# Adredes-weslee/elliptic-gnn-project

Hardware: AMD Instinct MI355X
Metric: edges/s full-batch SAGE fwd+bwd, Elliptic 203k/234k/166-feat, 1→8 MI355X (higher is better)
Workload: dtype f32; 1 GPU; configs/sage.yaml + symmetrize_edges=true: SAGE 2L 166->128->2, dropout 0.5, full-batch train step (fwd+masked CE+bwd+clip+Adam); global_nodes=203769, global_edges=468710, feats=166, max_nodes_per_gpu=203769, max_edges_per_gpu=468710, parallelism=single, launch=hip-graph replay of the whole step

## Files before the change

### elliptic_gnn_project_amd/_lib.py

```python
from __future__ import annotations

import ctypes
import os
from pathlib import Path

import torch

PKG_DIR = Path(__file__).resolve().parent
LIB_PATH = Path(os.environ["GNNMP_LIB"]) if os.environ.get("GNNMP_LIB") else PKG_DIR / "libgnnmp.so"
ABI_VERSION = 27

DTYPE_F32 = 0
DTYPE_BF16 = 1

MATH_SPLIT_BF16 = 0
MATH_F32 = 1
MATH_HALF_PAIR = 2

PLANES_SPLIT_BF16 = 0
PLANES_HALF_PAIR = 1

GNN_OK = 0
_STATUS_EXC = {
    1: ValueError,
    2: IndexError,
    3: RuntimeError,
    4: RuntimeError,
    5: NotImplementedError,
}

LOOPS_KEEP = 0
LOOPS_REPLACE = 1

AGG_SUM = 0
AGG_MEAN = 1
AGG_MEAN_BWD = 2
AGG_GCN = 3
AGG_EDGE_W = 4

c_i64 = ctypes.c_int64
c_i32 = ctypes.c_int32
c_ptr = ctypes.c_void_p
c_size = ctypes.c_size_t


class GnnSplit(ctypes.Structure):
    _fields_ = [
        ("seg_len", c_i32),
        ("reserved", c_i32),
        ("num_long", c_i64),
        ("num_pieces", c_i64),
        ("ptr", c_ptr),
        ("nbr", c_ptr),
        ("piece0", c_ptr),
        ("piece_seg", c_ptr),
        ("long_seg", c_ptr),
        ("order", c_ptr),
    ]


class GnnGraph(ctypes.Structure):
    _fields_ = [
        ("num_nodes", c_i64),
# ... 26 lines not shown
        ("seed_ptr", c_ptr),
        ("addend2", c_ptr),
        ("ld_add2", c_i64),
    ]


class GnnGemmNTParams(ctypes.Structure):
    _fields_ = [
        ("M", c_i64), ("N", c_i64),
        ("a1", c_ptr), ("lda1", c_i64), ("k1", c_i64),
        ("a2", c_ptr), ("lda2", c_i64), ("k2", c_i64),
        ("bt", c_ptr), ("ldb", c_i64),
        ("w1", c_ptr), ("w2", c_ptr), ("ldw1", c_i64), ("ldw2", c_i64),
        ("c", c_ptr), ("ldc", c_i64),
        ("bias", c_ptr),
        ("relu", c_i32),
        ("dropout_p", ctypes.c_float),
        ("seed", ctypes.c_uint64),
        ("seed_ptr", c_ptr),
        ("proj", c_ptr), ("nproj", c_i32), ("z", c_ptr), ("ldz", c_i64),
        ("math", c_i32),
        ("workspace", c_ptr), ("workspace_bytes", c_size),
        ("a_dtype", c_i32), ("c_dtype", c_i32),
        ("mask", c_ptr), ("ldmask", c_i64), ("mask_scale", ctypes.c_float),
        ("a_planes", c_ptr), ("planes_ld", c_i64), ("planes_stride", c_i64), ("planes_col2", c_i64),
        ("planes_format", c_i32), ("keep_mask", c_ptr), ("b_ready", c_i32), ("planes_exp", c_i32),
        ("colsum_part", c_ptr), ("colsum_cap", c_i64),
        ("row_exp", c_ptr),
    ]


class GnnGemmTNParams(ctypes.Structure):
    _fields_ = [
        ("M", c_i64), ("Nr", c_i64),
        ("g", c_ptr), ("ldg", c_i64),
        ("dz", c_ptr), ("lddz", c_i64),
        ("proj", c_ptr), ("nproj", c_i32),
        ("h", c_ptr), ("ldh", c_i64), ("hscale", ctypes.c_float),
        ("gout", c_ptr), ("ldgout", c_i64),
        ("a1", c_ptr), ("lda1", c_i64), ("k1", c_i64),
        ("a2", c_ptr), ("lda2", c_i64), ("k2", c_i64),
        ("math", c_i32),
        ("a_dtype", c_i32), ("h_dtype", c_i32),
        ("a_planes", c_ptr), ("planes_ld", c_i64), ("planes_stride", c_i64), ("planes_col2", c_i64),
        ("planes_format", c_i32), ("g_dtype", c_i32), ("planes_exp", c_i32),
        ("sq_partial", c_ptr), ("sq_step", c_ptr), ("sq_skip_lo", c_i64), ("sq_skip_hi", c_i64), ("sq_cap", c_i64),
        ("row_exp", c_ptr),
        ("g_rowmax", c_ptr),
        ("dz_graph", c_ptr), ("dz_u", c_ptr), ("ldu", c_i64), ("dz_cols", c_i32),
    ]


ROWMAX_ROWS = 16


ACT_NONE = 0
ACT_ELU = 1


class GnnGatFwdParams(ctypes.Structure):
    _fields_ = [
        ("heads", c_i32), ("chans", c_i32), ("concat", c_i32),
        ("slope", ctypes.c_float),
        ("xh", c_ptr), ("ld_xh", c_i64),
        ("att_src", c_ptr), ("att_dst", c_ptr),
        ("bias", c_ptr),
        ("act", ctypes.c_int),
        ("dropout_p", ctypes.c_float),
        ("seed", ctypes.c_uint64), ("seed_ptr", c_ptr),
        ("a_src", c_ptr), ("a_dst", c_ptr),
        ("alpha", c_ptr),
        ("out", c_ptr), ("ldo", c_i64),
        ("edge_w", c_ptr),
        ("proj", c_ptr), ("nproj", c_i32), ("z", c_ptr), ("ldz", c_i64),
    ]


ADAM_MAX_TENSORS = 24


class GnnAdamTensor(ctypes.Structure):
    _fields_ = [("param", c_ptr), ("grad", c_ptr), ("exp_avg", c_ptr), ("exp_avg_sq", c_ptr), ("numel", c_i64)]


class GnnAdamGroup(ctypes.Structure):
    _fields_ = [
        ("num_tensors", c_i32),
        ("lr", ctypes.c_double), ("beta1", ctypes.c_double), ("beta2", ctypes.c_double), ("eps", ctypes.c_double),
        ("weight_decay", ctypes.c_double), ("max_norm", ctypes.c_double),
        ("tensors", GnnAdamTensor * ADAM_MAX_TENSORS),
        ("skip_nonfinite", c_i32),
        ("bump_counter", c_ptr),
        ("loss_partial", c_ptr), ("loss_nblk", c_i32), ("loss_scale", ctypes.c_float), ("loss_out", c_ptr),
        ("grad_sq_partial", c_ptr), ("grad_sq_nblk", c_i32),
    ]


class GnnCeSpec(ctypes.Structure):
    _fields_ = [
        ("y", c_ptr), ("mask", c_ptr), ("class_w", c_ptr), ("row_w", c_ptr),
        ("inv_denom", ctypes.c_float), ("focal", c_i32), ("focal_gamma", ctypes.c_float),
        ("reserved", c_i32 * 5),
    ]


SIGNATURES = {
    "gnn_abi_version": (ctypes.c_int, []),
    "gnn_status_string": (ctypes.c_char_p, [ctypes.c_int]),
    "gnn_last_error": (ctypes.c_char_p, []),
    "gnn_graph_workspace_size": (ctypes.c_int, [c_i64, c_i64, ctypes.POINTER(c_size)]),
    "gnn_graph_build": (
        ctypes.c_int,
        [c_ptr, c_i64, c_i64, ctypes.c_int, c_ptr, c_ptr, c_ptr, c_ptr, c_ptr, c_ptr, c_ptr, c_ptr, c_size, c_ptr],
    ),
    "gnn_split_workspace_size": (ctypes.c_int, [c_i64, ctypes.POINTER(c_size)]),
    "gnn_split_count": (ctypes.c_int, [c_ptr, c_i64, c_i32, c_ptr, c_ptr]),
    "gnn_split_build": (
        ctypes.c_int,
        [c_ptr, c_ptr, c_i64, c_i32, c_ptr, c_ptr, c_ptr, c_ptr, c_ptr, c_ptr, c_ptr, c_size, c_ptr],
    ),
    "gnn_in_degree_f32": (ctypes.c_int, [ctypes.POINTER(GnnGraph), c_ptr, c_ptr]),
    "gnn_gcn_norm_f32": (ctypes.c_int, [ctypes.POINTER(GnnGraph), c_ptr, c_ptr]),
    "gnn_aggregate_f32": (
        ctypes.c_int,
        [ctypes.POINTER(GnnGraph), ctypes.POINTER(GnnAggParams), c_ptr, c_i64, c_i64, c_ptr, c_i64, c_ptr],
    ),
    "gnn_aggregate_bf16": (
        ctypes.c_int,
        [ctypes.POINTER(GnnGraph), ctypes.POINTER(GnnAggParams), c_ptr, c_i64, c_i64, c_ptr, c_i64, c_ptr],
    ),
    "gnn_sage_mean_fwd_f32": (
        ctypes.c_int,
        [ctypes.POINTER(GnnGraph), c_ptr, c_ptr, c_i64, c_i64, c_ptr, c_i64, c_ptr],
    ),
    "gnn_split_planes_f32": (ctypes.c_int, [c_ptr, c_i64, c_i64, c_i64, c_ptr, c_i64, c_i64, c_i64, c_i64, c_ptr]),
    "gnn_sage_mean_fwd_planes": (
        ctypes.c_int,
        [ctypes.POINTER(GnnGraph), c_ptr, c_ptr, c_i64, c_i64, c_ptr, c_i64, c_i64, c_i64, c_ptr],
    ),
    "gnn_split_h2_f32": (ctypes.c_int, [c_ptr, c_i64, c_i64, c_i64, c_ptr, c_i64, c_i64, c_i64, c_i64, c_i32, c_ptr]),
    "gnn_sage_mean_fwd_h2": (
        ctypes.c_int,
        [ctypes.POINTER(GnnGraph), c_ptr, c_ptr, c_i64, c_i64, c_ptr, c_i64, c_i64, c_i64, c_i32,
         c_ptr, c_i64, ctypes.c_float, ctypes.c_uint64, c_ptr, ctypes.POINTER(GnnGemmNTParams),
         ctypes.POINTER(GnnSplit), c_ptr],
    ),
    "gnn_sage_out_mean_ce_f32": (
        ctypes.c_int,
        [ctypes.POINTER(GnnGraph), c_ptr, c_ptr, c_i64, c_i32, c_ptr, c_ptr, c_i64, c_ptr, c_ptr, c_ptr,
         ctypes.c_float, c_ptr, c_i64, c_ptr, c_i64, c_ptr, c_ptr, c_ptr, c_size, c_ptr],
    ),
    "gnn_sage_mean_bwd_f32": (
        ctypes.c_int,
        [ctypes.POINTER(GnnGraph), c_ptr, c_ptr, c_i64, c_i64, c_ptr, c_i64, c_ptr],
    ),
    "gnn_edge_dot_f32": (
        ctypes.c_int,
        [ctypes.POINTER(GnnGraph), c_ptr, c_ptr, c_ptr, c_i64, c_ptr, c_i64, c_i64, c_ptr, c_ptr],
    ),
    "gnn_gat_scores_f32": (
        ctypes.c_int,
        [c_i64, c_i32, c_i32, c_ptr, c_i64, c_ptr, c_ptr, c_ptr, c_ptr, c_ptr],
    ),
    "gnn_gat_fwd_f32": (
        ctypes.c_int,
        [ctypes.POINTER(GnnGraph), c_i32, c_i32, c_i32, ctypes.c_float, c_ptr, c_i64, c_ptr, c_ptr,
         c_ptr, c_ptr, c_ptr, c_i64, c_ptr],
    ),
    "gnn_gat_fwd_fused_f32": (ctypes.c_int, [ctypes.POINTER(GnnGraph), ctypes.POINTER(GnnGatFwdParams), c_ptr]),
    "gnn_gat_out_ce_f32": (
        ctypes.c_int,
        [ctypes.POINTER(GnnGraph), ctypes.POINTER(GnnGatFwdParams), c_ptr, c_ptr, c_ptr, ctypes.c_float, c_ptr, c_i64,
         c_ptr, c_ptr, c_ptr, c_size, c_ptr]),
    "gnn_gat_act_bwd_f32": (
        ctypes.c_int,
        [c_i64, c_i64, ctypes.c_int, ctypes.c_float, ctypes.c_uint64, c_ptr, c_ptr, c_i64, c_ptr, c_i64, c_ptr,
         c_i64, c_ptr],
    ),
    "gnn_gat_bwd_workspace_size": (ctypes.c_int, [c_i64, c_i64, c_i32, c_i32, ctypes.POINTER(c_size)]),
    "gnn_gat_bwd_f32": (
        ctypes.c_int,
        [ctypes.POINTER(GnnGraph), c_i32, c_i32, c_i32, ctypes.c_float, c_ptr, c_i64, c_ptr, c_ptr, c_ptr,
         c_ptr, c_ptr, c_ptr, c_i64, c_ptr, c_i64, c_ptr, c_ptr, c_ptr, c_size, c_ptr],
    ),
    "gnn_gat_bwd_act_proj_f32": (
        ctypes.c_int,
        [ctypes.POINTER(GnnGraph), c_i32, c_i32, ctypes.c_float, c_ptr, c_i64, c_ptr, c_ptr, c_ptr, c_ptr, c_ptr,
         c_i32, ctypes.c_float, ctypes.c_uint64, c_ptr, c_ptr, c_i64, c_ptr, c_i64, c_ptr, c_i32, c_ptr, c_i64,
         c_ptr, c_i64, c_ptr, c_ptr, c_ptr, c_ptr, c_size, c_ptr]),
    "gnn_gat_bwd_act_f32": (
        ctypes.c_int,
        [ctypes.POINTER(GnnGraph), c_i32, c_i32, ctypes.c_float, c_ptr, c_i64, c_ptr, c_ptr, c_ptr, c_ptr, c_ptr,
         c_i32, ctypes.c_float, ctypes.c_uint64, c_ptr, c_ptr, c_i64, c_ptr, c_i64, c_ptr, c_i64, c_ptr, c_i64,
         c_ptr, c_ptr, c_ptr, c_size, c_ptr],
    ),
    "gnn_gat_bwd_ew_f32": (
        ctypes.c_int,
        [ctypes.POINTER(GnnGraph), c_i32, c_i32, c_i32, ctypes.c_float, c_ptr, c_i64, c_ptr, c_ptr, c_ptr,
         c_ptr, c_ptr, c_ptr, c_i64, c_ptr, c_i64, c_ptr, c_ptr, c_ptr, c_ptr, c_ptr, c_size, c_ptr],
    ),
    "gnn_gemm_nt_workspace_size": (ctypes.c_int, [c_i64, c_i64, c_i64, ctypes.POINTER(c_size)]),
    "gnn_gemm_nt_f32": (ctypes.c_int, [ctypes.POINTER(GnnGemmNTParams), c_ptr]),
    "gnn_gemm_nt_prep_b": (ctypes.c_int, [ctypes.POINTER(GnnGemmNTParams), c_ptr]),
    "gnn_masked_ce_finish": (ctypes.c_int, [c_ptr, c_i32, ctypes.c_float, c_ptr, c_ptr]),
    "gnn_gemm_tn_workspace_size": (ctypes.c_int, [c_i64, c_i64, c_i64, c_i32, ctypes.POINTER(c_size)]),
    "gnn_gemm_tn_sq_blocks": (ctypes.c_int, [c_i64, ctypes.POINTER(c_i32)]),
    "gnn_gemm_tn_f32": (ctypes.c_int, [ctypes.POINTER(GnnGemmTNParams), c_ptr, c_ptr, c_size, c_ptr]),
    "gnn_gemm_nt_planes_ok": (ctypes.c_int, [ctypes.POINTER(GnnGemmNTParams)]),
    "gnn_gemm_nt_colsum_blocks": (ctypes.c_int, [ctypes.POINTER(GnnGemmNTParams), ctypes.POINTER(c_i32)]),
    "gnn_colsum_finish_f32": (ctypes.c_int, [c_ptr, c_i32, c_i64, c_ptr, c_ptr]),
    "gnn_gemm_tn_planes_ok": (ctypes.c_int, [ctypes.POINTER(GnnGemmTNParams)]),
    "gnn_colsum_workspace_size": (ctypes.c_int, [c_i64, c_i64, ctypes.POINTER(c_size)]),
    "gnn_colsum_f32": (ctypes.c_int, [c_i64, c_i64, c_ptr, c_i64, c_ptr, c_ptr, c_size, c_ptr]),
    "gnn_masked_ce_workspace_size": (ctypes.c_int, [c_i64, ctypes.POINTER(c_size)]),
    "gnn_masked_ce_f32": (
        ctypes.c_int,
        [c_i64, c_i32, c_ptr, c_i64, c_ptr, c_ptr, c_ptr, ctypes.c_float, c_ptr, c_i64, c_ptr, c_ptr, c_size, c_ptr],
    ),
    "gnn_gcn_out_ce_f32": (
        ctypes.c_int,
        [ctypes.POINTER(GnnGraph), c_ptr, c_ptr, c_i64, c_i32, c_ptr, c_ptr, c_i64, c_ptr, c_ptr, c_ptr,
         ctypes.c_float, c_ptr, c_i64, c_ptr, c_ptr, c_ptr, c_size, c_ptr],
    ),
    "gnn_masked_ce_colsum_f32": (
        ctypes.c_int,
        [c_i64, c_i32, c_ptr, c_i64, c_ptr, c_ptr, c_ptr, ctypes.c_float, c_ptr, c_i64, c_ptr, c_ptr, c_size, c_ptr,
         c_ptr],
    ),
    "gnn_masked_ce_spec_f32": (
        ctypes.c_int,
        [c_i64, c_i32, c_ptr, c_i64, ctypes.POINTER(GnnCeSpec), c_ptr, c_i64, c_ptr, c_ptr, c_size, c_ptr, c_ptr],
    ),
    "gnn_sage_out_mean_ce_spec_f32": (
        ctypes.c_int,
        [ctypes.POINTER(GnnGraph), c_ptr, c_ptr, c_i64, c_i32, c_ptr, c_ptr, c_i64, ctypes.POINTER(GnnCeSpec),
         c_ptr, c_i64, c_ptr, c_i64, c_ptr, c_ptr, c_ptr, c_size, c_ptr],
    ),
    "gnn_gcn_out_ce_spec_f32": (
        ctypes.c_int,
        [ctypes.POINTER(GnnGraph), c_ptr, c_ptr, c_i64, c_i32, c_ptr, c_ptr, c_i64, ctypes.POINTER(GnnCeSpec),
         c_ptr, c_i64, c_ptr, c_ptr, c_ptr, c_size, c_ptr],
    ),
    "gnn_gat_out_ce_spec_f32": (
        ctypes.c_int,
        [ctypes.POINTER(GnnGraph), ctypes.POINTER(GnnGatFwdParams), ctypes.POINTER(GnnCeSpec), c_ptr, c_i64,
         c_ptr, c_ptr, c_ptr, c_size, c_ptr]),
    "gnn_clip_adam_workspace_size": (ctypes.c_int, [ctypes.POINTER(c_size)]),
    "gnn_neighbor_sample_workspace_size": (ctypes.c_int, [c_i64, c_i64, c_i64, ctypes.POINTER(c_size)]),
    "gnn_neighbor_sample": (
        ctypes.c_int,
        [ctypes.POINTER(GnnGraph), c_ptr, c_ptr, c_i64, c_i32, c_ptr, ctypes.c_uint64, c_ptr, c_i64, c_ptr, c_ptr,
         c_ptr, c_i64, c_ptr, c_ptr, c_ptr, c_size, c_ptr],
    ),
    "gnn_clip_adam_f32": (ctypes.c_int, [ctypes.POINTER(GnnAdamGroup), c_ptr, c_ptr, c_ptr, c_size, c_ptr]),
    "gnn_bn_workspace_size": (ctypes.c_int, [c_i64, ctypes.POINTER(c_size)]),
    "gnn_bn_stats_f32": (
        ctypes.c_int,
        [c_ptr, c_i64, c_i64, c_i64, c_ptr, c_i32, ctypes.c_float, ctypes.c_float, c_ptr, c_ptr, c_ptr, c_ptr,
         c_ptr, c_ptr, c_size, c_ptr],
    ),
# ... 84 lines not shown
```

### elliptic_gnn_project_amd/aggregation.py

```python
from __future__ import annotations

import os

import torch

from . import _lib
from .graph import GraphPlan, get_plan

__all__ = ["mean_aggregate", "masked_mean_aggregate", "masked_gcn_aggregate", "edge_dot", "gcn_aggregate", "gat_attention", "gat_attention_proj", "aggregate", "colsum", "KernelTimer"]


class KernelTimer:

    active = False
    records: list = []

    @classmethod
    def start(cls):
        cls.records = []
        cls.active = True

    @classmethod
    def begin(cls):
        if not cls.active:
            return None
        e = torch.cuda.Event(enable_timing=True)
        e.record()
        return e

    @classmethod
    def end(cls, e0, tag, amount):
        if e0 is None:
            return
        e1 = torch.cuda.Event(enable_timing=True)
        e1.record()
        cls.records.append((tag, e0, e1, int(amount)))

    @classmethod
    def stop(cls):
        cls.active = False
        torch.cuda.synchronize()
        out = {}
        for tag, a, b, amount in cls.records:
            ms = a.elapsed_time(b)
            d = out.setdefault(tag, {"launches": 0, "ms": 0.0, "amount": 0})
            d["launches"] += 1
            d["ms"] += ms
            d["amount"] += amount
        cls.records = []
        return out

_custom_fwd = torch.amp.custom_fwd(device_type="cuda", cast_inputs=torch.float32)
_custom_bwd = torch.amp.custom_bwd(device_type="cuda")


def _as_f32_rows(x: torch.Tensor) -> torch.Tensor:
    if x.dtype != torch.float32:
        raise TypeError(f"libgnnmp fp32 path got {x.dtype}")
    if x.dim() != 2:
        raise ValueError(f"expected [N, F] features, got {tuple(x.shape)}")
    if x.stride(1) != 1 or x.stride(0) < x.size(1):
        x = x.contiguous()
    return x


def _ld(x: torch.Tensor) -> int:
    return max(int(x.stride(0)), int(x.size(1)), 1)


SPLIT_MAX_F = 128


def aggregate(plan: GraphPlan, x: torch.Tensor, mode: int, transpose: bool = False,
              nodew: torch.Tensor | None = None, ew: torch.Tensor | None = None, heads: int = 1,
              addend: torch.Tensor | None = None, bias: torch.Tensor | None = None,
              relu: bool = False, out: torch.Tensor | None = None, dropout_p: float = 0.0, seed: int = 0,
              seed_ptr: torch.Tensor | None = None, addend2: torch.Tensor | None = None) -> torch.Tensor:
    if x.dtype == torch.bfloat16:
        if dropout_p > 0 or addend2 is not None:
            raise NotImplementedError("dropout / addend2 epilogue on the bf16-storage aggregation")
        return _aggregate_bf16(plan, x, mode, transpose, nodew, addend, bias, relu, out)
    x = _as_f32_rows(x)
    N, F = plan.num_nodes, x.size(1)
    if x.size(0) != N:
        raise ValueError(f"feature rows {x.size(0)} != plan nodes {N}")
    if out is None:
        out = torch.empty((N, F), dtype=torch.float32, device=x.device)
    if addend is not None:
        addend = _as_f32_rows(addend)
    if addend2 is not None:
        addend2 = _as_f32_rows(addend2)
    npieces = plan.split_pieces(transpose) if (mode != _lib.AGG_EDGE_W and 8 < F <= SPLIT_MAX_F) else 0
    part = torch.empty(npieces * F, dtype=torch.float32, device=x.device) if npieces else None
    p = _lib.GnnAggParams(
        mode, int(transpose), _lib.ptr(nodew), _lib.ptr(ew), int(heads),
        _lib.ptr(addend), _ld(addend) if addend is not None else 0,
        _lib.ptr(bias), int(relu), _lib.ptr(part), part.numel() * 4 if part is not None else 0,
        float(dropout_p), int(seed) & 0xFFFFFFFFFFFFFFFF, _lib.ptr(seed_ptr),
        _lib.ptr(addend2), _ld(addend2) if addend2 is not None else 0,
    )
    if KernelTimer.active:
        a = torch.cuda.Event(enable_timing=True)
        b = torch.cuda.Event(enable_timing=True)
        a.record()
    _lib.call("gnn_aggregate_f32", plan.c_graph, p, x.data_ptr(), _ld(x), F, out.data_ptr(), _ld(out),
              _lib.stream_handle(x.device))
    if KernelTimer.active:
        b.record()
        KernelTimer.records.append((("agg", int(mode), bool(transpose), int(F)), a, b,
                                    agg_bytes(plan, F, mode, transpose, int(addend is not None) + int(addend2 is not None))))
    return out


def _aggregate_bf16(plan, x, mode, transpose, nodew, addend, bias, relu, out):
    if x.dim() != 2 or x.stride(1) != 1:
        x = x.contiguous()
    N, F = plan.num_nodes, x.size(1)
    if x.size(0) != N:
        raise ValueError(f"feature rows {x.size(0)} != plan nodes {N}")
    if out is None:
        out = torch.empty((N, F), dtype=torch.bfloat16, device=x.device)
    if out.dtype != torch.bfloat16:
        raise TypeError("bf16 aggregation writes bf16")
    if addend is not None:
        addend = _as_f32_rows(addend)
    p = _lib.GnnAggParams(
        mode, int(transpose), _lib.ptr(nodew), None, 1,
        _lib.ptr(addend), _ld(addend) if addend is not None else 0,
        _lib.ptr(bias), int(relu), None, 0,
    )
    if KernelTimer.active:
        a = torch.cuda.Event(enable_timing=True)
        b = torch.cuda.Event(enable_timing=True)
        a.record()
    _lib.call("gnn_aggregate_bf16", plan.c_graph, p, x.data_ptr(), _ld(x), F, out.data_ptr(), _ld(out),
              _lib.stream_handle(x.device))
    if KernelTimer.active:
        b.record()
        KernelTimer.records.append((("agg_bf16", int(mode), bool(transpose), int(F)), a, b,
                                    agg_bytes(plan, F, mode, transpose, addend is not None, elem=2)))
    return out


def agg_bytes(plan: GraphPlan, F: int, mode: int, transpose: bool, has_addend, elem: int = 4) -> int:
    N, S = plan.num_nodes, plan.num_slots
    b = 4 * (N + 1) + 4 * S + elem * S * F + elem * N * F
    if mode in (_lib.AGG_MEAN,):
        b += 4 * N
    elif mode in (_lib.AGG_MEAN_BWD, _lib.AGG_GCN):
        b += 4 * S
    b += 4 * N * F * int(has_addend)
    return b


def colsum_of(x: torch.Tensor) -> torch.Tensor:
    part = getattr(x, "_gnnmp_colsum", None)
    if part is not None and x.dim() == 2 and x.size(1) > 0 and part.numel() % x.size(1) == 0 and part.numel() > 0:
        out = torch.empty(x.size(1), dtype=torch.float32, device=x.device)
        _lib.call("gnn_colsum_finish_f32", part.data_ptr(), part.numel() // x.size(1), x.size(1), out.data_ptr(),
# ... 411 lines not shown
```

### elliptic_gnn_project_amd/csrc/aggregate.hip

```cpp
#include "gemm_common.hpp"

namespace gnnmp {
namespace {

template <int VEC>
struct VecT;
template <>
struct VecT<1> { using T = float; };
template <>
struct VecT<2> { using T = float2; };
template <>
struct VecT<4> { using T = float4; };

template <int VEC>
__device__ __forceinline__ void vload(const float* p, float (&v)[VEC]) {
  if constexpr (VEC == 4) {
    float4 t = *reinterpret_cast<const float4*>(p);
    v[0] = t.x; v[1] = t.y; v[2] = t.z; v[3] = t.w;
  } else if constexpr (VEC == 2) {
    float2 t = *reinterpret_cast<const float2*>(p);
    v[0] = t.x; v[1] = t.y;
  } else {
    v[0] = *p;
  }
// ... 16 lines not shown
    const uint4 t = *reinterpret_cast<const uint4*>(p);
    v[0] = __uint_as_float(t.x << 16); v[1] = __uint_as_float(t.x & 0xffff0000u);
    v[2] = __uint_as_float(t.y << 16); v[3] = __uint_as_float(t.y & 0xffff0000u);
    v[4] = __uint_as_float(t.z << 16); v[5] = __uint_as_float(t.z & 0xffff0000u);
    v[6] = __uint_as_float(t.w << 16); v[7] = __uint_as_float(t.w & 0xffff0000u);
  } else if constexpr (VEC == 4) {
    const uint2 t = *reinterpret_cast<const uint2*>(p);
    v[0] = __uint_as_float(t.x << 16); v[1] = __uint_as_float(t.x & 0xffff0000u);
    v[2] = __uint_as_float(t.y << 16); v[3] = __uint_as_float(t.y & 0xffff0000u);
  } else if constexpr (VEC == 2) {
    const uint32_t t = *reinterpret_cast<const uint32_t*>(p);
    v[0] = __uint_as_float(t << 16); v[1] = __uint_as_float(t & 0xffff0000u);
  } else {
    v[0] = __uint_as_float((uint32_t)p[0] << 16);
  }
}

__device__ __forceinline__ uint16_t to_bf16(float f) { return __builtin_bit_cast(uint16_t, (__bf16)f); }

template <int VEC>
__device__ __forceinline__ void vstore_bf(uint16_t* p, const float (&v)[VEC]) {
  if constexpr (VEC == 8) {
    *reinterpret_cast<uint4*>(p) = make_uint4((uint32_t)to_bf16(v[0]) | ((uint32_t)to_bf16(v[1]) << 16),
                                              (uint32_t)to_bf16(v[2]) | ((uint32_t)to_bf16(v[3]) << 16),
                                              (uint32_t)to_bf16(v[4]) | ((uint32_t)to_bf16(v[5]) << 16),
                                              (uint32_t)to_bf16(v[6]) | ((uint32_t)to_bf16(v[7]) << 16));
  } else if constexpr (VEC == 4) {
    *reinterpret_cast<uint2*>(p) = make_uint2((uint32_t)to_bf16(v[0]) | ((uint32_t)to_bf16(v[1]) << 16),
                                              (uint32_t)to_bf16(v[2]) | ((uint32_t)to_bf16(v[3]) << 16));
  } else if constexpr (VEC == 2) {
    *reinterpret_cast<uint32_t*>(p) = (uint32_t)to_bf16(v[0]) | ((uint32_t)to_bf16(v[1]) << 16);
  } else {
    p[0] = to_bf16(v[0]);
  }
}

struct AggArgs {
  const int32_t* ptr;
  const int32_t* nbr;
  const int32_t* wslot;
  const float* nodew;
  const float* ew;
  int32_t heads;
  int32_t chan;
  const float* x; int64_t ldx;
  float* y; int64_t ldy;
  const float* add; int64_t ld_add;
  const float* add2; int64_t ld_add2;
  const float* bias;
  int32_t relu;
  int64_t nrows;
  int32_t F;
  const int32_t* piece0;
  const int32_t* order;
  float* part;
  const int32_t* fptr;
  const int32_t* fnbr;
  int32_t seg_len;
  int32_t dropout; uint32_t keep_thresh; float drop_scale; uint64_t seed; const int64_t* seed_ptr;
  uint16_t* yp; int64_t yps; int32_t ywidth;
  float yscale;
  uint32_t* kmask; int32_t kcols;
  H2Prep hp;
  int32_t nhub; float hub_deg; const int32_t* hubs;
  const int32_t* wstart;
  const int64_t* ce_y; const uint8_t* ce_mask; const float* ce_w; float ce_inv;
  float* ce_dl; int64_t ce_ldd; float* ce_part;
  float* ce_u; int64_t ce_ldu;
  const float* ce_rw; int32_t ce_focal; float ce_gamma;
  float* ce_cs;
};

__device__ __forceinline__ uint64_t agg_seed(const AggArgs& a) {
  return a.seed_ptr ? (uint64_t)(*a.seed_ptr) * 0x9E3779B97F4A7C15ull + a.seed : a.seed;
}

template <int VEC>
__device__ __forceinline__ void agg_dropout(const AggArgs& a, uint64_t seed, int64_t r, int f0, float (&t)[VEC]) {
  if (a.dropout) {
    const uint32_t i0 = (uint32_t)r * (uint32_t)a.F + (uint32_t)f0;
#pragma unroll
    for (int q = 0; q < VEC; ++q) t[q] = keep_elem(seed, i0 + (uint32_t)q, a.keep_thresh) ? t[q] * a.drop_scale : 0.0f;
  }
}

template <int MODE, int VEC>
__device__ __forceinline__ void contrib(const AggArgs& a, int32_t n, int32_t r, int64_t slot,
                                        int f0, float (&v)[VEC]) {
  if constexpr (MODE == GNN_AGG_MEAN_BWD) {
    float d = fmaxf(a.nodew[n], 1.0f);
#pragma unroll
    for (int q = 0; q < VEC; ++q) v[q] = v[q] / d;
  } else if constexpr (MODE == GNN_AGG_GCN) {
    const float w = a.nodew[n] * a.nodew[r];
#pragma unroll
    for (int q = 0; q < VEC; ++q) v[q] = w * v[q];
  } else if constexpr (MODE == GNN_AGG_EDGE_W) {
    int64_t ws = a.wslot ? (int64_t)a.wslot[slot] : slot;
    float w = a.ew[ws * a.heads + f0 / a.chan];
#pragma unroll
    for (int q = 0; q < VEC; ++q) v[q] = w * v[q];
  }
}

template <int MODE, int VEC, bool BF = false>
__device__ __forceinline__ void contrib_w(const AggArgs& a, float wn, int32_t r, float (&v)[VEC]) {
// ... 668 lines not shown
#pragma unroll
      for (int f = 0; f < NF; ++f) {
        float v = xv[f];
        if constexpr (MODE == GNN_AGG_GCN) {
          v = (wn * wr) * v;
        } else if constexpr (MODE == GNN_AGG_MEAN_BWD) {
          v = v / fmaxf(wn, 1.0f);
        } else {
          float t[1] = {v};
          contrib<MODE, 1>(a, n, (int32_t)r, k, f, t);
          v = t[0];
        }
        acc[f] += f < a.F ? v : 0.0f;
      }
    }
#pragma unroll
    for (int f = 0; f < NF; ++f) {
#pragma unroll
      for (int off = kGroup / 2; off >= 1; off >>= 1) acc[f] += __shfl_xor(acc[f], off);
    }
    if (sub == 0) {
      const int32_t p0 = a.piece0 ? a.piece0[r] : -1;
      const float dr = MODE == GNN_AGG_MEAN ? fmaxf(a.nodew[r], 1.0f) : 1.0f;
      float addv[NF], add2v[NF], bv[NF];
#pragma unroll
      for (int f = 0; f < NF; ++f) {
        const int fc = f < a.F ? f : 0;
        addv[f] = a.add ? a.add[r * a.ld_add + fc] : 0.0f;
        add2v[f] = a.add2 ? a.add2[r * a.ld_add2 + fc] : 0.0f;
        bv[f] = a.bias ? a.bias[fc] : 0.0f;
      }
      const uint64_t dseed = a.dropout ? agg_seed(a) : 0;
#pragma unroll
      for (int f = 0; f < NF; ++f) {
        if (f < a.F) {
          float t[1] = {acc[f]};
          if (p0 >= 0) {
            a.part[(int64_t)p0 * a.F + f] = t[0];
          } else {
            if constexpr (MODE == GNN_AGG_MEAN) t[0] = t[0] / dr;
            if (a.add) t[0] += addv[f];
            if (a.add2) t[0] += add2v[f];
            if (a.bias) t[0] += bv[f];
            if (a.relu) t[0] = fmaxf(t[0], 0.0f);
            if (a.dropout) agg_dropout<1>(a, dseed, r, f, t);
            a.y[r * a.ldy + f] = t[0];
          }
        }
      }
    }
  }
}

template <int MODE, int NF, int kNarrowCap = 256, bool COOP = false, bool CE = false, bool CEV = false>
__global__ __launch_bounds__(256) void agg_narrow_lds_kernel(AggArgs a) {
  __shared__ float sv[4][kNarrowCap * 4];
  const int lane = threadIdx.x & 63;
  const int w = threadIdx.x >> 6;
  const int64_t r0 = ((int64_t)blockIdx.x * 4 + w) * 64;
  float lg[4] = {0.f, 0.f, 0.f, 0.f};
  int64_t ce_t = -1;
  float ce_deg = 1.0f;
  uint8_t ce_m = 0;
  float ce_w[4] = {0.f, 0.f, 0.f, 0.f};
  float ce_rw = 1.0f;
  if constexpr (!CE) {
    if (r0 >= a.nrows) return;
  }
  if (r0 < a.nrows) {
  const int64_t r = r0 + lane;
  const bool rok = r < a.nrows;
  const int32_t pbeg = a.ptr[rok ? r : a.nrows];
  const int32_t pend = a.ptr[rok ? r + 1 : a.nrows];
  const int32_t base = __builtin_amdgcn_readfirstlane(a.ptr[r0]);
  const int64_t rlast = min(r0 + 64, a.nrows);
  const int32_t wend = __builtin_amdgcn_readfirstlane(a.ptr[rlast]);
  const int F = a.F;
  const int64_t rr = rok ? r : r0;
  float pdeg = 1.0f, padd[4] = {0.f, 0.f, 0.f, 0.f}, padd2[4] = {0.f, 0.f, 0.f, 0.f}, pbias[4] = {0.f, 0.f, 0.f, 0.f};
  if constexpr (MODE == GNN_AGG_MEAN) pdeg = fmaxf(a.nodew[rr], 1.0f);
  static_assert(MODE != GNN_AGG_GCN || NF == 2, "GCN rows stage their slot weight in plane 2");
  float wrow = 1.0f;
  if constexpr (MODE == GNN_AGG_GCN) wrow = a.nodew[rr];
  if (a.add) {
#pragma unroll
    for (int f = 0; f < NF; ++f) padd[f] = a.add[rr * a.ld_add + (f < F ? f : 0)];
  }
  if (a.add2) {
#pragma unroll
    for (int f = 0; f < NF; ++f) padd2[f] = a.add2[rr * a.ld_add2 + (f < F ? f : 0)];
  }
  if (a.bias) {
#pragma unroll
    for (int f = 0; f < NF; ++f) pbias[f] = a.bias[f < F ? f : 0];
  }
  if constexpr (CE) {
    ce_deg = pdeg;
    ce_t = a.ce_y[rr];
    ce_m = a.ce_mask[rr];
#pragma unroll
    for (int c = 0; c < 4; ++c) ce_w[c] = a.ce_w[c < F ? c : 0];
    if constexpr (CEV) {
      if (a.ce_rw) ce_rw = a.ce_rw[rr];
    }
  }
  float acc[4] = {0.f, 0.f, 0.f, 0.f};
  float* buf = sv[w];
  for (int32_t pb = base; pb < wend; pb += kNarrowCap) {
    const int32_t pe = min(pb + kNarrowCap, wend);
    constexpr int NI = kNarrowCap / 64;
    int32_t nn[NI];
#pragma unroll
    for (int i = 0; i < NI; ++i) {
      const int32_t k = pb + lane + 64 * i;
      nn[i] = a.nbr[k < pe ? k : pb];
    }
    float xv[NI][NF], dd[NI];
#pragma unroll
    for (int i = 0; i < NI; ++i) {
      const float* xr = a.x + (int64_t)nn[i] * a.ldx;
#pragma unroll
      for (int f = 0; f < NF; ++f) xv[i][f] = xr[f < F ? f : 0];
      dd[i] = 1.0f;
      if constexpr (MODE == GNN_AGG_MEAN_BWD || MODE == GNN_AGG_GCN) dd[i] = a.nodew[nn[i]];
    }
#pragma unroll
    for (int i = 0; i < NI; ++i) {
#pragma unroll
      for (int f = 0; f < NF; ++f) {
        float v = f < F ? xv[i][f] : 0.0f;
        if constexpr (MODE == GNN_AGG_MEAN_BWD) v = v / fmaxf(dd[i], 1.0f);
        buf[f * kNarrowCap + lane + 64 * i] = v;
      }
      if constexpr (MODE == GNN_AGG_GCN) buf[2 * kNarrowCap + lane + 64 * i] = dd[i];
    }
    __builtin_amdgcn_s_waitcnt(0xc07f);
    __builtin_amdgcn_wave_barrier();
    const int32_t lo = max(pbeg, pb), hi0 = min(pend, pe);
    constexpr int CAP = 32;
    const int32_t hi = COOP ? min(hi0, lo + CAP) : hi0;
    float q1[4] = {0.f, 0.f, 0.f, 0.f}, q2[4] = {0.f, 0.f, 0.f, 0.f}, q3[4] = {0.f, 0.f, 0.f, 0.f};
    auto sv_at = [&](int f, int32_t s, float wr) __attribute__((always_inline)) {
      const float x = buf[f * kNarrowCap + (s - pb)];
      if constexpr (MODE == GNN_AGG_GCN) return (buf[2 * kNarrowCap + (s - pb)] * wr) * x;
      else return x;
    };
    int32_t k = lo;
    for (; k + 3 < hi; k += 4) {
#pragma unroll
      for (int f = 0; f < NF; ++f) {
        acc[f] += sv_at(f, k, wrow);
        q1[f] += sv_at(f, k + 1, wrow);
        q2[f] += sv_at(f, k + 2, wrow);
        q3[f] += sv_at(f, k + 3, wrow);
      }
    }
    for (; k < hi; ++k) {
#pragma unroll
      for (int f = 0; f < NF; ++f) acc[f] += sv_at(f, k, wrow);
    }
#pragma unroll
    for (int f = 0; f < NF; ++f) acc[f] += (q1[f] + q2[f]) + q3[f];
    if constexpr (COOP) {
      uint64_t longm = __ballot(hi0 - lo > CAP);
      while (longm) {
        const int L = __builtin_ctzll(longm);
        longm &= longm - 1;
        const int32_t s0 = __builtin_amdgcn_readlane(lo, L) + CAP, s1 = __builtin_amdgcn_readlane(hi0, L);
        const float wL = __int_as_float(__builtin_amdgcn_readlane(__float_as_int(wrow), L));
        float part[NF];
#pragma unroll
        for (int f = 0; f < NF; ++f) part[f] = 0.f;
        for (int32_t k2 = s0 + lane; k2 < s1; k2 += 64) {
#pragma unroll
          for (int f = 0; f < NF; ++f) part[f] += sv_at(f, k2, wL);
        }
#pragma unroll
        for (int f = 0; f < NF; ++f) {
#pragma unroll
          for (int off = 32; off >= 1; off >>= 1) part[f] += __shfl_xor(part[f], off);
          if (lane == L) acc[f] += part[f];
        }
      }
    }
    __builtin_amdgcn_wave_barrier();
  }
  if (rok) {
    const int32_t p0 = a.piece0 ? a.piece0[r] : -1;
#pragma unroll
    for (int f = 0; f < 4; ++f) {
      if (f < F) {
        float t[1] = {acc[f]};
        if (p0 >= 0) {
          a.part[(int64_t)p0 * F + f] = t[0];
        } else {
          if constexpr (MODE == GNN_AGG_MEAN) t[0] = t[0] / pdeg;
          if (a.add) t[0] += padd[f];
          if (a.add2) t[0] += padd2[f];
          if (a.bias) t[0] += pbias[f];
          if (a.relu) t[0] = fmaxf(t[0], 0.0f);
          if (a.dropout) agg_dropout<1>(a, agg_seed(a), r, f, t);
          a.y[r * a.ldy + f] = t[0];
          lg[f] = t[0];
        }
      }
    }
  }
  }
  if constexpr (CE) {
    const int64_t r = r0 + lane;
    const int C = a.F;
    float l = 0.f;
    float dlv[4] = {0.f, 0.f, 0.f, 0.f};
    if (r < a.nrows) {
      const int64_t tg = ce_t;
      const bool on = ce_m != 0 && tg >= 0 && tg < C;
      const float wt = tg == 0 ? ce_w[0] : tg == 1 ? ce_w[1] : tg == 2 ? ce_w[2] : ce_w[3];
      if constexpr (CEV)
        l = masked_ce_row<4, true>(lg, C, tg, on, on ? wt : 0.f, a.ce_inv, a.ce_dl + r * a.ce_ldd, dlv, ce_rw,
                                   a.ce_focal != 0, a.ce_gamma);
      else
        l = masked_ce_row<4>(lg, C, tg, on, on ? wt : 0.f, a.ce_inv, a.ce_dl + r * a.ce_ldd, dlv);
      if (a.ce_u) {
#pragma unroll
        for (int c = 0; c < 4; ++c)
          if (c < C) a.ce_u[r * a.ce_ldu + c] = dlv[c] / ce_deg;
      }
    }
    __shared__ float cesh[4];
    for (int o = 32; o > 0; o >>= 1) l += __shfl_xor(l, o);
    if (lane == 0) cesh[w] = l;
    __syncthreads();
    if (threadIdx.x == 0) {
      float t = 0.f;
      for (int i = 0; i < 4; ++i) t += cesh[i];
      a.ce_part[blockIdx.x] = t;
    }
    if (a.ce_cs) {
      __shared__ float cssh[4][4];
#pragma unroll
      for (int c = 0; c < 4; ++c) {
        float v = c < C ? dlv[c] : 0.f;
        for (int o = 32; o > 0; o >>= 1) v += __shfl_xor(v, o);
        if (lane == 0) cssh[c][w] = v;
      }
      __syncthreads();
      if ((int)threadIdx.x < C) {
        float t = 0.f;
        for (int i = 0; i < 4; ++i) t += cssh[threadIdx.x][i];
        a.ce_cs[(int64_t)blockIdx.x * C + threadIdx.x] = t;
      }
    }
  }
}

template <int MODE, int VEC, int NCH>
__device__ __forceinline__ void agg_piece_wide_body(const AggArgs& a, int64_t npieces, const int32_t* piece_seg,
// ... 89 lines not shown
  int rpw = 16;
  bool prefetch = false;
  bool no_fold = false;
  bool no_split = false;
  bool wave_split = false;
  bool lane_walk = false;
};
#ifdef GNNMP_AGG_LAB
int g_agg_lab_variant = 0;
AggLab agg_lab() {
  const int v = g_agg_lab_variant;
  AggLab l;
  l.rpg = v == 5 ? 4 : v == 6 ? 8 : v == 8 ? -1 : (v == 9 || v == 11) ? 1 : 0;
  l.rpw = (v == 1 || v == 14) ? 8 : (v == 2 || v == 13) ? 4 : v == 3 ? 32 : 16;
  l.prefetch = v == 10 || v == 11; l.no_fold = v == 16; l.no_split = v == 7;
  l.wave_split = v >= 12 && v <= 14; l.lane_walk = v == 15;
  return l;
}
#else
constexpr AggLab agg_lab() { return {}; }
#endif

template <class Fn>
void with_vec(int vec, Fn&& f) {
  if (vec == 4) f(std::integral_constant<int, 4>{});
  else if (vec == 2) f(std::integral_constant<int, 2>{});
  else f(std::integral_constant<int, 1>{});
}

int flat_lps(int nchunk) { return nchunk <= 8 ? 8 : nchunk <= 16 ? 16 : nchunk <= 32 ? 32 : 64; }

template <int MODE, int VEC, int LPS, int NCHMAX>
void launch_flat(const AggArgs& a, int rpg, unsigned blocks, hipStream_t st, [[maybe_unused]] bool prefetch) {
#ifdef GNNMP_AGG_LAB
  if (prefetch) return (void)agg_flat_kernel<MODE, VEC, LPS, NCHMAX, true><<<blocks, 256, 0, st>>>(a, rpg);
#endif
  agg_flat_kernel<MODE, VEC, LPS, NCHMAX><<<blocks, 256, 0, st>>>(a, rpg);
}

template <int MODE>
gnn_status launch_mode(const AggArgs& a, int vec, hipStream_t st, const gnn_split* fold = nullptr) {
  if (a.nrows == 0 || a.F == 0) return GNN_OK;
  const AggLab lab = agg_lab();
  constexpr int kLdsF = MODE == GNN_AGG_EDGE_W ? 0 : MODE == GNN_AGG_GCN ? 2 : 4;
  if (a.F <= kLdsF) {
    if constexpr (kLdsF >= 2) {
      const unsigned nb = (unsigned)ceil_div(a.nrows, 256);
#ifdef GNNMP_AGG_LAB
      if (lab.lane_walk) {
        if (a.F <= 2) agg_narrow_lds_kernel<MODE, 2, 256, false><<<nb, 256, 0, st>>>(a);
        else if constexpr (kLdsF >= 4) agg_narrow_lds_kernel<MODE, 4, 256, false><<<nb, 256, 0, st>>>(a);
      } else
#endif
      if (a.F <= 2) agg_narrow_lds_kernel<MODE, 2, 256, true><<<nb, 256, 0, st>>>(a);
      else if constexpr (kLdsF >= 4) agg_narrow_lds_kernel<MODE, 4, 256, true><<<nb, 256, 0, st>>>(a);
    }
  } else if (a.F <= 8) {
    int64_t blocks = ceil_div(a.nrows * kGroup, 256);
    if (blocks > ((int64_t)1 << 20)) blocks = (int64_t)1 << 20;
    if (a.F > 4) agg_group_kernel<MODE, 8><<<(unsigned)blocks, 256, 0, st>>>(a);
    else if constexpr (kLdsF < 4) {
      if (a.F > 2) agg_group_kernel<MODE, 4><<<(unsigned)blocks, 256, 0, st>>>(a);
      else if constexpr (kLdsF < 2) agg_group_kernel<MODE, 2><<<(unsigned)blocks, 256, 0, st>>>(a);
    }
  } else {
    const int nchunk = a.F / vec;
    const int lps = flat_lps(nchunk);
    if (nchunk > 64 * 4) return fail(GNN_ERR_UNSUPPORTED, "gnn_aggregate_f32", "F too wide for the gather kernel");
    const int rpg = lab.rpg > 0 ? lab.rpg : lab.rpg < 0 ? lps - 1 : a.order ? 1 : (lps == 8 ? 7 : lps == 16 ? 2 : 8);
    const unsigned blocks = (unsigned)ceil_div(ceil_div(a.nrows, rpg) * lps, 256);
    const unsigned wblocks = (unsigned)ceil_div(ceil_div(a.nrows, lab.rpw) * 64, 256);
    with_vec(vec, [&](auto v) {
      constexpr int V = decltype(v)::value;
      if (lps == 64 && nchunk <= 128) agg_wave_kernel<MODE, V, 2, false, 8><<<wblocks, 256, 0, st>>>(a, lab.rpw);
      else if (lps == 64) launch_flat<MODE, V, 64, 4>(a, rpg, blocks, st, lab.prefetch);
      else if (lps == 32) launch_flat<MODE, V, 32, 1>(a, rpg, blocks, st, lab.prefetch);
      else if (lps == 16 && !fold) launch_flat<MODE, V, 16, 1>(a, rpg, blocks, st, lab.prefetch);
      else if (lps == 8) {
        if constexpr (V > 1) launch_flat<MODE, V, 8, 1>(a, rpg, blocks, st, lab.prefetch);
      } else if constexpr (MODE != GNN_AGG_EDGE_W) {
        const unsigned pblocks = (unsigned)ceil_div(fold->num_pieces * 64, 256);
        agg_flat_pieces_kernel<MODE, V, 16, 1><<<blocks + pblocks, 256, 0, st>>>(a, rpg, fold->num_pieces,
                                                                               fold->piece_seg, pblocks);
      }
    });
  }
  return hip_check(hipGetLastError(), "gnn_aggregate_f32");
}

template <int MODE>
gnn_status launch_mode_split(const AggArgs& a, int vec, hipStream_t st, const gnn_split* sp) {
  if (a.nrows == 0 || a.F == 0) return GNN_OK;
  const AggLab lab = agg_lab();
  const bool pieces = sp->num_pieces > sp->num_long;
  const bool fold = pieces && flat_lps(a.F / vec) == 16 && !lab.prefetch && !lab.no_fold;
  const gnn_status s = launch_mode<MODE>(a, vec, st, fold ? sp : nullptr);
  if (s != GNN_OK || sp->num_long == 0) return s;
  const unsigned pblocks = (unsigned)ceil_div(sp->num_pieces * 64, 256);
  const unsigned cblocks = (unsigned)ceil_div(sp->num_long * 64, 256);
  with_vec(vec, [&](auto v) {
    constexpr int V = decltype(v)::value;
#ifdef GNNMP_AGG_LAB
    if (a.F / V > 64) {
      if (pieces) agg_piece_wide_kernel<MODE, V, 2><<<pblocks, 256, 0, st>>>(a, sp->num_pieces, sp->piece_seg);
      return (void)agg_combine_kernel<MODE, V, 2><<<cblocks, 256, 0, st>>>(a, sp->num_long, sp->long_seg);
    }
// ... 44 lines not shown
  const int c = blockIdx.x;
  const int t = threadIdx.x;
  float a0 = 0.f, a1 = 0.f, a2 = 0.f, a3 = 0.f;
  int b = t;
  for (; b + 768 < nblk; b += 1024) {
    a0 += part[(int64_t)b * F + c];
    a1 += part[(int64_t)(b + 256) * F + c];
    a2 += part[(int64_t)(b + 512) * F + c];
    a3 += part[(int64_t)(b + 768) * F + c];
  }
  for (; b < nblk; b += 256) a0 += part[(int64_t)b * F + c];
  red[t] = (a0 + a1) + (a2 + a3);
  __syncthreads();
  for (int s = 128; s > 0; s >>= 1) {
    if (t < s) red[t] += red[t + s];
    __syncthreads();
  }
  if (t == 0) out[c] = red[0];
}

constexpr int64_t kColsumBlocks = 1024;

}
}

using namespace gnnmp;

#ifdef GNNMP_AGG_LAB
extern "C" void gnnx_set_agg_variant(int v) { g_agg_lab_variant = v; }
#endif

static gnn_status agg_args_common(AggArgs& a, const gnn_graph* g, const gnn_agg_params* p, int64_t F, const char* fn) {
  a.ptr = p->transpose ? g->colptr : g->rowptr;
  a.nbr = p->transpose ? g->row : g->col;
  a.nodew = p->nodew;
  a.add = p->addend; a.ld_add = p->ld_add;
  a.bias = p->bias; a.relu = p->relu;
  if (p->dropout_p < 0.f || p->dropout_p >= 1.f) return fail(GNN_ERR_INVALID_ARG, fn, "dropout p in [0,1)");
  if (p->dropout_p > 0.f && (int64_t)g->num_nodes * (int64_t)F >= ((int64_t)1 << 32))
    return fail(GNN_ERR_UNSUPPORTED, fn, "dropout element index (rows x width) must be < 2^32");
  a.dropout = p->dropout_p > 0.f;
  a.keep_thresh = (uint32_t)((1.0 - (double)p->dropout_p) * 16777216.0);
  a.drop_scale = a.dropout ? (float)(1.0 / (1.0 - (double)p->dropout_p)) : 1.0f;
  a.seed = p->seed;
  a.seed_ptr = p->seed_ptr;
  a.nrows = g->num_nodes;
  a.F = (int32_t)F;
  return GNN_OK;
}

extern "C" gnn_status gnn_aggregate_f32(const gnn_graph* g, const gnn_agg_params* p, const float* x,
                                        int64_t ldx, int64_t F, float* y, int64_t ldy,
                                        gnn_stream_t stream) {
  if (!g || !p) return fail(GNN_ERR_INVALID_ARG, __func__, "null graph or params");
  if (F < 0 || F > INT32_MAX || ldx < F || ldy < F)
    return fail(GNN_ERR_INVALID_ARG, __func__, "bad F / leading dimensions");
  if (g->num_nodes > 0 && F > 0 && (!x || !y)) return fail(GNN_ERR_INVALID_ARG, __func__, "null x/y");
  if (p->addend && p->ld_add < F) return fail(GNN_ERR_INVALID_ARG, __func__, "bad ld_add");
  if (p->addend2 && p->ld_add2 < F) return fail(GNN_ERR_INVALID_ARG, __func__, "bad ld_add2");
  AggArgs a{};
  if (const gnn_status s = agg_args_common(a, g, p, F, __func__); s != GNN_OK) return s;
  a.wslot = (p->mode == GNN_AGG_EDGE_W && p->transpose) ? g->csc2csr : nullptr;
  a.ew = p->ew;
  a.heads = p->heads > 0 ? p->heads : 1;
  a.x = x; a.ldx = ldx; a.y = y; a.ldy = ldy;
  a.add2 = p->addend2; a.ld_add2 = p->ld_add2;
  if (!a.ptr || (g->num_slots > 0 && !a.nbr)) return fail(GNN_ERR_INVALID_ARG, __func__, "plan arrays null");
  if ((p->mode == GNN_AGG_MEAN || p->mode == GNN_AGG_MEAN_BWD || p->mode == GNN_AGG_GCN) && !p->nodew)
    return fail(GNN_ERR_INVALID_ARG, __func__, "mode needs nodew");
  if (p->mode == GNN_AGG_EDGE_W) {
    if (!p->ew) return fail(GNN_ERR_INVALID_ARG, __func__, "EDGE_W needs ew");
    if (F % a.heads) return fail(GNN_ERR_INVALID_ARG, __func__, "F not divisible by heads");
    if (p->transpose && !g->csc2csr) return fail(GNN_ERR_INVALID_ARG, __func__, "EDGE_W transpose needs csc2csr");
  }
  a.chan = (int32_t)(F / a.heads > 0 ? F / a.heads : 1);
  auto ok_vec = [&](int v) {
    if (F % v || ldx % v || ldy % v) return false;
    if (p->addend && p->ld_add % v) return false;
    if (p->addend2 && p->ld_add2 % v) return false;
    if (p->mode == GNN_AGG_EDGE_W && a.chan % v) return false;
    int b = 4 * v;
    return aligned(x, b) && aligned(y, b) && aligned(p->addend, b) && aligned(p->addend2, b);
  };
  const gnn_split* sp = p->transpose ? g->csc_split : g->csr_split;
  if (sp && (p->mode == GNN_AGG_EDGE_W || !p->part || sp->seg_len < 1 || sp->seg_len > 64 ||
             p->part_bytes < (size_t)sp->num_pieces * (size_t)F * sizeof(float) ||
             (sp->num_long > 0 && (!sp->ptr || !sp->nbr || !sp->piece0 || !sp->piece_seg || !sp->long_seg))))
    sp = nullptr;
  if (sp) {
    a.fptr = a.ptr;
    a.fnbr = a.nbr;
    a.ptr = sp->ptr;
    a.nbr = sp->nbr;
    a.piece0 = sp->piece0;
    a.order = sp->order;
    a.part = p->part;
    a.seg_len = sp->seg_len;
  }
  int vec = ok_vec(4) ? 4 : (ok_vec(2) ? 2 : 1);
  while (sp && vec > 1 && !aligned(p->part, 4 * vec)) vec >>= 1;
  const AggLab lab = agg_lab();
  if (sp && (F <= 8 || F / vec > (lab.wave_split ? 128 : 32) || lab.no_split)) sp = nullptr;
  if (!sp) {
    a.ptr = p->transpose ? g->colptr : g->rowptr;
    a.nbr = p->transpose ? g->row : g->col;
    a.piece0 = nullptr;
    a.order = nullptr;
    a.part = nullptr;
  }
  hipStream_t st = (hipStream_t)stream;
  switch (p->mode) {
    case GNN_AGG_SUM: return sp ? launch_mode_split<GNN_AGG_SUM>(a, vec, st, sp) : launch_mode<GNN_AGG_SUM>(a, vec, st);
    case GNN_AGG_MEAN: return sp ? launch_mode_split<GNN_AGG_MEAN>(a, vec, st, sp) : launch_mode<GNN_AGG_MEAN>(a, vec, st);
    case GNN_AGG_MEAN_BWD:
      return sp ? launch_mode_split<GNN_AGG_MEAN_BWD>(a, vec, st, sp) : launch_mode<GNN_AGG_MEAN_BWD>(a, vec, st);
    case GNN_AGG_GCN: return sp ? launch_mode_split<GNN_AGG_GCN>(a, vec, st, sp) : launch_mode<GNN_AGG_GCN>(a, vec, st);
    case GNN_AGG_EDGE_W: return launch_mode<GNN_AGG_EDGE_W>(a, vec, st);
  }
  return fail(GNN_ERR_INVALID_ARG, __func__, "unknown mode");
// ... 341 lines not shown
```

### elliptic_gnn_project_amd/csrc/gemm_common.hpp

```cpp
#pragma once
#include "common.hpp"

#include <utility>

typedef float floatx16 __attribute__((ext_vector_type(16)));

namespace gnnmp {

template <typename F, int... I>
__device__ __forceinline__ void static_for_impl(F&& f, std::integer_sequence<int, I...>) {
  (f(std::integral_constant<int, I>{}), ...);
}
template <int N, typename F>
__device__ __forceinline__ void static_for(F&& f) {
  static_for_impl(f, std::make_integer_sequence<int, N>{});
}


constexpr uint32_t kDropGolden = 0x9E3779B1u;
__device__ __forceinline__ bool keep_premixed(uint32_t h, uint64_t seed, uint32_t keep_thresh) {
  h ^= (uint32_t)(seed >> 32);
  h ^= h >> 16;
  h *= 0x85EBCA6Bu;
  h ^= h >> 13;
// ... 98 lines not shown
      const bool hi16 = lane & 16, hi8 = lane & 8;
      const int qsel = (hi16 ? 2 : 0) + (hi8 ? 1 : 0);
#pragma unroll
      for (int r = 0; r < 16; ++r) {
        float ps[4];
#pragma unroll
        for (int q = 0; q < 4; ++q) {
          float sum = acc[tm][0][r] * pw[q][0];
          sum = fmaf(acc[tm][1][r], pw[q][1], sum);
          sum = fmaf(acc[tm][2][r], pw[q][2], sum);
          ps[q] = fmaf(acc[tm][3][r], pw[q][3], sum);
        }
        const float s0 = hi16 ? ps[0] : ps[2], s1 = hi16 ? ps[1] : ps[3];
        const float k0 = (hi16 ? ps[2] : ps[0]) + __shfl_xor(s0, 16);
        const float k1 = (hi16 ? ps[3] : ps[1]) + __shfl_xor(s1, 16);
        float m = (hi8 ? k1 : k0) + __shfl_xor(hi8 ? k0 : k1, 8);
        m += __shfl_xor(m, 4);
        m += __shfl_xor(m, 2);
        m += __shfl_xor(m, 1);
        const int64_t row = rbase + (r & 3) + 8 * (r >> 2);
        if ((lane & 7) == 0 && qsel < a.nproj && row < a.M) a.z[row * a.ldz + qsel] = m;
      }
    }
  }
}

constexpr int TN_THREADS = 1024;
constexpr int KT_PER_WAVE = 3;
constexpr int KMAX = 4 * KT_PER_WAVE * 32;
constexpr int TN_APITCH = KMAX;
constexpr int MAXPROJ = 4;

struct TNArgs {
  int64_t M;
  int32_t Nr;
  const float* g; int64_t ldg;
  const float* dz; int64_t lddz; const float* proj; int32_t nproj;
  const float* h; int64_t ldh; float hscale;
  float* gout; int64_t ldgout;
  const float* a1; int64_t lda1; int32_t k1;
  const float* a2; int64_t lda2; int32_t k2;
  float* slab; int64_t slab_stride;
  int64_t rows_per_block;
  int32_t want_db;
  int32_t a_bf16;
  int32_t h_bf16;
  int32_t g_bf16;
  const uint16_t* ap; int32_t ap_ld; int32_t ap_col2; int64_t ap_ps;
  int32_t ap_h2;
  int32_t ap_exp;
  const int32_t* rowexp;
  const uint32_t* growmax;
  const int32_t* cptr; const int32_t* cnbr; const float* cu; int64_t ldu; int32_t ccols;
};

void launch_nt_x3(const NTArgs& a, void* ws, size_t ws_bytes, hipStream_t st);
size_t nt_x3_workspace(int64_t k1, int64_t k2);
void launch_tn_x3(const TNArgs& a, int nblk, hipStream_t st);
bool nt_h2s_ok(const NTArgs& a);
size_t nt_h2s_workspace(int64_t k1, int64_t k2);
void launch_nt_h2s(const NTArgs& a, void* ws, hipStream_t st);
bool tn_h2s_ok(const TNArgs& a);
void launch_tn_h2s(const TNArgs& a, int nblk, hipStream_t st);

bool nt_ws_ok(const NTArgs& a);
size_t nt_ws_tail_offset(int64_t k1, int64_t k2);
void launch_nt_ws(const NTArgs& a, uint4* img, hipStream_t st);
bool nt_planes_ok(const NTArgs& a);
constexpr int NT_PHASE_PREP = 1, NT_PHASE_RUN = 2, NT_PHASE_ALL = 3;
void launch_nt_ws_planes(const NTArgs& a, uint4* img, hipStream_t st, int phase = NT_PHASE_ALL);
bool nt_img16_ok(const NTArgs& a);
void launch_nt_img16(const NTArgs& a, uint4* img, hipStream_t st, int phase = NT_PHASE_ALL);
bool nt_h2_ok(const NTArgs& a);
H2Prep h2_prep_of(const NTArgs& a, uint4* img);
gnn_status nt_h2_prep_from_params(const gnn_gemm_nt_params* p, H2Prep* out, const char* fn);
void launch_nt_h2(const NTArgs& a, uint4* img, hipStream_t st, int phase = NT_PHASE_ALL);
void launch_prep_h2(const H2Prep& p, hipStream_t st);
bool tn_h2_ok(const TNArgs& a);
void launch_tn_h2(const TNArgs& a, int nblk, hipStream_t st, bool ks = false);
bool tn_planes_ok(const TNArgs& a);
void launch_tn_planes(const TNArgs& a, int nblk, hipStream_t st);
bool tn_img16_ok(const TNArgs& a);
void launch_tn_img16(const TNArgs& a, int nblk, hipStream_t st);
__device__ __forceinline__ void split3_pair(float a, float b, uint32_t& h, uint32_t& m, uint32_t& l) {
  typedef __bf16 bf16x2_ __attribute__((ext_vector_type(2)));
  typedef float f32x2_ __attribute__((ext_vector_type(2)));
  h = __builtin_bit_cast(uint32_t, __builtin_convertvector(f32x2_{a, b}, bf16x2_));
  a -= __uint_as_float(h << 16);
  b -= __uint_as_float(h & 0xffff0000u);
  m = __builtin_bit_cast(uint32_t, __builtin_convertvector(f32x2_{a, b}, bf16x2_));
  a -= __uint_as_float(m << 16);
  b -= __uint_as_float(m & 0xffff0000u);
  l = __builtin_bit_cast(uint32_t, __builtin_convertvector(f32x2_{a, b}, bf16x2_));
}

__device__ __forceinline__ void split_h2_pair(float a, float b, uint32_t& h, uint32_t& l) {
  typedef _Float16 h2_ __attribute__((ext_vector_type(2)));
  typedef float f32x2_ __attribute__((ext_vector_type(2)));
  const h2_ hv = __builtin_convertvector(f32x2_{a, b}, h2_);
  h = __builtin_bit_cast(uint32_t, hv);
  const float ra = (a - (float)hv[0]) * 2048.0f;
  const float rb = (b - (float)hv[1]) * 2048.0f;
  l = __builtin_bit_cast(uint32_t, __builtin_convertvector(f32x2_{ra, rb}, h2_));
}

__device__ __forceinline__ uint32_t h2_scale_pair(uint32_t h, float s) {
  typedef _Float16 h2_ __attribute__((ext_vector_type(2)));
// ... 78 lines not shown
```

### elliptic_gnn_project_amd/csrc/gemm_f32.hip

```cpp
#include "common.hpp"

#include <algorithm>
#include <cstdlib>

#include "gemm_common.hpp"

namespace gnnmp {
namespace {

constexpr int BNP = BN + 2;


template <int KC, int TM>
struct NTShape {
  static constexpr int BM = 128 * TM;
  static constexpr int APITCH = KC + 1;
  static constexpr int A_PER_THREAD = BM * KC / 256;
  static constexpr int B_PER_THREAD = KC * BN / 256;
};

template <int KC>
__device__ __forceinline__ void nt_chunk_range(const NTArgs& a, int c, const float*& A, int64_t& lda, int& k0,
                                               int& kb0, int& klen) {
  const int nch1 = (a.k1 + KC - 1) / KC;
// ... 652 lines not shown
    if (j + 3 < n) out[j + 3] = t.w;
  }
  if (sq.part) {
    float s2 = 0.f, nf = 0.f;
    const float tv[4] = {t.x, t.y, t.z, t.w};
#pragma unroll
    for (int e = 0; e < 4; ++e) {
      const int64_t je = j + e;
      const bool use = je < n && (je < sq.skip_lo || je >= sq.skip_hi);
      s2 = use ? fmaf(tv[e], tv[e], s2) : s2;
      nf += (use && !isfinite(tv[e])) ? 1.f : 0.f;
    }
#pragma unroll
    for (int off = 8; off >= 1; off >>= 1) {
      s2 += __shfl_xor(s2, off, 16);
      nf += __shfl_xor(nf, off, 16);
    }
    if (o == 0) {
      sq.part[blockIdx.x] = s2;
      sq.part[gridDim.x + blockIdx.x] = nf;
      if (blockIdx.x == 0) sq.part[2 * gridDim.x] = sq.step[0];
    }
  }
}

int tn_blocks(int64_t M) {
  const int64_t chunks = ceil_div(M, 32);
  if (chunks <= 0) return 1;
  const int64_t per = ceil_div(chunks, 256);
  return (int)ceil_div(chunks, per);
}
static int64_t tn_ksplit_max_m() {
  static const int64_t v = [] {
    const char* e = std::getenv("GNNMP_TN_KSPLIT_MAXM");
    return e ? std::atoll(e) : (int64_t)32768;
  }();
  return v;
}

static int64_t tn_h2_rows_per_block(int64_t M, bool dz) {
  const int64_t chunks = ceil_div(M, 32);
  if (dz && M <= tn_ksplit_max_m()) return ceil_div(chunks, 128) * 32;
  return ceil_div(chunks, tn_blocks(M)) * 32;
}
static bool tn_csc_in_kernel(int64_t rows_per_block) {
  static const int v = [] {
    const char* e = std::getenv("GNNMP_TN_CSC_INKERNEL");
    return e ? std::atoi(e) : -1;
  }();
  if (rows_per_block > 1792) return false;
  if (v >= 0) return v != 0;
  return (rows_per_block + 63) / 64 + 1 <= 8;
}

int tn_blocks2(int64_t M) {
  const int64_t chunks = ceil_div(M, 32);
  if (chunks <= 0) return 1;
  const int64_t per = ceil_div(chunks, 768);
  return (int)ceil_div(chunks, per);
}

}
}

using namespace gnnmp;

static gnn_status gemm_nt_dispatch(const gnn_gemm_nt_params* p, gnn_stream_t stream, const char* fn, int phase) {
  if (!p) return fail(GNN_ERR_INVALID_ARG, fn, "null params");
  if (phase == NT_PHASE_ALL && p->b_ready) phase = NT_PHASE_RUN;
  const bool planes_only = p->a_planes && !p->a1;
  if (p->M < 0 || p->N < 1 || p->k1 < 1 || p->k2 < 0 || (!p->a1 && !p->a_planes) ||
      (p->k2 > 0 && !p->a2 && !planes_only))
    return fail(GNN_ERR_INVALID_ARG, fn, "bad shapes / null operands");
  if (!p->bt && !(p->w1 && (p->k2 == 0 || p->w2)))
    return fail(GNN_ERR_INVALID_ARG, fn, "need bt or w1 (and w2 when k2 > 0)");
  if (p->w1 && (p->N > BN || p->ldw1 < p->k1 || (p->k2 > 0 && p->ldw2 < p->k2)))
    return fail(GNN_ERR_INVALID_ARG, fn, "w1/w2 form needs N <= 128 and ldw >= k");
  if ((!planes_only && (p->lda1 < p->k1 || (p->k2 > 0 && p->lda2 < p->k2))) || (p->bt && p->ldb < p->N) ||
      (p->c && p->ldc < p->N))
    return fail(GNN_ERR_INVALID_ARG, fn, "bad leading dimensions");
  if (p->nproj < 0 || p->nproj > 4 || (p->nproj > 0 && (p->N > BN || !p->proj || !p->z || p->ldz < p->nproj)))
    return fail(GNN_ERR_INVALID_ARG, fn, "projection needs N <= 128, nproj <= 4, proj and z");
  if (p->dropout_p < 0.f || p->dropout_p >= 1.f) return fail(GNN_ERR_INVALID_ARG, fn, "dropout p in [0,1)");
  if (p->dropout_p > 0.f && (int64_t)p->M * (int64_t)p->N >= ((int64_t)1 << 32))
    return fail(GNN_ERR_UNSUPPORTED, fn, "dropout element index (rows x width) must be < 2^32");
  if (p->math != GNN_MATH_SPLIT_BF16 && p->math != GNN_MATH_F32 && p->math != GNN_MATH_HALF_PAIR)
    return fail(GNN_ERR_INVALID_ARG, fn, "bad math mode");
  if ((p->a_dtype != GNN_DTYPE_F32 && p->a_dtype != GNN_DTYPE_BF16) || (p->c_dtype != GNN_DTYPE_F32 && p->c_dtype != GNN_DTYPE_BF16))
    return fail(GNN_ERR_INVALID_ARG, fn, "bad dtype");
  if (p->row_exp && (p->a_planes || p->colsum_part || phase != NT_PHASE_ALL))
    return fail(GNN_ERR_UNSUPPORTED, fn, "row_exp needs the in-kernel half-pair NT over f32 A1 / A2");
  if (p->M == 0 && phase != NT_PHASE_PREP) return GNN_OK;
  NTArgs a{};
  a.M = p->M; a.Nc = (int32_t)p->N;
  a.a1 = p->a1; a.lda1 = p->lda1; a.k1 = (int32_t)p->k1;
  a.a2 = p->a2; a.lda2 = p->lda2; a.k2 = (int32_t)p->k2;
  a.bt = p->bt; a.ldb = p->ldb; a.w1 = p->w1; a.w2 = p->w2; a.ldw1 = p->ldw1; a.ldw2 = p->ldw2; a.c = p->c;
  a.ldc = p->ldc; a.bias = p->bias; a.relu = p->relu;
  a.dropout = p->dropout_p > 0.f;
  a.keep_thresh = (uint32_t)((1.0 - (double)p->dropout_p) * 16777216.0);
  a.drop_scale = a.dropout ? (float)(1.0 / (1.0 - (double)p->dropout_p)) : 1.0f;
  a.seed = p->seed;
  a.seed_ptr = p->seed_ptr;
  a.proj = p->proj; a.nproj = p->nproj; a.z = p->z; a.ldz = p->ldz;
  auto al = [](const void* q, int b) { return (reinterpret_cast<uintptr_t>(q) % b) == 0; };
  a.wvec2 = a.w1 && (a.ldw1 % 2 == 0) && (a.k1 % 2 == 0) && al(a.w1, 8) &&
// ... 66 lines not shown
    return fail(phase == NT_PHASE_PREP ? GNN_ERR_UNSUPPORTED : GNN_ERR_INVALID_ARG, fn,
                "a separate B prep (prep_b / b_ready) needs an image-A kernel (gnn_gemm_nt_planes_ok)");
  const bool h2s = p->math == GNN_MATH_HALF_PAIR && nt_h2s_ok(a) && p->workspace &&
                   p->workspace_bytes >= nt_h2s_workspace(a.k1, a.k2);
  if (p->row_exp && !h2s)
    return fail(GNN_ERR_UNSUPPORTED, fn, "row_exp needs the in-kernel half-pair NT (GNN_MATH_HALF_PAIR, the w1/w2 "
                                         "form, N <= 128, k1 / k2 multiples of 16, k1 + k2 <= 128, f32, a workspace)");
  if (!p->row_exp && launch_nt_skinny(a, st)) return hip_check(hipGetLastError(), fn);
  if (p->mask) return fail(GNN_ERR_UNSUPPORTED, fn, "the mask epilogue needs a skinny shape (K <= 8 or N <= 8)");
  if (a.a_bf16 || a.c_bf16) {
    if (!a.a_bf16 || !a.w1 || a.Nc > BN || p->math == GNN_MATH_F32)
      return fail(GNN_ERR_UNSUPPORTED, fn, "bf16 NT needs bf16 A, the w1/w2 form, N <= 128 and split math");
    launch_nt_x3(a, p->workspace, p->workspace_bytes, st);
    return hip_check(hipGetLastError(), fn);
  }
  if (h2s) {
    a.rowexp = p->row_exp;
    launch_nt_h2s(a, p->workspace, st);
    return hip_check(hipGetLastError(), fn);
  }
  if (p->math != GNN_MATH_F32 && a.w1 && a.Nc <= BN) {
    launch_nt_x3(a, p->workspace, p->workspace_bytes, st);
    return hip_check(hipGetLastError(), fn);
  }
  if (v4) launch_nt_f32<4>(a, st);
  else if (v2) launch_nt_f32<2>(a, st);
  else launch_nt_f32<1>(a, st);
  return hip_check(hipGetLastError(), fn);
}

extern "C" gnn_status gnn_gemm_nt_workspace_size(int64_t N, int64_t k1, int64_t k2, size_t* bytes) {
  if (!bytes || N < 1 || k1 < 1 || k2 < 0) return fail(GNN_ERR_INVALID_ARG, __func__, "bad args");
  *bytes = N <= BN ? std::max(nt_x3_workspace(k1, k2), (size_t)21 * 3 * 256 * 16 + BN * sizeof(float)) : 0;
  return GNN_OK;
}

extern "C" gnn_status gnn_gemm_nt_f32(const gnn_gemm_nt_params* p, gnn_stream_t stream) {
  return gemm_nt_dispatch(p, stream, __func__, NT_PHASE_ALL);
}

extern "C" gnn_status gnn_gemm_nt_prep_b(const gnn_gemm_nt_params* p, gnn_stream_t stream) {
  return gemm_nt_dispatch(p, stream, __func__, NT_PHASE_PREP);
}


extern "C" gnn_status gnn_gemm_tn_workspace_size(int64_t M, int64_t Nr, int64_t Kc, int32_t nproj, size_t* bytes) {
  if (!bytes || M < 0 || Nr < 1 || Kc < 1 || nproj < 0) return fail(GNN_ERR_INVALID_ARG, __func__, "bad args");
  int64_t stride = Nr * Kc + Nr + (int64_t)nproj * Nr + nproj;
  stride = (stride + 63) / 64 * 64;
  int64_t nb = tn_blocks(M);
  if (Nr <= 8 && nproj == 0) nb = std::max<int64_t>(nb, tn_skinny_blocks(M));
  if (Nr <= 64 && Kc <= 128 && nproj == 0) nb = std::max<int64_t>(nb, tn_blocks2(M));
  *bytes = (size_t)nb * stride * sizeof(float);
  return GNN_OK;
}

static gnn_status gemm_tn_dispatch(const gnn_gemm_tn_params* p, float* out, void* workspace,
                                   size_t workspace_bytes, gnn_stream_t stream);

static bool tn_csc_args(const gnn_gemm_tn_params* p, TNArgs* a) {
  a->cptr = nullptr; a->cnbr = nullptr; a->cu = nullptr; a->ldu = 0; a->ccols = 0;
  const gnn_graph* cg = p->dz_graph;
  if (!cg) return true;
  if (!p->dz || !p->dz_u || !cg->colptr || !cg->row || cg->num_nodes != p->M || p->dz_cols < 1 || p->dz_cols > 2 ||
      p->dz_cols > p->nproj || p->ldu < p->dz_cols)
    return false;
  a->cptr = cg->colptr; a->cnbr = cg->row; a->cu = p->dz_u; a->ldu = p->ldu; a->ccols = p->dz_cols;
  return true;
}

static unsigned red_blocks(int64_t n_out) { return (unsigned)ceil_div(ceil_div(n_out, 4), kRedOut); }

extern "C" gnn_status gnn_gemm_tn_sq_blocks(int64_t n_out, int32_t* nb) {
  if (!nb || n_out < 1) return fail(GNN_ERR_INVALID_ARG, __func__, "bad args");
  *nb = (int32_t)red_blocks(n_out);
  return GNN_OK;
}

extern "C" gnn_status gnn_gemm_tn_f32(const gnn_gemm_tn_params* p, float* out, void* workspace,
                                      size_t workspace_bytes, gnn_stream_t stream) {
  return gemm_tn_dispatch(p, out, workspace, workspace_bytes, stream);
}


static gnn_status gemm_tn_dispatch(const gnn_gemm_tn_params* p, float* out, void* workspace,
                                   size_t workspace_bytes, gnn_stream_t stream) {
  const char* __fn = "gnn_gemm_tn_f32";
  if (!p || !out) return fail(GNN_ERR_INVALID_ARG, __fn, "null params/out");
  if (p->M < 0 || p->Nr < 1 || p->Nr > 128 || p->k1 < 1 || p->k2 < 0 || p->k1 + p->k2 > KMAX)
    return fail(GNN_ERR_UNSUPPORTED, __fn, "needs 1 <= Nr <= 128 and k1 + k2 <= 384");
  const bool planes_only = p->a_planes && !p->a1;
  if (!planes_only && (!p->a1 || (p->k2 > 0 && !p->a2) || p->lda1 < p->k1 || (p->k2 > 0 && p->lda2 < p->k2)))
    return fail(GNN_ERR_INVALID_ARG, __fn, "bad A operands");
  if (p->dz) {
    if (p->nproj < 1 || p->nproj > MAXPROJ || !p->proj || p->lddz < p->nproj)
      return fail(GNN_ERR_INVALID_ARG, __fn, "dz form needs 1 <= nproj <= 4 and proj");
  } else if (!p->g || p->ldg < p->Nr) {
    return fail(GNN_ERR_INVALID_ARG, __fn, "need g (or dz + proj)");
  }
  if (p->h && p->ldh < p->Nr) return fail(GNN_ERR_INVALID_ARG, __fn, "bad ldh");
  if (p->math != GNN_MATH_SPLIT_BF16 && p->math != GNN_MATH_F32 && p->math != GNN_MATH_HALF_PAIR)
    return fail(GNN_ERR_INVALID_ARG, __fn, "bad math mode");
  if (p->gout && p->ldgout < p->Nr) return fail(GNN_ERR_INVALID_ARG, __fn, "bad ldgout");
  const int32_t nproj = p->dz ? p->nproj : 0;
  const int64_t Kc = p->k1 + p->k2;
  const int64_t n_out = p->Nr * Kc + p->Nr + (int64_t)nproj * p->Nr + nproj;
  int64_t stride = (n_out + 63) / 64 * 64;
  int nblk = tn_blocks(p->M);
  if (!workspace || workspace_bytes < (size_t)nblk * stride * sizeof(float))
    return fail(GNN_ERR_WORKSPACE, __fn, "workspace too small");
  hipStream_t st = (hipStream_t)stream;
  SqOut sqo{};
  if (p->sq_partial) {
    if (!p->sq_step || p->sq_cap < 2 * (int64_t)red_blocks(n_out) + 1 || p->sq_skip_lo > p->sq_skip_hi)
      return fail(GNN_ERR_INVALID_ARG, __fn, "sq_partial needs sq_step, sq_cap >= 2 nb + 1, skip_lo <= skip_hi");
    sqo = SqOut{p->sq_partial, p->sq_step, p->sq_skip_lo, p->sq_skip_hi};
  }
  if (p->M == 0) {
    if (!p->sq_partial) return hip_check(hipMemsetAsync(out, 0, n_out * sizeof(float), st), __fn);
    slab_reduce_kernel<<<red_blocks(n_out), 256, 0, st>>>(static_cast<float*>(workspace), stride, 0, out, n_out, sqo);
    return hip_check(hipGetLastError(), __fn);
  }
  TNArgs a{};
  a.M = p->M; a.Nr = (int32_t)p->Nr;
  a.g = p->g; a.ldg = p->ldg; a.dz = p->dz; a.lddz = p->lddz; a.proj = p->proj; a.nproj = nproj;
  a.h = p->h; a.ldh = p->ldh; a.hscale = p->hscale;
  a.gout = p->gout; a.ldgout = p->ldgout;
  a.a1 = p->a1; a.lda1 = p->lda1; a.k1 = (int32_t)p->k1;
  a.a2 = p->a2; a.lda2 = p->lda2; a.k2 = (int32_t)p->k2;
  a.slab = static_cast<float*>(workspace); a.slab_stride = stride;
  a.rows_per_block = ceil_div(ceil_div(p->M, 32), nblk) * 32;
  if (!tn_csc_args(p, &a))
    return fail(GNN_ERR_INVALID_ARG, __fn, "dz_graph needs the dz form, dz_u, 1 <= dz_cols <= 2 and num_nodes == M");
  auto al8 = [](const void* q) { return (reinterpret_cast<uintptr_t>(q) & 7) == 0; };
  const bool v2 = (a.k1 % 2 == 0) && (a.lda1 % 2 == 0) && al8(a.a1) &&
                  (a.k2 == 0 || ((a.k2 % 2 == 0) && (a.lda2 % 2 == 0) && al8(a.a2)));
  const bool proj = a.dz != nullptr, mask = a.h != nullptr;
  a.a_bf16 = p->a_dtype == GNN_DTYPE_BF16;
  a.h_bf16 = p->h_dtype == GNN_DTYPE_BF16;
  a.g_bf16 = p->g_dtype == GNN_DTYPE_BF16;
  if ((p->a_dtype != GNN_DTYPE_F32 && p->a_dtype != GNN_DTYPE_BF16) || (p->h_dtype != GNN_DTYPE_F32 && p->h_dtype != GNN_DTYPE_BF16) ||
      (p->g_dtype != GNN_DTYPE_F32 && p->g_dtype != GNN_DTYPE_BF16))
    return fail(GNN_ERR_INVALID_ARG, __fn, "bad dtype");
  if (a.g_bf16 && !(p->a_planes && a.a_bf16))
    return fail(GNN_ERR_UNSUPPORTED, __fn, "bf16 g / gout need the bf16-image TN (a bf16 a_planes)");
  if (a.h_bf16 && !a.a_bf16) return fail(GNN_ERR_UNSUPPORTED, __fn, "bf16 h needs bf16 A");
  const int64_t ldmax = std::max({a.lda1, a.k2 > 0 ? a.lda2 : 0, a.h ? a.ldh : 0, a.g ? a.ldg : 0, a.dz ? a.lddz : 0});
  if (p->a_planes) {
    if (p->planes_format != GNN_PLANES_SPLIT_BF16 && p->planes_format != GNN_PLANES_HALF_PAIR)
      return fail(GNN_ERR_INVALID_ARG, __fn, "bad planes_format");
    a.ap = static_cast<const uint16_t*>(p->a_planes);
    a.ap_ld = (int32_t)std::min<int64_t>(p->planes_ld, INT32_MAX);
    a.ap_col2 = (int32_t)std::min<int64_t>(p->planes_col2, INT32_MAX);
    a.ap_ps = p->planes_stride;
    a.ap_h2 = p->planes_format == GNN_PLANES_HALF_PAIR;
    a.ap_exp = a.ap_h2 ? p->planes_exp : 0;
    if (a.ap_exp < -100 || a.ap_exp > 100) return fail(GNN_ERR_INVALID_ARG, __fn, "planes_exp outside [-100, 100]");
    if (a.ap_h2) {
      a.growmax = (!a.dz && a.g) ? p->g_rowmax : nullptr;
      if (p->math != GNN_MATH_F32 && tn_h2_ok(a)) {
        int nred = nblk;
        const bool ks = a.dz && a.M <= tn_ksplit_max_m();
        if (ks) {
          const int64_t chunks = ceil_div(a.M, 32), per = ceil_div(chunks, 128);
          nred = (int)ceil_div(chunks, per);
          a.rows_per_block = per * 32;
        }
        if (a.rows_per_block != tn_h2_rows_per_block(a.M, a.dz != nullptr))
          return fail(GNN_ERR_HIP, __fn, "internal: TN row-block rule mismatch");
        if (a.cptr && !tn_csc_in_kernel(a.rows_per_block)) {
          gnn_agg_params ag{};
          ag.mode = GNN_AGG_SUM;
          ag.transpose = 1;
          const gnn_status s = gnn_aggregate_f32(p->dz_graph, &ag, p->dz_u, p->ldu, p->dz_cols,
                                                 const_cast<float*>(p->dz), p->lddz, stream);
          if (s != GNN_OK) return s;
          a.cptr = nullptr;
        }
        launch_tn_h2(a, ks ? 2 * nred : nblk, st, ks);
        GNN_LAUNCH_CHECK();
        slab_reduce_kernel<<<red_blocks(n_out), 256, 0, st>>>(a.slab, stride, nred, out, n_out, sqo);
        GNN_LAUNCH_CHECK();
        return GNN_OK;
      }
      if (planes_only) return fail(GNN_ERR_UNSUPPORTED, __fn, "half-pair image A outside the half-pair kernel's shapes");
      a.ap = nullptr;
    }
  }
  if (a.cptr)
    return fail(GNN_ERR_UNSUPPORTED, __fn, "dz_graph outside the half-pair dz-form TN (gnn_gemm_tn_planes_ok)");
  if (p->a_planes) {
    if (a.ap && a.a_bf16) {
      if (p->math == GNN_MATH_F32 || !tn_img16_ok(a))
        return fail(GNN_ERR_UNSUPPORTED, __fn, "bf16 image A outside the image kernel's shapes");
      launch_tn_img16(a, nblk, st);
      GNN_LAUNCH_CHECK();
      slab_reduce_kernel<<<red_blocks(n_out), 256, 0, st>>>(a.slab, stride, nblk, out, n_out, sqo);
      GNN_LAUNCH_CHECK();
      return GNN_OK;
    }
    if (a.ap && p->math != GNN_MATH_F32 && tn_planes_ok(a)) {
      launch_tn_planes(a, nblk, st);
      GNN_LAUNCH_CHECK();
      slab_reduce_kernel<<<red_blocks(n_out), 256, 0, st>>>(a.slab, stride, nblk, out, n_out, sqo);
      GNN_LAUNCH_CHECK();
      return GNN_OK;
    }
    if (planes_only) return fail(GNN_ERR_UNSUPPORTED, __fn, "split-image A outside the planes kernel's shapes");
    a.ap = nullptr;
  }
  if (tn_skinny_ok(a)) {
    nblk = tn_skinny_blocks(a.M);
    if (workspace_bytes < (size_t)nblk * stride * sizeof(float))
      return fail(GNN_ERR_WORKSPACE, __fn, "workspace too small");
    launch_tn_skinny(a, nblk, st);
    GNN_LAUNCH_CHECK();
    slab_reduce_kernel<<<red_blocks(n_out), 256, 0, st>>>(a.slab, stride, nblk, out, n_out, sqo);
    GNN_LAUNCH_CHECK();
    return GNN_OK;
  }
  if (a.a_bf16 && (p->math == GNN_MATH_F32 || (a.M + 32) * ldmax >= ((int64_t)1 << 31) || a.M < 16))
    return fail(GNN_ERR_UNSUPPORTED, __fn, "bf16 TN needs split math, M >= 16 and M*ld < 2^31");
  a.rowexp = p->row_exp;
  if (p->math == GNN_MATH_HALF_PAIR && tn_h2s_ok(a) && (a.M + 32) * ldmax < ((int64_t)1 << 31)) {
    if (a.Nr <= 64 && Kc <= 128 && !nproj && workspace_bytes >= (size_t)tn_blocks2(a.M) * stride * sizeof(float)) {
      nblk = tn_blocks2(a.M);
      a.rows_per_block = ceil_div(ceil_div(a.M, 32), nblk) * 32;
    }
    launch_tn_h2s(a, nblk, st);
    GNN_LAUNCH_CHECK();
    slab_reduce_kernel<<<red_blocks(n_out), 256, 0, st>>>(a.slab, stride, nblk, out, n_out, sqo);
    GNN_LAUNCH_CHECK();
// ... 87 lines not shown
```

### elliptic_gnn_project_amd/csrc/gemm_planes.hip

```cpp
#include "gemm_common.hpp"

typedef __bf16 bf16x8 __attribute__((ext_vector_type(8)));
typedef short s16x4 __attribute__((ext_vector_type(4)));
typedef unsigned int u32x4 __attribute__((ext_vector_type(4)));
typedef __bf16 bf16x2v_t __attribute__((ext_vector_type(2)));
typedef float f32x2v_t __attribute__((ext_vector_type(2)));

namespace gnnmp {
namespace {

__global__ __launch_bounds__(256) void split_planes_kernel(const float* __restrict__ x, int64_t ldx, int64_t rows,
                                                           int32_t F, uint16_t* __restrict__ img, int64_t ld,
                                                           int64_t ps, int32_t width) {
  const int hw = width >> 1;
  const int64_t i = (int64_t)blockIdx.x * 256 + threadIdx.x;
  if (i >= rows * hw) return;
  const int64_t r = i / hw;
  const int c = 2 * (int)(i - r * hw);
  const float* xr = x + r * ldx;
  const float a = c < F ? xr[c] : 0.0f;
  const float b = c + 1 < F ? xr[c + 1] : 0.0f;
  uint32_t h, m, l;
  split3_pair(a, b, h, m, l);
  uint32_t* d = reinterpret_cast<uint32_t*>(img + r * ld + c);
// ... 401 lines not shown
      for (; k + 3 < hi; k += 4) {
#pragma unroll
        for (int f = 0; f < 2; ++f) {
          acc[f] += buf[f * CAP + (k - pb)];
          q1[f] += buf[f * CAP + (k + 1 - pb)];
          q2[f] += buf[f * CAP + (k + 2 - pb)];
          q3[f] += buf[f * CAP + (k + 3 - pb)];
        }
      }
      for (; k < hi; ++k) {
#pragma unroll
        for (int f = 0; f < 2; ++f) acc[f] += buf[f * CAP + (k - pb)];
      }
#pragma unroll
      for (int f = 0; f < 2; ++f) acc[f] += (q1[f] + q2[f]) + q3[f];
      uint64_t longm = __ballot(hi0 - lo > LCAP);
      while (longm) {
        const int L = __builtin_ctzll(longm);
        longm &= longm - 1;
        const int32_t s0 = __builtin_amdgcn_readlane(lo, L) + LCAP, s1 = __builtin_amdgcn_readlane(hi0, L);
        float part[2] = {0.f, 0.f};
        for (int32_t k2 = s0 + lane; k2 < s1; k2 += 64) {
#pragma unroll
          for (int f = 0; f < 2; ++f) part[f] += buf[f * CAP + (k2 - pb)];
        }
#pragma unroll
        for (int f = 0; f < 2; ++f) {
#pragma unroll
          for (int off = 32; off >= 1; off >>= 1) part[f] += __shfl_xor(part[f], off);
          if (lane == L) acc[f] += part[f];
        }
      }
      __builtin_amdgcn_wave_barrier();
    }
    if (rok && r >= mbeg && r < mend) {
#pragma unroll
      for (int f = 0; f < 2; ++f)
        if (f < F) dz[r * a.lddz + f] = acc[f];
      float v[MAXPROJ];
#pragma unroll
      for (int q = 0; q < MAXPROJ; ++q) v[q] = q == 0 ? acc[0] : (q == 1 && F > 1) ? acc[1] : dv[q];
      float sr = 0.f;
#pragma unroll
      for (int q = 0; q < MAXPROJ; ++q) {
        sr += q < nq ? fabsf(v[q]) : 0.f;
        dzb[(r - mbeg) * MAXPROJ + q] = v[q];
      }
      zm = fmaxf(zm, sr);
    }
  }
  return zm;
}

template <int KT, bool GOUT, int LAB = 0, int NW = 4, bool GF = false, int KS = 1, bool CSC = false>
__global__ __launch_bounds__(64 * NW) void gemm_tn_h2_kernel(TNArgs a) {
  static_assert(NW == 4 || NW == 8, "4 or 8 waves");
  static_assert(KS == 1 || (KS == 2 && NW == 8), "split-K: the 8-wave form");
  constexpr int T = 64 * NW;
  constexpr int NPA = (2 * PT_ROWS * (PT_MAXLD / 8) + T - 1) / T;
  constexpr int RP = PT_ROWS / (T / 128);
  constexpr int KTB = KS == 1 ? KT : (KT + 1) / 2;
  constexpr int KTW = NW == 4 ? KTB : (KTB + 1) / 2;
  __shared__ __attribute__((aligned(16))) uint16_t Gt[2][3 * PT_GPL];
  __shared__ __attribute__((aligned(16))) uint16_t At[2][2 * PT_APL];
  __shared__ float dzL[2][256];
  __shared__ float redm[2 * NW];
  constexpr int NU = 2 * NPA + RP / 2 + 2 * RP + RP / 2 + 3;
  constexpr int NG = 3 * KTW;
  constexpr int RING = (LAB & 16) ? 2 : 1;
  constexpr int RGN = 1;
  const int tid = threadIdx.x;
  const int lane = tid & 63;
  const int wave = tid >> 6;
  const int ld = a.ap_ld;
  const int kpart = KS == 1 ? 0 : (int)(blockIdx.x & 1);
  const int rblk = KS == 1 ? (int)blockIdx.x : (int)(blockIdx.x >> 1);
  const int kt0 = kpart * KTB;
  const int ktb = KS == 1 ? KT : (kpart ? KT - KTB : KTB);
  const int pr = min(4 * ktb, (ld - 32 * kt0) >> 3);
  const int64_t mbeg = (int64_t)rblk * a.rows_per_block;
  const int64_t mend = min(a.M, mbeg + a.rows_per_block);
  const int nch = mend > mbeg ? (int)((mend - mbeg + PT_ROWS - 1) / PT_ROWS) : 0;
  typedef _Float16 f16x8 __attribute__((ext_vector_type(8)));
  const int wrow = 32 * (wave & 3);
  const int tbase = NW == 4 ? 0 : (wave >> 2) * KTW;
  const int ntl = NW == 4 ? KT : max(0, min(KTW, ktb - tbase));

  floatx16 acc[KTW];
#pragma unroll
  for (int t = 0; t < KTW; ++t)
#pragma unroll
    for (int r = 0; r < 16; ++r) acc[t][r] = 0.0f;

  const __amdgpu_buffer_rsrc_t arsrc =
      __builtin_amdgcn_make_buffer_rsrc(const_cast<uint16_t*>(a.ap), 0, (int)(2 * a.ap_ps * 2), 0x00020000);
  uint32_t goff[NPA], loff[NPA];
#pragma unroll
  for (int j = 0; j < NPA; ++j) {
    const int q = tid + T * j;
    const int per_plane = PT_ROWS * pr;
    const bool ok = q < 2 * per_plane;
    const int p = q / per_plane, rr = q - p * per_plane;
    const int row = rr / pr, c16 = rr - row * pr;
    goff[j] = ok ? (uint32_t)(((int64_t)p * a.ap_ps + (int64_t)row * ld + 32 * kt0 + 8 * c16) * 2) : 0u;
    loff[j] = ok ? (uint32_t)((p * PT_APL + row * PT_AP + 8 * c16) * 2)
                 : (uint32_t)(((tid & 15) * PT_AP + PT_MAXLD + 8 * ((tid >> 4) & 1)) * 2);
  }

  const int gn = tid & 127, go = tid >> 7;
  const bool gcol = gn < a.Nr;
  const int gnc = gcol ? gn : 0;
  const float* hb = GF ? a.g + gnc : a.h + gnc;
  const int hld = GF ? (int)a.ldg : (int)a.ldh;
  const int zr = (tid & 63) / MAXPROJ, zq = (tid & 63) % MAXPROJ;
  const int zqc = min(zq, a.nproj - 1);
  float pcol[MAXPROJ];
#pragma unroll
  for (int q = 0; q < MAXPROJ; ++q) pcol[q] = (!GF && q < a.nproj && gcol) ? a.proj[q * a.Nr + gn] : 0.0f;

  float gsc = 1.f, gunsc = 1.f;
  float zm_fold = 0.f;
  auto scan_scale = [&]() __attribute__((always_inline)) {
    float zm = zm_fold;
    const int nq = a.nproj;
    if (GF && a.growmax) {
      const int64_t q1 = (mend + GNN_ROWMAX_ROWS - 1) / GNN_ROWMAX_ROWS;
      for (int64_t q = mbeg / GNN_ROWMAX_ROWS + tid; q < q1; q += T) zm = fmaxf(zm, __uint_as_float(a.growmax[q]));
    } else if constexpr (GF) {
      constexpr int SU = 16;
      const int n4 = (a.Nr + 3) >> 2;
      const int64_t npc = (mend - mbeg) * n4;
      for (int64_t q0 = tid; q0 < npc; q0 += SU * T) {
        float4 v[SU];
#pragma unroll
        for (int u = 0; u < SU; ++u) {
          const int64_t q = min(q0 + (int64_t)T * u, npc - 1);
          const int64_t r = mbeg + q / n4;
          const int c4 = (int)(q - (q / n4) * n4) * 4;
          v[u] = *reinterpret_cast<const float4*>(a.g + r * a.ldg + c4);
        }
#pragma unroll
        for (int u = 0; u < SU; ++u) {
          const int64_t q = q0 + (int64_t)T * u;
          const int c4 = (int)(min(q, npc - 1) % n4) * 4;
          float m = fabsf(v[u].x);
          m = fmaxf(m, c4 + 1 < a.Nr ? fabsf(v[u].y) : 0.f);
          m = fmaxf(m, c4 + 2 < a.Nr ? fabsf(v[u].z) : 0.f);
          m = fmaxf(m, c4 + 3 < a.Nr ? fabsf(v[u].w) : 0.f);
          zm = fmaxf(zm, q < npc ? m : 0.f);
        }
      }
    }
    for (int64_t r0 = mbeg + tid; !GF && !CSC && r0 < mend; r0 += 4 * T) {
      float v[4][MAXPROJ];
#pragma unroll
      for (int u = 0; u < 4; ++u) {
        const int64_t r = min(r0 + (int64_t)T * u, mend - 1);
#pragma unroll
        for (int q = 0; q < MAXPROJ; ++q) v[u][q] = a.dz[r * a.lddz + min(q, nq - 1)];
      }
#pragma unroll
      for (int u = 0; u < 4; ++u) {
        float s = 0.f;
#pragma unroll
        for (int q = 0; q < MAXPROJ; ++q) s += q < nq ? fabsf(v[u][q]) : 0.f;
        zm = fmaxf(zm, r0 + (int64_t)T * u < mend ? s : 0.f);
      }
    }
    float pm = 0.f;
#pragma unroll
    for (int q = 0; q < MAXPROJ; ++q) pm = fmaxf(pm, fabsf(pcol[q]));
#pragma unroll
    for (int o = 32; o > 0; o >>= 1) {
      zm = fmaxf(zm, __shfl_xor(zm, o));
      pm = fmaxf(pm, __shfl_xor(pm, o));
    }
    if (lane == 0) {
      redm[wave] = zm;
      redm[NW + wave] = pm;
    }
    __syncthreads();
    zm = redm[0];
    pm = redm[NW];
#pragma unroll
    for (int w = 1; w < NW; ++w) {
      zm = fmaxf(zm, redm[w]);
      pm = fmaxf(pm, redm[NW + w]);
    }
    const float bound = GF ? zm : zm * pm * a.hscale;
    int E = 0;
    if (bound > 0.f && isfinite(bound)) frexpf(bound, &E);
    gsc = ldexpf(1.0f, 4 - E);
    gunsc = ldexpf(1.0f, E - 4 - 11 - a.ap_exp);
  };

  const int Mi = (int)a.M;
  auto ldbase = [&](int c) __attribute__((always_inline)) { return min((int)mbeg + c * PT_ROWS, Mi - PT_ROWS); };
  const int clast = max(nch - 1, 0);
  u32x4 ra[RING][NPA];
  float rg[RGN][RP];
  float rz = 0.f;
  auto load_a = [&](int s, int j, int c) __attribute__((always_inline)) {
    ra[s][j] = __builtin_amdgcn_raw_buffer_load_b128(arsrc, (int)goff[j], ldbase(c) * ld * 2, 0);
  };
  auto load_g = [&](int sg, int c) __attribute__((always_inline)) {
    uint32_t o = (uint32_t)((ldbase(c) + RP * go) * hld);
#pragma unroll
    for (int i = 0; i < RP; ++i) {
      rg[sg][i] = hb[o];
      o += (uint32_t)hld;
    }
  };
  auto load_z = [&](int c) __attribute__((always_inline)) {
    if constexpr (!GF) rz = a.dz[(uint32_t)((ldbase(c) + zr) * (int)a.lddz + zqc)];
  };
  auto put_zv = [&](int k, float v) __attribute__((always_inline)) {
    if constexpr (GF) return;
    const int mb = ldbase(k);
    const bool ok = tid < PT_ROWS * MAXPROJ && zq < a.nproj && zr >= (int)mbeg + k * PT_ROWS - mb && zr < (int)mend - mb;
    if (T == 256 || tid < 256) dzL[k & 1][tid] = ok ? v : 0.0f;
  };
  auto put_z = [&](int k) __attribute__((always_inline)) { put_zv(k, rz); };

  float db = 0.f, dzs = 0.f;
  float dw2[MAXPROJ] = {0.f, 0.f, 0.f, 0.f};
  float e[RP];
  uint32_t w[RP / 2][3];
  float4 zv[RP];
  float zsv[RP];
  auto z_read = [&](int c, int i0, int n) __attribute__((always_inline)) {
    if constexpr (GF) return;
    const int buf = c & 1;
#pragma unroll
    for (int i = i0; i < i0 + n; ++i) {
      const int r = RP * go + i;
      zv[i] = *reinterpret_cast<const float4*>(&dzL[buf][r * MAXPROJ]);
      zsv[i] = dzL[buf][r * MAXPROJ + (gn & (MAXPROJ - 1))];
    }
  };
  auto put_a = [&](int s, int j, int c) __attribute__((always_inline)) {
    *reinterpret_cast<u32x4*>(reinterpret_cast<char*>(At[c & 1]) + loff[j]) = ra[s][j];
  };
  auto g_row = [&](int i, int c, int half, int sg) __attribute__((always_inline)) {
    if constexpr (GF) {
      if (half == 0) return;
      const int mb = ldbase(c);
      const int r = RP * go + i;
      const bool ok = r >= (int)mbeg + c * PT_ROWS - mb && r < (int)mend - mb && gcol;
      const float g = ok ? rg[sg][i] : 0.0f;
      db += g;
      e[i] = g * gsc;
      return;
    }
    if (half == 0) {
      const float4 z = zv[i];
      float g = z.x * pcol[0];
      g = fmaf(z.y, pcol[1], g);
      g = fmaf(z.z, pcol[2], g);
      e[i] = fmaf(z.w, pcol[3], g);
      dw2[0] = fmaf(z.x, rg[sg][i], dw2[0]);
      dw2[1] = fmaf(z.y, rg[sg][i], dw2[1]);
      dw2[2] = fmaf(z.z, rg[sg][i], dw2[2]);
      dw2[3] = fmaf(z.w, rg[sg][i], dw2[3]);
      return;
    }
    float g = e[i];
    dzs += gn < MAXPROJ ? zsv[i] : 0.0f;
    g = rg[sg][i] > 0.0f ? g * a.hscale : 0.0f;
    db += g;
    if constexpr (GOUT) {
      const int mb = ldbase(c);
      const int r = RP * go + i;
      const bool ok = r >= (int)mbeg + c * PT_ROWS - mb && r < (int)mend - mb && gcol;
      if (a.gout && ok) a.gout[(int64_t)(mb + r) * a.ldgout + gn] = g;
    }
    e[i] = g * gsc;
  };
  auto split_pair = [&](int j) __attribute__((always_inline)) {
    split_h2_pair(e[2 * j], e[2 * j + 1], w[j][1], w[j][2]);
    w[j][0] = h2_scale_pair(w[j][1], 2048.0f);
  };
  auto g_put = [&](int c) __attribute__((always_inline)) {
    uint16_t* gd = Gt[c & 1] + gn * PT_GP + RP * go;
#pragma unroll
    for (int p = 0; p < 3; ++p) {
      if constexpr (RP == 8) *reinterpret_cast<uint4*>(gd + p * PT_GPL) = make_uint4(w[0][p], w[1][p], w[2][p], w[3][p]);
      else *reinterpret_cast<uint2*>(gd + p * PT_GPL) = make_uint2(w[0][p], w[1][p]);
    }
  };
  auto unit = [&](int k, int c, int par) __attribute__((always_inline)) {
    constexpr int Z0 = 2 * NPA, G0 = Z0 + RP / 2, S0 = G0 + 2 * RP, P0 = S0 + RP / 2;
    const int sa = RING == 1 ? 0 : (par ^ 1);
    const int sg = RGN == 1 ? 0 : (par ^ 1);
    if (k < Z0) {
      if (k & 1) load_a(sa, k >> 1, min(c + 1 + RING, clast));
      else put_a(sa, k >> 1, c + 1);
    } else if (k < G0) {
      z_read(c + 1, 2 * (k - Z0), 2);
    } else if (k < S0) {
      g_row((k - G0) >> 1, c + 1, (k - G0) & 1, sg);
    } else if (k < P0) {
      split_pair(k - S0);
    } else if (k == P0) {
      g_put(c + 1);
    } else if (k == P0 + 1) {
      load_g(sg, min(c + 1 + RGN, clast));
    } else if (k == P0 + 2) {
      put_z(c + 2);
      load_z(min(c + 3, clast));
    }
  };

  const int gfo = (wrow + (lane & 31)) * PT_GP + 8 * (lane >> 5);
  const int grp = lane >> 4, li = lane & 15;
  const int afo = (8 * (grp >> 1) + (li >> 2)) * PT_AP + 16 * (grp & 1) + 4 * (li & 3);
  auto afrag = [&](const uint16_t* base, int t, int p) __attribute__((always_inline)) {
    const uint16_t* q = base + p * PT_APL + t * 32;
    return __builtin_bit_cast(f16x8, cat_frag(tr_read(q), tr_read(q + 4 * PT_AP)));
  };
#define TH_FENCE __builtin_amdgcn_sched_barrier(0)
  auto compute = [&](int c, auto parc) __attribute__((always_inline)) {
    constexpr int par = decltype(parc)::value;
    const int buf = c & 1;
    f16x8 gf[3], af[2][2];
#pragma unroll
    for (int p = 0; p < 3; ++p) gf[p] = *reinterpret_cast<const f16x8*>(Gt[buf] + p * PT_GPL + gfo);
    const uint16_t* ab = At[buf] + afo;
#pragma unroll
    for (int p = 0; p < 2; ++p) af[0][p] = afrag(ab, tbase, p);
    constexpr int pg[3] = {2, 1, 0}, pa[3] = {0, 1, 0};
    static_for<KTW>([&](auto tc) __attribute__((always_inline)) {
      constexpr int t = decltype(tc)::value;
      if constexpr (t + 1 < KTW && !(LAB & 4)) {
#pragma unroll
        for (int p = 0; p < 2; ++p) af[(t + 1) & 1][p] = afrag(ab, tbase + t + 1, p);
      }
      static_for<3>([&](auto mc) __attribute__((always_inline)) {
        constexpr int m = decltype(mc)::value;
        constexpr int gap = 3 * t + m;
        TH_FENCE;
        if constexpr (!(LAB & 1)) {
          if (NW == 4 || t < ntl)
            acc[t] = __builtin_amdgcn_mfma_f32_32x32x16_f16(gf[pg[m]], af[(LAB & 4) ? 0 : (t & 1)][pa[m]], acc[t], 0, 0, 0);
        }
        TH_FENCE;
        if constexpr (!(LAB & 2)) {
          static_for<(gap + 1) * NU / NG - gap * NU / NG>([&](auto uc) __attribute__((always_inline)) {
            unit(gap * NU / NG + decltype(uc)::value, c, par);
          });
        }
      });
      TH_FENCE;
    });
    if constexpr (NU > NG) {}
    if constexpr ((LAB & 1) != 0) {
#pragma unroll
      for (int t = 0; t < KTW; ++t) acc[t][0] += (float)gf[0][0] + (float)af[0][0][0] + (float)af[1][1][1];
    }
  };
#undef TH_FENCE

  if (nch > 0) {
#pragma unroll
    for (int j = 0; j < NPA; ++j) load_a(0, j, 0);
    if constexpr (RING == 2) {
#pragma unroll
      for (int j = 0; j < NPA; ++j) load_a(1, j, min(1, clast));
    }
    load_g(0, 0);
    if constexpr (RGN == 2) load_g(1, min(1, clast));
    float* dzb = reinterpret_cast<float*>(&At[0][0]) + NW * 2 * 256;
    if constexpr (CSC && !GF) {
      zm_fold = tn_csc_fold<NW>(a, mbeg, mend, reinterpret_cast<float*>(&At[0][0]) + wave * 2 * 256, dzb, lane, wave);
      __syncthreads();
    }
    float rz0 = 0.f, rz1 = 0.f;
    if constexpr (CSC && !GF) {
      auto dzb_at = [&](int c) __attribute__((always_inline)) {
        const int64_t rl = ldbase(c) + zr - mbeg;
        return (rl >= 0 && rl < mend - mbeg) ? dzb[rl * MAXPROJ + zq] : 0.f;
      };
      rz0 = dzb_at(0);
      rz1 = dzb_at(min(1, clast));
    } else if constexpr (!GF) {
      rz0 = a.dz[(uint32_t)((ldbase(0) + zr) * (int)a.lddz + zqc)];
      rz1 = a.dz[(uint32_t)((ldbase(min(1, clast)) + zr) * (int)a.lddz + zqc)];
    }
    load_z(min(2, clast));
    put_zv(0, rz0);
    put_zv(1, rz1);
    scan_scale();
#pragma unroll
    for (int j = 0; j < NPA; ++j) put_a(0, j, 0);
    z_read(0, 0, RP);
#pragma unroll
    for (int i = 0; i < RP; ++i) {
      g_row(i, 0, 0, 0);
      g_row(i, 0, 1, 0);
    }
#pragma unroll
    for (int j = 0; j < RP / 2; ++j) split_pair(j);
    g_put(0);
#pragma unroll
    for (int j = 0; j < NPA; ++j) load_a(0, j, min(RING, clast));
    load_g(0, min(RGN, clast));
    __syncthreads();
    for (int c = 0; c < nch; c += 2) {
      compute(c, std::integral_constant<int, 0>{});
      __syncthreads();
      if (c + 1 < nch) {
        compute(c + 1, std::integral_constant<int, 1>{});
        __syncthreads();
      }
    }
  }

  float* slab = a.slab + (int64_t)rblk * a.slab_stride;
  const int Kc = a.k1 + a.k2;
#pragma unroll
  for (int t = 0; t < KTW; ++t) {
    if (NW == 8 && t >= ntl) break;
    const int kp = (kt0 + tbase + t) * 32 + (lane & 31);
    const bool s1 = kp < a.k1;
    const bool s2 = kp >= a.ap_col2 && kp < a.ap_col2 + a.k2;
#pragma unroll
    for (int r = 0; r < 16; ++r) {
      const int row = wrow + (r & 3) + 8 * (r >> 2) + 4 * (lane >> 5);
      const int64_t idx = s1 ? (int64_t)row * a.k1 + kp : (int64_t)a.Nr * a.k1 + (int64_t)row * a.k2 + (kp - a.ap_col2);
      if constexpr ((LAB & 128) != 0) {
        if (row < a.Nr && (s1 || s2) && acc[t][r] == 1.2345f) slab[idx] = 0.f;
      } else {
        if (row < a.Nr && (s1 || s2)) slab[idx] = acc[t][r] * gunsc;
      }
    }
  }
  __syncthreads();
  float* red = reinterpret_cast<float*>(&At[0][0]);
  constexpr int ns = 2 + MAXPROJ;
  red[(go * 128 + gn) * ns + 0] = db;
  red[(go * 128 + gn) * ns + 1] = dzs;
#pragma unroll
  for (int q = 0; q < MAXPROJ; ++q) red[(go * 128 + gn) * ns + 2 + q] = dw2[q];
  __syncthreads();
  constexpr int NGO = T / 128;
  auto comb = [&](int col, int f) __attribute__((always_inline)) {
    float v = red[col * ns + f];
#pragma unroll
// ... 298 lines not shown
template <int KT>
void launch_tn_planes_kt(const TNArgs& a, int nblk, hipStream_t st) {
  const bool proj = a.dz != nullptr, mask = a.h != nullptr;
  if (proj && mask) launch_tn_planes_k<true, true, KT>(a, nblk, st);
  else if (proj) launch_tn_planes_k<true, false, KT>(a, nblk, st);
  else if (mask) launch_tn_planes_k<false, true, KT>(a, nblk, st);
  else launch_tn_planes_k<false, false, KT>(a, nblk, st);
}

}

bool tn_img16_ok(const TNArgs& a) {
  if (!a.ap || a.ap_h2 || !a.a_bf16 || (a.h && !a.h_bf16)) return false;
  auto al = [](const void* q, int b) { return (reinterpret_cast<uintptr_t>(q) % b) == 0; };
  const int gb = a.g_bf16 ? 8 : 16;
  if (a.Nr % 4 || (a.h && (a.ldh % 4 || !al(a.h, 8))) || (a.g && !a.dz && (a.ldg % 4 || !al(a.g, gb))) ||
      (a.gout && (a.ldgout % 4 || !al(a.gout, gb))))
    return false;
  if ((a.ap_ld != 256 && a.ap_ld != 336) || (reinterpret_cast<uintptr_t>(a.ap) & 15)) return false;
  if (a.k1 < 1 || a.k1 > a.ap_col2 || a.ap_col2 % 8 || a.ap_col2 + a.k2 > a.ap_ld) return false;
  if (a.ap_ps < a.M * (int64_t)a.ap_ld || a.ap_ps * 2 >= ((int64_t)1 << 31) || a.M < PT_ROWS) return false;
  const int64_t ldmax = std::max({a.h ? a.ldh : 0, a.g ? a.ldg : 0, a.dz ? a.lddz : 0});
  return (a.M + 32) * ldmax < ((int64_t)1 << 31);
}

void launch_tn_img16(const TNArgs& a, int nblk, hipStream_t st) {
  if (a.ap_ld == 256) launch_tn_img16_kt<8>(a, nblk, st);
  else launch_tn_img16_kt<11>(a, nblk, st);
}

bool tn_h2_ok(const TNArgs& a) {
  if (!a.ap || !a.ap_h2 || a.a_bf16 || a.h_bf16 || a.g_bf16 || (reinterpret_cast<uintptr_t>(a.ap) & 15)) return false;
  const bool gf = !a.dz && a.g && !a.h && !a.gout;
  if (gf) {
    if ((a.ap_ld != 336 && a.ap_ld != 176) || a.ldg % 4 || (reinterpret_cast<uintptr_t>(a.g) & 15)) return false;
  } else if (!a.dz || !a.proj || !a.h || a.nproj < 1 || a.ap_ld != 336) {
    return false;
  }
  if (a.cptr && (gf || a.gout || !a.cnbr || !a.cu || a.ccols < 1 || a.ccols > 2 || a.ccols > a.nproj ||
                 a.ldu < a.ccols || a.M * a.ldu >= ((int64_t)1 << 31)))
    return false;
  if (a.k1 < 1 || a.k1 > a.ap_col2 || a.ap_col2 % 8 || a.ap_col2 + a.k2 > a.ap_ld) return false;
  if (a.ap_ps < a.M * (int64_t)a.ap_ld || 2 * a.ap_ps * 2 >= ((int64_t)1 << 31) || a.M < PT_ROWS) return false;
  const int64_t ldmax = gf ? a.ldg : std::max({a.ldh, a.lddz});
  return (a.M + 32) * ldmax < ((int64_t)1 << 31);
}

void launch_tn_h2(const TNArgs& a, int nblk, hipStream_t st, bool ks) {
  if (!a.dz) {
    if (a.ap_ld == 176) gemm_tn_h2_kernel<6, false, 0, 8, true><<<nblk, 512, 0, st>>>(a);
    else gemm_tn_h2_kernel<11, false, 0, 8, true><<<nblk, 512, 0, st>>>(a);
    return;
  }
  if (a.cptr) {
    if (ks) gemm_tn_h2_kernel<11, false, 0, 8, false, 2, true><<<nblk, 512, 0, st>>>(a);
    else gemm_tn_h2_kernel<11, false, 0, 8, false, 1, true><<<nblk, 512, 0, st>>>(a);
    return;
  }
  if (ks) {
    if (a.gout) gemm_tn_h2_kernel<11, true, 0, 8, false, 2><<<nblk, 512, 0, st>>>(a);
    else gemm_tn_h2_kernel<11, false, 0, 8, false, 2><<<nblk, 512, 0, st>>>(a);
    return;
  }
  if (a.gout) gemm_tn_h2_kernel<11, true, 0, 8><<<nblk, 512, 0, st>>>(a);
  else gemm_tn_h2_kernel<11, false, 0, 8><<<nblk, 512, 0, st>>>(a);
}

bool tn_planes_ok(const TNArgs& a) {
  if (!a.ap || a.ap_h2 || a.a_bf16 || a.h_bf16 || a.g_bf16) return false;
  if (a.ap_ld % 16 || a.ap_ld > PT_MAXLD || a.ap_ld < 32) return false;
  if (a.k1 < 1 || a.k1 > a.ap_col2 || a.ap_col2 % 8 || a.ap_col2 + a.k2 > a.ap_ld) return false;
  if (a.ap_ps < a.M * (int64_t)a.ap_ld || (reinterpret_cast<uintptr_t>(a.ap) & 15)) return false;
  if (3 * a.ap_ps * 2 >= ((int64_t)1 << 31) || a.M < PT_ROWS) return false;
  const int64_t ldmax = std::max({a.h ? a.ldh : 0, a.g ? a.ldg : 0, a.dz ? a.lddz : 0});
  return (a.M + 32) * ldmax < ((int64_t)1 << 31);
}

void launch_tn_planes(const TNArgs& a, int nblk, hipStream_t st) {
  const int kt = (a.ap_ld + 31) / 32;
  if (kt <= 4) launch_tn_planes_kt<4>(a, nblk, st);
  else if (kt <= 6) launch_tn_planes_kt<6>(a, nblk, st);
  else if (kt <= 8) launch_tn_planes_kt<8>(a, nblk, st);
  else launch_tn_planes_kt<11>(a, nblk, st);
}

}

using namespace gnnmp;

extern "C" gnn_status gnn_split_h2_f32(const float* x, int64_t ldx, int64_t rows, int64_t F, void* img, int64_t ld,
                                       int64_t plane_stride, int64_t col0, int64_t width, int32_t scale_exp,
                                       gnn_stream_t stream) {
  if (scale_exp < -100 || scale_exp > 100) return fail(GNN_ERR_INVALID_ARG, __func__, "scale_exp outside [-100, 100]");
  if (rows < 0 || F < 0 || ldx < F || width < F || (width & 1) || (col0 & 1) || col0 < 0 || col0 + width > ld ||
      plane_stride < rows * ld || (plane_stride & 1) || (ld & 1))
    return fail(GNN_ERR_INVALID_ARG, __func__, "bad shapes (width >= F, even width / col0 / ld / plane_stride)");
  if (rows == 0 || width == 0) return GNN_OK;
  if (!x && F > 0) return fail(GNN_ERR_INVALID_ARG, __func__, "null x");
  if (!img || (reinterpret_cast<uintptr_t>(img) & 3)) return fail(GNN_ERR_INVALID_ARG, __func__, "null or unaligned image");
  const int64_t n = rows * (width / 2);
  split_h2_kernel<<<(unsigned)ceil_div(n, 256), 256, 0, (hipStream_t)stream>>>(
      x, ldx, rows, (int32_t)F, static_cast<uint16_t*>(img) + col0, ld, plane_stride, (int32_t)width,
      ldexpf(1.0f, scale_exp));
  return hip_check(hipGetLastError(), __func__);
}

// ... 14 lines not shown
```

### elliptic_gnn_project_amd/fused.py

```python
from __future__ import annotations

import ctypes
import functools
import os
from typing import List

import torch

from . import _lib
from .aggregation import KernelTimer, aggregate, agg_bytes
from .graph import GraphPlan, get_plan
from .planes import (BfImage, HalfPairImage, SplitImage, bf_x_image, h2_ok, is_registered, mean_planes_ok, padded_mean_planes_ok, x_padded,
                     register_input, x_image, x_only_image)

_PLANES = os.environ.get("GNNMP_PLANES", "1") != "0"
_H2 = os.environ.get("GNNMP_H2", "1") != "0"
_KEEP_MASK = os.environ.get("GNNMP_KEEP_MASK", "0") == "1"
_K1_PREP = os.environ.get("GNNMP_K1_PREP", "1") != "0"
_AGG_CACHE = os.environ.get("GNNMP_AGG_CACHE", "1") != "0"
_K1_PAD = os.environ.get("GNNMP_K1_PAD", "1") != "0"
_SIDE_PREP = os.environ.get("GNNMP_SIDE_PREP", "0") == "1"
_TN_CSC = os.environ.get("GNNMP_TN_CSC", "1") != "0"
_NT_COLSUM = os.environ.get("GNNMP_NT_COLSUM", "1") != "0"
_GCN_CE = os.environ.get("GNNMP_GCN_CE", "1") != "0"
_BN_COLSUM = os.environ.get("GNNMP_BN_COLSUM", "1") != "0"
_SIDE_STREAMS = {}


def _side_stream(dev: torch.device) -> torch.cuda.Stream:
    key = dev.index if dev.index is not None else torch.cuda.current_device()
    if key not in _SIDE_STREAMS:
        _SIDE_STREAMS[key] = torch.cuda.Stream(device=key)
    return _SIDE_STREAMS[key]

MAX_PROJ = 4

GEMM_MATH = {"split_bf16": _lib.MATH_SPLIT_BF16, "f32": _lib.MATH_F32, "half_pair": _lib.MATH_HALF_PAIR}
_DEFAULT_MATH = GEMM_MATH[os.environ.get("GNNMP_GEMM_MATH", "split_bf16")]


def _math(math) -> int:
    if math is None:
        return _DEFAULT_MATH
    return GEMM_MATH[math] if isinstance(math, str) else int(math)


def _ld(t: torch.Tensor) -> int:
    return max(int(t.stride(0)), int(t.size(1)), 1)


@functools.lru_cache(maxsize=256)
def _nt_ws_bytes(n, k1, k2) -> int:
    nb = _lib.c_size(0)
    _lib.call("gnn_gemm_nt_workspace_size", n, k1, k2, nb)
    return int(nb.value)


@functools.lru_cache(maxsize=256)
def _tn_ws_bytes(M, nr, kc, nproj) -> int:
    nb = _lib.c_size(0)
    _lib.call("gnn_gemm_tn_workspace_size", M, nr, kc, nproj, nb)
    return int(nb.value)


def _nt_workspace(device, n, k1, k2):
    return torch.empty(max(_nt_ws_bytes(n, k1, k2) // 4, 1), dtype=torch.float32, device=device)


def _planes_fields(planes):
    if planes is None:
        return (None, 0, 0, 0, _lib.PLANES_SPLIT_BF16)
    return (planes.ptr, planes.ld, planes.ps, planes.col2, getattr(planes, "fmt", _lib.PLANES_SPLIT_BF16))


_BF_IMAGE = os.environ.get("GNNMP_BF_IMAGE", "1") != "0"
# ... 29 lines not shown
        _math(math),
        _lib.ptr(ws), ws.numel() * 4 if ws is not None else 0,
        _lib.DTYPE_BF16 if bf else _lib.DTYPE_F32,
        _lib.DTYPE_BF16 if (out is not None and out.dtype == torch.bfloat16) else _lib.DTYPE_F32,
        _lib.ptr(mask), _ld(mask) if mask is not None else 0, float(mask_scale),
        *_planes_fields(planes), _lib.ptr(keep_mask), int(b_stage == "ready"),
        int(getattr(planes, "exp", 0)),
    )
    if row_exp is not None:
        p.row_exp = row_exp.data_ptr()
    part = None
    if colsum and out is not None and b_stage is None and not check_planes:
        nb = ctypes.c_int32(0)
        _lib.call("gnn_gemm_nt_colsum_blocks", p, ctypes.byref(nb))
        if nb.value > 0:
            part = torch.empty(nb.value * n, dtype=torch.float32, device=dev)
            p.colsum_part, p.colsum_cap = part.data_ptr(), part.numel()
    if check_planes:
        return bool(_lib.load().gnn_gemm_nt_planes_ok(p))
    if b_stage == "params":
        return p
    if b_stage == "prep":
        _lib.call("gnn_gemm_nt_prep_b", p, _lib.stream_handle(dev))
        return None
    if KernelTimer.active:
        e0 = torch.cuda.Event(enable_timing=True)
        e1 = torch.cuda.Event(enable_timing=True)
        e0.record()
    _lib.call("gnn_gemm_nt_f32", p, _lib.stream_handle(dev))
    if KernelTimer.active:
        e1.record()
        k = k1 + k2
        ea = 2 if bf else (4 if a1 is None else a1.element_size())
        prod = 0 if (_math(math) == _lib.MATH_F32 or w1 is None) else (1 if ea == 2 else 6)
        if getattr(planes, "fmt", None) == _lib.PLANES_HALF_PAIR or (
                _math(math) == _lib.MATH_HALF_PAIR and planes is None and h2s_nt_ok(n, k1, k2, a1.dtype)):
            prod = 3
        if ea == 4 and proj is None and (n <= 8 or (k <= 8 and a2 is None)):
            prod = -1
        KernelTimer.records.append((("gemm_nt", M, k, n, ea, out.element_size() if out is not None else 0, prod),
                                    e0, e1, 2 * M * k * n))
    if colsum:
        from .aggregation import colsum as _colsum

        if part is None:
            return out, _colsum(out)
        db = torch.empty(n, dtype=torch.float32, device=dev)
        _lib.call("gnn_colsum_finish_f32", part.data_ptr(), part.numel() // n, n, db.data_ptr(), _lib.stream_handle(dev))
        return out, db
    return out


def gemm_tn(nr, a1, a2=None, g=None, dz=None, proj=None, h=None, hscale=1.0, gout=None, math=None,
            planes=None, check_planes=False, sq=None, sq_skip=(0, 0), row_exp=None, csc=None):
    if planes is not None:
        M, k1, k2, dev = planes.n, planes.k1, planes.k2, planes.img.device
    else:
        M, k1, k2, dev = a1.size(0), a1.size(1), (a2.size(1) if a2 is not None else 0), a1.device
    bf = getattr(planes, "bf16", False) or (a1 is not None and a1.dtype == torch.bfloat16)
    nproj = proj.size(0) if dz is not None else 0
    n_out = nr * (k1 + k2) + nr + nproj * nr + nproj
    p = _lib.GnnGemmTNParams(
        M, nr,
        _lib.ptr(g), _ld(g) if g is not None else 0,
        _lib.ptr(dz), _ld(dz) if dz is not None else 0,
        _lib.ptr(proj), nproj,
        _lib.ptr(h), _ld(h) if h is not None else 0, float(hscale),
        _lib.ptr(gout), _ld(gout) if gout is not None else 0,
        _lib.ptr(a1), _ld(a1) if a1 is not None else 0, k1,
        _lib.ptr(a2), _ld(a2) if a2 is not None else 0, k2,
        _math(math),
        _lib.DTYPE_BF16 if bf else _lib.DTYPE_F32,
        _lib.DTYPE_BF16 if (h is not None and h.dtype == torch.bfloat16) else _lib.DTYPE_F32,
        *_planes_fields(planes),
        _lib.DTYPE_BF16 if any(t is not None and t.dtype == torch.bfloat16 for t in (g, gout)) else _lib.DTYPE_F32,
        int(getattr(planes, "exp", 0)),
    )
    if row_exp is not None:
        p.row_exp = row_exp.data_ptr()
    if g is not None and dz is None and planes is not None:
        from .aggregation import rowmax_of

        rm = rowmax_of(g)
        if rm is not None:
            p.g_rowmax = rm.data_ptr()
    if csc is not None:
        cplan, u = csc
        p.dz_graph, p.dz_u, p.ldu, p.dz_cols = ctypes.addressof(cplan.c_graph), u.data_ptr(), _ld(u), u.size(1)
    if check_planes:
        return bool(_lib.load().gnn_gemm_tn_planes_ok(p))
    out = torch.empty(n_out, dtype=torch.float32, device=dev)
    if sq is not None:
        lo, hi = (int(v) + n_out if v < 0 else int(v) for v in sq_skip)
        p.sq_partial, p.sq_step = sq[0].data_ptr(), sq[1].data_ptr()
        p.sq_skip_lo, p.sq_skip_hi, p.sq_cap = lo, hi, sq[0].numel()
    ws = torch.empty(max(_tn_ws_bytes(M, nr, k1 + k2, nproj) // 4, 1), dtype=torch.float32, device=dev)
    if KernelTimer.active:
        e0 = torch.cuda.Event(enable_timing=True)
        e1 = torch.cuda.Event(enable_timing=True)
        e0.record()
    _lib.call("gnn_gemm_tn_f32", p, out.data_ptr(), ws.data_ptr(), ws.numel() * 4, _lib.stream_handle(dev))
    if sq is not None:
        from .train_ops import grad_sq_produced

        grad_sq_produced(dev, (out, n_out, (lo, hi), _sq_blocks(n_out), sq[0], sq[1], out._version))
    if KernelTimer.active:
        e1.record()
        ea = 2 if bf else (4 if a1 is None else a1.element_size())
        prod = 0 if _math(math) == _lib.MATH_F32 else (1 if ea == 2 else 6)
        if getattr(planes, "fmt", None) == _lib.PLANES_HALF_PAIR or (
                _math(math) == _lib.MATH_HALF_PAIR and row_exp is not None and g is not None and dz is None):
            prod = 3
        if ea == 4 and nr <= 8 and dz is None and h is None and gout is None:
            prod = -1
        KernelTimer.records.append((("gemm_tn", M, k1 + k2, nr, ea, h.element_size() if h is not None else 4, prod),
                                    e0, e1, 2 * M * (k1 + k2) * nr))
    o = 0
    dW1 = out[o: o + nr * k1].view(nr, k1)
    o += nr * k1
    dW2_ = out[o: o + nr * k2].view(nr, k2) if k2 else None
    o += nr * k2
    db = out[o: o + nr]
    o += nr
    dW2 = out[o: o + nproj * nr].view(nproj, nr) if nproj else None
    o += nproj * nr
    dzs = out[o: o + nproj] if nproj else None
    return (dW1, dW2_), db, dW2, dzs


@functools.lru_cache(maxsize=64)
def _sq_blocks(n_out: int) -> int:
    nb = _lib.c_i32(0)
    _lib.call("gnn_gemm_tn_sq_blocks", n_out, ctypes.byref(nb))
    return int(nb.value)


def gemm_nt_input(x: torch.Tensor, n: int, **kw):
    if _H2:
        im = x_only_image(x, HalfPairImage)
        if im is not None and gemm_nt(None, None, n, planes=im, check_planes=True, **kw):
            return gemm_nt(None, None, n, planes=im, **kw)
    im = x_only_image(x)
    if im is not None and gemm_nt(None, None, n, planes=im, check_planes=True, **kw):
        return gemm_nt(None, None, n, planes=im, **kw)
    return gemm_nt(x, None, n, **kw)


def _csc_fold(ctx, dz, u, hscale):
    L = ctx.meta[0]
    if not _TN_CSC or L != 2 or ctx.needs_input_grad[0] or ctx.bimgs[0] is not None:
        return None
    saved = ctx.saved_tensors
    if saved[L] is not None or getattr(ctx, "image", None) is None or not isinstance(ctx.image[0], HalfPairImage):
        return None
    im = ctx.image[0]
    hs1, Wl0 = saved[1], saved[2 * L - 1]
    csc = (ctx.plan, u)
    if not gemm_tn(Wl0.size(0), None, None, h=hs1, hscale=hscale, planes=im, check_planes=True, dz=dz, proj=ctx.P,
                   csc=csc):
        return None
    return csc


def gemm_tn_input(nr: int, x: torch.Tensor, g: torch.Tensor):
    if _H2:
        im = x_only_image(x, HalfPairImage)
        if im is not None and gemm_tn(nr, None, g=g, planes=im, check_planes=True):
            return gemm_tn(nr, None, g=g, planes=im)
    im = x_only_image(x)
    if im is not None and gemm_tn(nr, None, g=g, planes=im, check_planes=True):
        return gemm_tn(nr, None, g=g, planes=im)
    return gemm_tn(nr, x, g=g)


def _k1_pads(x: torch.Tensor) -> bool:
    return _K1_PAD and (x.size(1) + 7) // 8 * 8 > x.size(1)


def _layer0_image(x: torch.Tensor, n_out: int, nt_kw, h2: bool = False, plan=None):
    if not (_PLANES and is_registered(x) and mean_planes_ok(x)) or x.size(0) < 32:
        return None
    if _k1_pads(x) and not padded_mean_planes_ok(x):
        return None
    if h2 and _H2 and HalfPairImage.addressable(x.size(0), x.size(1), x.size(1)) and h2_ok(x):
        im = x_image(x, HalfPairImage)
        if gemm_nt(None, None, n_out, planes=im, check_planes=True, **nt_kw):
            return None if (plan is not None and im.agg_foreign(plan)) else im
    if not SplitImage.addressable(x.size(0), x.size(1), x.size(1)):
        return None
    im = x_image(x)
    if not gemm_nt(None, None, n_out, planes=im, check_planes=True, **nt_kw):
        return None
    return None if (plan is not None and im.agg_foreign(plan)) else im


def _bf_image0(x: torch.Tensor, L: int, Wl, plan=None):
    if not _BF_IMAGE or L < 2 or x.dim() != 2 or x.size(0) < 32 or x.stride(1) != 1:
        return None
    n, fi = x.size(0), x.size(1)
    for l in range(L - 1):
        fo = Wl[l].size(0)
        ld = ((fi + 7) // 8 * 16 + 15) // 16 * 16
        if ld not in (256, 336) or not (8 <= fo <= 128 and fo % 8 == 0):
            return None
        if n * max(ld, fo) * 2 >= 2 ** 31 or n * 4 * 4 >= 2 ** 31:
            return None
        fi = fo
    im = bf_x_image(x)
    return None if (plan is not None and im.agg_foreign(plan)) else im


class _FusedSAGE(torch.autograd.Function):
    @staticmethod
    @torch.amp.custom_fwd(device_type="cuda", cast_inputs=torch.float32)
# ... 51 lines not shown
                ws, side, ready = _nt_workspace(h.device, n_out, im.k1, im.k2), None, False
                prep_b = None
                if _K1_PREP and isinstance(im, HalfPairImage):
                    prep_b = lambda: gemm_nt(None, None, n_out, planes=im, workspace=ws, b_stage="params", **nt_kw)
                elif _SIDE_PREP:
                    side, cur = _side_stream(h.device), torch.cuda.current_stream(h.device)
                    side.wait_stream(cur)
                    with torch.cuda.stream(side):
                        gemm_nt(None, None, n_out, planes=im, workspace=ws, b_stage="prep", **nt_kw)
                    ready = True
                xp = x_padded(h, im.col2) if _k1_pads(h) else None
                gen, hit = im.mean_cached(plan, h, keep, prep_b=prep_b, x_pad=xp, cache=_AGG_CACHE)
                ctx.image = (im, gen)
                if side is not None:
                    cur.wait_stream(side)
                if prep_b is not None and not hit:
                    ready = True
                hn = gemm_nt(None, None, n_out, planes=im, workspace=ws, b_stage="ready" if ready else None, **nt_kw)
                agg = None
            else:
                agg = aggregate(plan, h, _lib.AGG_MEAN, nodew=plan.deg)
                hn = gemm_nt(agg, None, Wl[l].size(0), a2=h, **nt_kw)
            aggs.append(agg)
            hs.append(hn)
        from .train_ops import ce_target, sage_out_mean_ce

        tgt = ce_target()
        if tgt is not None and any(ctx.needs_input_grad) and z.dtype == torch.float32 and C <= 4:
            e0 = KernelTimer.begin()
            logits, ce = sage_out_mean_ce(plan, z, C, bl[-1], tgt)
            KernelTimer.end(e0, ("agg", _lib.AGG_MEAN, False, C), agg_bytes(plan, C, _lib.AGG_MEAN, False, False))
            logits._gnnmp_ce = ce
        else:
            logits = aggregate(plan, z[:, :C], _lib.AGG_MEAN, nodew=plan.deg, addend=z[:, C:], bias=bl[-1])
        ctx.plan = plan
        ctx.meta = (L, C, float(dropout_p))
        ctx.P = P
        ctx.save_for_backward(*hs, *aggs, *params)
        return logits

    @staticmethod
    @torch.amp.custom_bwd(device_type="cuda")
    def backward(ctx, dlogits):
        plan = ctx.plan
        L, C, p = ctx.meta
        saved = ctx.saved_tensors
        hs = saved[:L]
        aggs = saved[L: 2 * L - 1]
        params = saved[2 * L - 1:]
        Wl, Wr = params[0::3], params[2::3]
        hscale = 1.0 / (1.0 - p) if p > 0 else 1.0
        N = dlogits.size(0)
        csc_fold = None
        buf = getattr(dlogits, "_gnnmp_dz", None)
        if (buf is not None and buf.shape == (N, 2 * C) and dlogits.stride() == (2 * C, 1)
                and dlogits.data_ptr() == buf.data_ptr() + C * buf.element_size()):
            dz = buf
            u = getattr(dlogits, "_gnnmp_u", None)
            if u is not None:
                csc_fold = _csc_fold(ctx, dz, u, hscale)
                if csc_fold is None:
                    aggregate(plan, u, _lib.AGG_SUM, transpose=True, out=dz[:, :C])
            else:
                aggregate(plan, dlogits, _lib.AGG_MEAN_BWD, transpose=True, nodew=plan.deg, out=dz[:, :C])
        else:
            dlogits = dlogits.contiguous()
            dz = torch.empty((N, 2 * C), dtype=torch.float32, device=dlogits.device)
            aggregate(plan, dlogits, _lib.AGG_MEAN_BWD, transpose=True, nodew=plan.deg, out=dz[:, :C])
            dz[:, C:].copy_(dlogits)
        P = ctx.P
        grads = [None] * (3 * L)
        need_x = ctx.needs_input_grad[0]
        from .train_ops import grad_sq_produced, grad_sq_request

        grad_sq_produced(dz.device, None)
        sq = grad_sq_request(dz.device) if (L == 2 and dz is buf) else None
        g = None
        for l in range(L - 2, -1, -1):
            fo, fi = Wl[l].shape
            need_g = l > 0 or need_x
            bim = ctx.bimgs[l]
            gimg = None
            if bim is not None and need_g and fi <= 128 and 8 <= fi and fi % 8 == 0 and 2 * fo in (256,) and _BF_IMAGE:
                gimg = BfImage(N, fo, fo, dz.device)
                gout = gimg.a2
            else:
                gout = torch.empty((N, fo), dtype=torch.float32, device=dz.device) if need_g else None
            a_l, im = aggs[l], None
            if bim is not None:
                tn_kw = dict(dz=dz, proj=P) if l == L - 2 else dict(g=g)
                if gemm_tn(fo, None, None, h=hs[l + 1], hscale=hscale, gout=gout, planes=bim, check_planes=True,
                           **tn_kw):
                    im = bim
            if a_l is None:
                im, gen = ctx.image
                if im.gen != gen:
                    im.fill_mean(plan, hs[0])
                tn_kw = dict(dz=dz, proj=P) if l == L - 2 else dict(g=g)
                if not gemm_tn(fo, None, None, h=hs[l + 1], hscale=hscale, gout=gout, planes=im,
                               check_planes=True, **tn_kw):
                    a_l, im = aggregate(plan, hs[0], _lib.AGG_MEAN, nodew=plan.deg), None
            if l == L - 2:
                dW, db, dW2, dzs = gemm_tn(fo, a_l, hs[l], dz=dz, proj=P, h=hs[l + 1], hscale=hscale,
                                           gout=gout, planes=im, sq=sq, sq_skip=(-2 * C, -C), csc=csc_fold)
                grads[3 * (L - 1) + 0] = dW2[:C]
                grads[3 * (L - 1) + 1] = dzs[C:]
                grads[3 * (L - 1) + 2] = dW2[C:]
            else:
                dW, db, _, _ = gemm_tn(fo, a_l, hs[l], g=g, h=hs[l + 1], hscale=hscale, gout=gout, planes=im)
            grads[3 * l + 0] = dW[0]
            grads[3 * l + 1] = db
            grads[3 * l + 2] = dW[1]
            if gimg is not None:
                aggregate(plan, gout, _lib.AGG_MEAN_BWD, transpose=True, nodew=plan.deg, out=gimg.a1)
                g = gemm_nt(None, None, fi, planes=gimg, w1=Wl[l].t().contiguous(), w2=Wr[l].t().contiguous(),
                            out=torch.empty((N, fi), dtype=torch.bfloat16, device=dz.device))
            elif need_g and fi <= 128:
                aggG = aggregate(plan, gout, _lib.AGG_MEAN_BWD, transpose=True, nodew=plan.deg)
                g = gemm_nt(aggG, None, fi, a2=gout, w1=Wl[l].t().contiguous(), w2=Wr[l].t().contiguous())
            elif need_g:
                dA = torch.empty((N, 2 * fi), dtype=torch.float32, device=dz.device)
                gemm_nt(gout, Wl[l], fi, out=dA[:, :fi])
                gemm_nt(gout, Wr[l], fi, out=dA[:, fi:])
                g = aggregate(plan, dA[:, :fi], _lib.AGG_MEAN_BWD, transpose=True, nodew=plan.deg,
                              addend=dA[:, fi:])
        dx = g.to(hs[0].dtype) if need_x else None
        return (dx, None, None, None, None, None, *grads)


class _FusedGCN(torch.autograd.Function):

    @staticmethod
    @torch.amp.custom_fwd(device_type="cuda", cast_inputs=torch.float32)
    def forward(ctx, x, plan: GraphPlan, dropout_p: float, seeds: List[int], seed_ctr, *params):
        L = len(params) // 2
        W, b = params[0::2], params[1::2]
        hs = [x.contiguous()]
        dinv = plan.dinv
        for l in range(L - 1):
            y = gemm_nt_input(hs[0], W[0].size(0), w1=W[0]) if l == 0 else gemm_nt(hs[-1], None, W[l].size(0), w1=W[l])
            hs.append(aggregate(plan, y, _lib.AGG_GCN, nodew=dinv, bias=b[l], relu=True,
                                dropout_p=dropout_p, seed=seeds[l], seed_ptr=seed_ctr))
        y = gemm_nt(hs[-1], None, W[-1].size(0), w1=W[-1])
        from .train_ops import ce_target, gcn_out_ce

        tgt = ce_target()
        if tgt is not None and any(ctx.needs_input_grad) and y.dtype == torch.float32 and y.size(1) <= 2 \
                and y.size(0) > 0 and _GCN_CE:
            e0 = KernelTimer.begin()
            logits, ce = gcn_out_ce(plan, y, b[-1], tgt)
            KernelTimer.end(e0, ("agg", _lib.AGG_GCN, False, y.size(1)), agg_bytes(plan, y.size(1), _lib.AGG_GCN, False, False))
            logits._gnnmp_ce = ce
        else:
            logits = aggregate(plan, y, _lib.AGG_GCN, nodew=dinv, bias=b[-1])
        ctx.plan = plan
        ctx.meta = (L, float(dropout_p))
        ctx.save_for_backward(*hs, *params)
# ... 331 lines not shown
```

### include/gnnmp.h

```cpp
#ifndef GNNMP_H_
#define GNNMP_H_

#include <stddef.h>
#include <stdint.h>

#ifdef __cplusplus
extern "C" {
#endif

#define GNNMP_ABI_VERSION 27

typedef struct ihipStream_t* gnn_stream_t;

typedef enum {
  GNN_OK = 0,
  GNN_ERR_INVALID_ARG = 1,
  GNN_ERR_INDEX_OUT_OF_RANGE = 2,
  GNN_ERR_HIP = 3,
  GNN_ERR_WORKSPACE = 4,
  GNN_ERR_UNSUPPORTED = 5
} gnn_status;

typedef enum {
  GNN_LOOPS_KEEP = 0,
  GNN_LOOPS_REPLACE = 1
} gnn_loop_mode;

typedef struct {
  int32_t seg_len;
  int32_t reserved;
  int64_t num_long;
  int64_t num_pieces;
  const int32_t* ptr;
  const int32_t* nbr;
  const int32_t* piece0;
  const int32_t* piece_seg;
  const int32_t* long_seg;
  const int32_t* order;
} gnn_split;

typedef struct {
  int64_t num_nodes;
  int64_t num_slots;
  const int32_t* rowptr;
  const int32_t* col;
  const int32_t* colptr;
  const int32_t* row;
  const int32_t* csc2csr;
  const gnn_split* csr_split;
  const gnn_split* csc_split;
} gnn_graph;

int gnn_abi_version(void);
const char* gnn_status_string(gnn_status s);
const char* gnn_last_error(void);

gnn_status gnn_graph_workspace_size(int64_t num_nodes, int64_t num_edges, size_t* bytes);

gnn_status gnn_graph_build(const int64_t* edge_index, int64_t num_edges, int64_t num_nodes,
                           gnn_loop_mode loops, int32_t* rowptr, int32_t* col, int32_t* csr_eid,
                           int32_t* colptr, int32_t* row, int32_t* csc2csr, int32_t* stats,
                           void* workspace, size_t workspace_bytes, gnn_stream_t stream);

gnn_status gnn_split_workspace_size(int64_t num_segs, size_t* bytes);
gnn_status gnn_split_count(const int32_t* ptr, int64_t num_segs, int32_t seg_len, int64_t* counts,
                           gnn_stream_t stream);
gnn_status gnn_split_build(const int32_t* ptr, const int32_t* nbr, int64_t num_segs, int32_t seg_len,
                           int32_t* tptr, int32_t* tnbr, int32_t* piece0, int32_t* piece_seg,
                           int32_t* long_seg, int32_t* order, void* workspace, size_t workspace_bytes,
                           gnn_stream_t stream);

gnn_status gnn_in_degree_f32(const gnn_graph* g, float* deg, gnn_stream_t stream);

gnn_status gnn_gcn_norm_f32(const gnn_graph* g, float* dinv, gnn_stream_t stream);

typedef enum {
  GNN_AGG_SUM = 0,
  GNN_AGG_MEAN = 1,
  GNN_AGG_MEAN_BWD = 2,
  GNN_AGG_GCN = 3,
  GNN_AGG_EDGE_W = 4
} gnn_agg_mode;

typedef struct {
  gnn_agg_mode mode;
  int32_t transpose;
  const float* nodew;
  const float* ew;
  int32_t heads;
  const float* addend;
  int64_t ld_add;
  const float* bias;
  int32_t relu;
  float* part;
  size_t part_bytes;
  float dropout_p;
  uint64_t seed;
  const int64_t* seed_ptr;
  const float* addend2;
  int64_t ld_add2;
} gnn_agg_params;

gnn_status gnn_aggregate_f32(const gnn_graph* g, const gnn_agg_params* p, const float* x,
                             int64_t ldx, int64_t F, float* y, int64_t ldy, gnn_stream_t stream);

gnn_status gnn_aggregate_bf16(const gnn_graph* g, const gnn_agg_params* p, const void* x, int64_t ldx,
                              int64_t F, void* y, int64_t ldy, gnn_stream_t stream);

gnn_status gnn_split_planes_f32(const float* x, int64_t ldx, int64_t rows, int64_t F, void* img, int64_t ld,
                                int64_t plane_stride, int64_t col0, int64_t width, gnn_stream_t stream);
gnn_status gnn_sage_mean_fwd_planes(const gnn_graph* g, const float* deg, const float* x, int64_t ldx, int64_t F,
                                    void* img, int64_t ld, int64_t plane_stride, int64_t width,
                                    gnn_stream_t stream);

gnn_status gnn_split_h2_f32(const float* x, int64_t ldx, int64_t rows, int64_t F, void* img, int64_t ld,
                            int64_t plane_stride, int64_t col0, int64_t width, int32_t scale_exp,
                            gnn_stream_t stream);
struct gnn_gemm_nt_params;
gnn_status gnn_sage_mean_fwd_h2(const gnn_graph* g, const float* deg, const float* x, int64_t ldx, int64_t F,
                                void* img, int64_t ld, int64_t plane_stride, int64_t width, int32_t scale_exp,
                                uint32_t* keep_mask, int64_t mask_cols, float dropout_p, uint64_t seed,
                                const uint64_t* seed_ptr, const struct gnn_gemm_nt_params* prep_b,
                                const gnn_split* hub, gnn_stream_t stream);
typedef enum {
  GNN_PLANES_SPLIT_BF16 = 0,
  GNN_PLANES_HALF_PAIR = 1
} gnn_planes_format;

gnn_status gnn_sage_out_mean_ce_f32(const gnn_graph* g, const float* deg, const float* z, int64_t ldz, int32_t C,
                                    const float* bias, float* logits, int64_t ldo, const int64_t* y,
                                    const uint8_t* mask, const float* class_w, float inv_denom, float* dlogits,
                                    int64_t ld_d, float* u, int64_t ldu, float* colsum, float* loss, void* workspace,
                                    size_t workspace_bytes, gnn_stream_t stream);

gnn_status gnn_sage_mean_fwd_f32(const gnn_graph* g, const float* deg, const float* x, int64_t ldx,
                                 int64_t F, float* out, int64_t ldo, gnn_stream_t stream);
gnn_status gnn_sage_mean_bwd_f32(const gnn_graph* g, const float* deg, const float* dout,
                                 int64_t ld_dout, int64_t F, float* dx, int64_t ld_dx,
                                 gnn_stream_t stream);

gnn_status gnn_edge_dot_f32(const gnn_graph* g, const int32_t* eid, const float* nodew, const float* a,
                            int64_t lda, const float* b, int64_t ldb, int64_t F, float* out,
                            gnn_stream_t stream);

gnn_status gnn_gat_scores_f32(int64_t N, int32_t H, int32_t C, const float* xh, int64_t ld_xh,
                              const float* att_src, const float* att_dst, float* a_src,
                              float* a_dst, gnn_stream_t stream);

gnn_status gnn_gat_fwd_f32(const gnn_graph* g, int32_t H, int32_t C, int32_t concat, float slope,
                           const float* xh, int64_t ld_xh, const float* a_src, const float* a_dst,
                           const float* bias, float* alpha, float* out, int64_t ldo,
                           gnn_stream_t stream);

typedef enum { GNN_ACT_NONE = 0, GNN_ACT_ELU = 1 } gnn_act;
typedef struct {
  int32_t heads, chans, concat;
  float slope;
// ... 78 lines not shown
  void* workspace; size_t workspace_bytes;
  int32_t a_dtype;
  int32_t c_dtype;
  const float* mask;
  int64_t ldmask;
  float mask_scale;
  const void* a_planes;
  int64_t planes_ld, planes_stride, planes_col2;
  int32_t planes_format;
  const uint32_t* keep_mask;
  int32_t b_ready;
  int32_t planes_exp;
  float* colsum_part; int64_t colsum_cap;
  int32_t* row_exp;
} gnn_gemm_nt_params;

gnn_status gnn_gemm_nt_colsum_blocks(const gnn_gemm_nt_params* p, int32_t* nb);
gnn_status gnn_gemm_nt_workspace_size(int64_t N, int64_t k1, int64_t k2, size_t* bytes);
gnn_status gnn_gemm_nt_f32(const gnn_gemm_nt_params* p, gnn_stream_t stream);
gnn_status gnn_gemm_nt_prep_b(const gnn_gemm_nt_params* p, gnn_stream_t stream);

typedef struct {
  int64_t M, Nr;
  const float* g; int64_t ldg;
  const float* dz; int64_t lddz;
  const float* proj; int32_t nproj;
  const float* h; int64_t ldh; float hscale;
  float* gout; int64_t ldgout;
  const float* a1; int64_t lda1; int64_t k1;
  const float* a2; int64_t lda2; int64_t k2;
  int32_t math;
  int32_t a_dtype;
  int32_t h_dtype;
  const void* a_planes;
  int64_t planes_ld, planes_stride, planes_col2;
  int32_t planes_format;
  int32_t g_dtype;
  int32_t planes_exp;
  float* sq_partial;
  const float* sq_step;
  int64_t sq_skip_lo, sq_skip_hi, sq_cap;
  const int32_t* row_exp;
  const uint32_t* g_rowmax;
  const gnn_graph* dz_graph;
  const float* dz_u; int64_t ldu;
  int32_t dz_cols;
} gnn_gemm_tn_params;

#define GNN_ROWMAX_ROWS 16

gnn_status gnn_gemm_tn_workspace_size(int64_t M, int64_t Nr, int64_t Kc, int32_t nproj, size_t* bytes);
gnn_status gnn_gemm_tn_f32(const gnn_gemm_tn_params* p, float* out, void* workspace, size_t workspace_bytes,
                           gnn_stream_t stream);
gnn_status gnn_gemm_tn_sq_blocks(int64_t n_out, int32_t* nb);
int gnn_gemm_nt_planes_ok(const gnn_gemm_nt_params* p);
int gnn_gemm_tn_planes_ok(const gnn_gemm_tn_params* p);

gnn_status gnn_colsum_workspace_size(int64_t rows, int64_t F, size_t* bytes);
gnn_status gnn_colsum_finish_f32(const float* part, int32_t nblk, int64_t F, float* out, gnn_stream_t stream);
gnn_status gnn_colsum_f32(int64_t rows, int64_t F, const float* x, int64_t ldx, float* out,
                          void* workspace, size_t workspace_bytes, gnn_stream_t stream);

gnn_status gnn_bn_workspace_size(int64_t C, size_t* bytes);
gnn_status gnn_bn_stats_f32(const float* z, int64_t ldz, int64_t N, int64_t C, double* stats, int32_t finalize,
                            float eps, float momentum, float* mean, float* invstd, float* running_mean,
                            float* running_var, int64_t* num_batches_tracked, void* workspace,
                            size_t workspace_bytes, gnn_stream_t stream);
gnn_status gnn_bn_finalize_f32(const double* stats, int64_t C, float eps, float momentum, float* mean,
                               float* invstd, float* running_mean, float* running_var,
                               int64_t* num_batches_tracked, gnn_stream_t stream);
gnn_status gnn_bn_act_res_fwd_f32(const float* z, int64_t ldz, const float* r, int64_t ldr, int64_t N, int64_t C,
                                  const float* mean, const float* invstd, const float* weight, const float* bias,
                                  float dropout_p, uint64_t seed, const int64_t* seed_ptr, float* h, int64_t ldh,
                                  gnn_stream_t stream);
gnn_status gnn_bn_act_bwd_reduce_f32(const float* dh, int64_t lddh, const float* z, int64_t ldz, int64_t N,
                                     int64_t C, const float* mean, const float* invstd, const float* weight,
                                     const float* bias, float dropout_p, uint64_t seed, const int64_t* seed_ptr,
                                     float* sums, void* workspace, size_t workspace_bytes, gnn_stream_t stream);
gnn_status gnn_bn_act_bwd_f32(const float* dh, int64_t lddh, const float* z, int64_t ldz, int64_t N, int64_t C,
                              const float* mean, const float* invstd, const float* weight, const float* bias,
                              float dropout_p, uint64_t seed, const int64_t* seed_ptr, const float* sums,
                              const double* n_total, float* dz, int64_t lddz, gnn_stream_t stream);
gnn_status gnn_bn_act_bwd_colsum_blocks(int64_t N, int64_t C, int32_t* nb);
gnn_status gnn_bn_act_bwd_colsum_f32(const float* dh, int64_t lddh, const float* z, int64_t ldz, int64_t N, int64_t C,
                                     const float* mean, const float* invstd, const float* weight, const float* bias,
                                     float dropout_p, uint64_t seed, const int64_t* seed_ptr, const float* sums,
                                     const double* n_total, float* dz, int64_t lddz, float* colsum,
                                     gnn_stream_t stream);

gnn_status gnn_time_inject_sin_f32(const float* x, int64_t ldx, int64_t N, int64_t F, const int64_t* t_idx,
                                   int64_t dim, int64_t max_timestep, float* out, int64_t ldo, gnn_stream_t stream);

gnn_status gnn_masked_ce_workspace_size(int64_t N, size_t* bytes);
gnn_status gnn_masked_ce_finish(const float* partial, int32_t nblk, float inv_denom, float* loss, gnn_stream_t stream);
gnn_status gnn_gcn_out_ce_f32(const gnn_graph* g, const float* dinv, const float* t, int64_t ldt, int32_t C,
                              const float* bias, float* logits, int64_t ldo, const int64_t* y, const uint8_t* mask,
                              const float* class_w, float inv_denom, float* dlogits, int64_t ld_d, float* colsum,
                              float* loss, void* workspace, size_t workspace_bytes, gnn_stream_t stream);
gnn_status gnn_masked_ce_colsum_f32(int64_t N, int32_t C, const float* logits, int64_t ldx, const int64_t* y,
                                    const uint8_t* mask, const float* class_w, float inv_denom, float* dlogits,
                                    int64_t ld_d, float* loss, void* workspace, size_t workspace_bytes,
                                    float* colsum, gnn_stream_t stream);
gnn_status gnn_masked_ce_f32(int64_t N, int32_t C, const float* logits, int64_t ldx, const int64_t* y,
                             const uint8_t* mask, const float* class_w, float inv_denom, float* dlogits,
                             int64_t ld_d, float* loss, void* workspace, size_t workspace_bytes,
                             gnn_stream_t stream);
// ... 59 lines not shown
```

Baseline: 2.213 billion edges/s.

## Skip zero dz row groups in layer-1 TN GEMM via aggregation activity flags

The transpose-sum aggregation that builds dz now also writes one activity byte per 16-row group, set when any row in the group has nonzero gradient or projection columns. A new ACT variant of the half-pair TN GEMM uses these flags to walk only active row chunks, skipping A/G/Z loads and MMA work for all-zero groups. With masked CE most nodes carry zero gradient, so this is meant to cut backward weight-gradient work. The cost is an extra ballot and flag store in the aggregation, k-split being disabled on this path, and added kernel variants and checks in the workspace and layout logic.

```diff
diff --git a/elliptic_gnn_project_amd/_lib.py b/elliptic_gnn_project_amd/_lib.py
--- a/elliptic_gnn_project_amd/_lib.py
+++ b/elliptic_gnn_project_amd/_lib.py
@@ -8,7 +8,7 @@
 
 PKG_DIR = Path(__file__).resolve().parent
 LIB_PATH = Path(os.environ["GNNMP_LIB"]) if os.environ.get("GNNMP_LIB") else PKG_DIR / "libgnnmp.so"
-ABI_VERSION = 27
+ABI_VERSION = 28
 
 DTYPE_F32 = 0
 DTYPE_BF16 = 1
@@ -141,6 +141,11 @@
 
 
 ROWMAX_ROWS = 16
+ACTIVE_ROWS = 16
+
+
+class GnnAggActive(ctypes.Structure):
+    _fields_ = [("row_active", c_ptr), ("active_with", c_ptr), ("ld_active_with", c_i64), ("active_with_cols", c_i32)]
 
 
 ACT_NONE = 0
@@ -214,6 +219,11 @@
         ctypes.c_int,
         [ctypes.POINTER(GnnGraph), ctypes.POINTER(GnnAggParams), c_ptr, c_i64, c_i64, c_ptr, c_i64, c_ptr],
     ),
+    "gnn_aggregate_active_f32": (
+        ctypes.c_int,
+        [ctypes.POINTER(GnnGraph), ctypes.POINTER(GnnAggParams), c_ptr, c_i64, c_i64, c_ptr, c_i64,
+         ctypes.POINTER(GnnAggActive), c_ptr],
+    ),
     "gnn_aggregate_bf16": (
         ctypes.c_int,
         [ctypes.POINTER(GnnGraph), ctypes.POINTER(GnnAggParams), c_ptr, c_i64, c_i64, c_ptr, c_i64, c_ptr],
@@ -295,6 +305,8 @@
     "gnn_gemm_tn_workspace_size": (ctypes.c_int, [c_i64, c_i64, c_i64, c_i32, ctypes.POINTER(c_size)]),
     "gnn_gemm_tn_sq_blocks": (ctypes.c_int, [c_i64, ctypes.POINTER(c_i32)]),
     "gnn_gemm_tn_f32": (ctypes.c_int, [ctypes.POINTER(GnnGemmTNParams), c_ptr, c_ptr, c_size, c_ptr]),
+    "gnn_gemm_tn_active_f32": (ctypes.c_int, [ctypes.POINTER(GnnGemmTNParams), c_ptr, c_ptr, c_ptr, c_size, c_ptr]),
+    "gnn_gemm_tn_active_pays": (ctypes.c_int, [c_i64]),
     "gnn_gemm_nt_planes_ok": (ctypes.c_int, [ctypes.POINTER(GnnGemmNTParams)]),
     "gnn_gemm_nt_colsum_blocks": (ctypes.c_int, [ctypes.POINTER(GnnGemmNTParams), ctypes.POINTER(c_i32)]),
     "gnn_colsum_finish_f32": (ctypes.c_int, [c_ptr, c_i32, c_i64, c_ptr, c_ptr]),
diff --git a/elliptic_gnn_project_amd/aggregation.py b/elliptic_gnn_project_amd/aggregation.py
--- a/elliptic_gnn_project_amd/aggregation.py
+++ b/elliptic_gnn_project_amd/aggregation.py
@@ -75,8 +75,11 @@
               nodew: torch.Tensor | None = None, ew: torch.Tensor | None = None, heads: int = 1,
               addend: torch.Tensor | None = None, bias: torch.Tensor | None = None,
               relu: bool = False, out: torch.Tensor | None = None, dropout_p: float = 0.0, seed: int = 0,
-              seed_ptr: torch.Tensor | None = None, addend2: torch.Tensor | None = None) -> torch.Tensor:
+              seed_ptr: torch.Tensor | None = None, addend2: torch.Tensor | None = None,
+              active: tuple | None = None) -> torch.Tensor:
     if x.dtype == torch.bfloat16:
+        if active is not None:
+            raise NotImplementedError("activity flags on the bf16-storage aggregation")
         if dropout_p > 0 or addend2 is not None:
             raise NotImplementedError("dropout / addend2 epilogue on the bf16-storage aggregation")
         return _aggregate_bf16(plan, x, mode, transpose, nodew, addend, bias, relu, out)
@@ -103,8 +106,19 @@
         a = torch.cuda.Event(enable_timing=True)
         b = torch.cuda.Event(enable_timing=True)
         a.record()
-    _lib.call("gnn_aggregate_f32", plan.c_graph, p, x.data_ptr(), _ld(x), F, out.data_ptr(), _ld(out),
-              _lib.stream_handle(x.device))
+    if active is not None:
+        flags, with_ = active
+        if flags.dtype != torch.uint8 or flags.numel() < (N + _lib.ACTIVE_ROWS - 1) // _lib.ACTIVE_ROWS:
+            raise ValueError("activity flags: uint8, one per 16 rows")
+        if with_ is not None and (with_.dtype != torch.float32 or with_.size(0) != N or with_.stride(1) != 1):
+            raise ValueError("active with_: f32 rows of the plan's nodes")
+        act = _lib.GnnAggActive(flags.data_ptr(), _lib.ptr(with_), _ld(with_) if with_ is not None else 0,
+                                with_.size(1) if with_ is not None else 0)
+        _lib.call("gnn_aggregate_active_f32", plan.c_graph, p, x.data_ptr(), _ld(x), F, out.data_ptr(), _ld(out),
+                  act, _lib.stream_handle(x.device))
+    else:
+        _lib.call("gnn_aggregate_f32", plan.c_graph, p, x.data_ptr(), _ld(x), F, out.data_ptr(), _ld(out),
+                  _lib.stream_handle(x.device))
     if KernelTimer.active:
         b.record()
         KernelTimer.records.append((("agg", int(mode), bool(transpose), int(F)), a, b,
diff --git a/elliptic_gnn_project_amd/csrc/aggregate.hip b/elliptic_gnn_project_amd/csrc/aggregate.hip
--- a/elliptic_gnn_project_amd/csrc/aggregate.hip
+++ b/elliptic_gnn_project_amd/csrc/aggregate.hip
@@ -92,6 +92,7 @@
   int64_t nrows;
   int32_t F;
   const int32_t* piece0;
+  uint8_t* row_active; const float* act_with; int64_t ld_act_with; int32_t act_cols;
   const int32_t* order;
   float* part;
   const int32_t* fptr;
@@ -866,8 +867,10 @@
   }
 }
 
-template <int MODE, int NF, int kNarrowCap = 256, bool COOP = false, bool CE = false, bool CEV = false>
+template <int MODE, int NF, int kNarrowCap = 256, bool COOP = false, bool CE = false, bool CEV = false,
+          bool ACT = false>
 __global__ __launch_bounds__(256) void agg_narrow_lds_kernel(AggArgs a) {
+  static_assert(!ACT || (!CE && GNN_ACTIVE_ROWS == 16), "ACT: the plain aggregation, 16-row groups");
   __shared__ float sv[4][kNarrowCap * 4];
   const int lane = threadIdx.x & 63;
   const int w = threadIdx.x >> 6;
@@ -918,6 +921,12 @@
       if (a.ce_rw) ce_rw = a.ce_rw[rr];
     }
   }
+  float actv[4] = {0.f, 0.f, 0.f, 0.f};
+  if constexpr (ACT) {
+#pragma unroll
+    for (int c = 0; c < 4; ++c)
+      if (a.act_cols > 0) actv[c] = a.act_with[rr * a.ld_act_with + min(c, a.act_cols - 1)];
+  }
   float acc[4] = {0.f, 0.f, 0.f, 0.f};
   float* buf = sv[w];
   for (int32_t pb = base; pb < wend; pb += kNarrowCap) {
@@ -1017,6 +1026,26 @@
           a.y[r * a.ldy + f] = t[0];
           lg[f] = t[0];
         }
+      }
+    }
+  }
+  if constexpr (ACT) {
+    bool nz = false;
+    if (rok) {
+      nz = a.piece0 && a.piece0[r] >= 0;
+#pragma unroll
+      for (int f = 0; f < 4; ++f) nz = nz || (f < F && lg[f] != 0.0f) || (f < a.act_cols && actv[f] != 0.0f);
+    }
+    const uint64_t bm = __ballot(nz);
+    uint32_t word = 0u;
+#pragma unroll
+    for (int gq = 0; gq < 4; ++gq) word |= ((bm >> (16 * gq)) & 0xffffu) ? (1u << (8 * gq)) : 0u;
+    const int64_t g0 = r0 / GNN_ACTIVE_ROWS, ng = (a.nrows + GNN_ACTIVE_ROWS - 1) / GNN_ACTIVE_ROWS;
+    if (lane == 0) {
+      if (g0 + 4 <= ng) {
+        *reinterpret_cast<uint32_t*>(a.row_active + g0) = word;
+      } else {
+        for (int gq = 0; g0 + gq < ng; ++gq) a.row_active[g0 + gq] = (uint8_t)((word >> (8 * gq)) & 0xffu);
       }
     }
   }
@@ -1212,6 +1241,10 @@
         else if constexpr (kLdsF >= 4) agg_narrow_lds_kernel<MODE, 4, 256, false><<<nb, 256, 0, st>>>(a);
       } else
 #endif
+      if (a.row_active) {
+        if (a.F <= 2) agg_narrow_lds_kernel<MODE, 2, 256, true, false, false, true><<<nb, 256, 0, st>>>(a);
+        else if constexpr (kLdsF >= 4) agg_narrow_lds_kernel<MODE, 4, 256, true, false, false, true><<<nb, 256, 0, st>>>(a);
+      } else
       if (a.F <= 2) agg_narrow_lds_kernel<MODE, 2, 256, true><<<nb, 256, 0, st>>>(a);
       else if constexpr (kLdsF >= 4) agg_narrow_lds_kernel<MODE, 4, 256, true><<<nb, 256, 0, st>>>(a);
     }
@@ -1362,7 +1395,22 @@
 extern "C" gnn_status gnn_aggregate_f32(const gnn_graph* g, const gnn_agg_params* p, const float* x,
                                         int64_t ldx, int64_t F, float* y, int64_t ldy,
                                         gnn_stream_t stream) {
+  return gnn_aggregate_active_f32(g, p, x, ldx, F, y, ldy, nullptr, stream);
+}
+
+extern "C" gnn_status gnn_aggregate_active_f32(const gnn_graph* g, const gnn_agg_params* p, const float* x,
+                                               int64_t ldx, int64_t F, float* y, int64_t ldy,
+                                               const gnn_agg_active* act, gnn_stream_t stream) {
   if (!g || !p) return fail(GNN_ERR_INVALID_ARG, __func__, "null graph or params");
+  if (act && !act->row_active) act = nullptr;
+  if (act) {
+    if (act->active_with_cols < 0 || act->active_with_cols > 4 || (act->active_with_cols > 0 && !act->active_with) ||
+        act->ld_active_with < act->active_with_cols || (reinterpret_cast<uintptr_t>(act->row_active) & 3))
+      return fail(GNN_ERR_INVALID_ARG, __func__, "activity flags: 0 <= active_with_cols <= 4, ld >= cols, 4-byte aligned flags");
+    const int64_t fmax = p->mode == GNN_AGG_EDGE_W ? 0 : p->mode == GNN_AGG_GCN ? 2 : 4;
+    if (F < 1 || F > fmax || agg_lab().lane_walk)
+      return fail(GNN_ERR_UNSUPPORTED, __func__, "activity flags need the narrow form (F <= 4; GCN F <= 2; not EDGE_W)");
+  }
   if (F < 0 || F > INT32_MAX || ldx < F || ldy < F)
     return fail(GNN_ERR_INVALID_ARG, __func__, "bad F / leading dimensions");
   if (g->num_nodes > 0 && F > 0 && (!x || !y)) return fail(GNN_ERR_INVALID_ARG, __func__, "null x/y");
@@ -1375,6 +1423,10 @@
   a.heads = p->heads > 0 ? p->heads : 1;
   a.x = x; a.ldx = ldx; a.y = y; a.ldy = ldy;
   a.add2 = p->addend2; a.ld_add2 = p->ld_add2;
+  if (act) {
+    a.row_active = act->row_active; a.act_with = act->active_with;
+    a.ld_act_with = act->ld_active_with; a.act_cols = act->active_with_cols;
+  }
   if (!a.ptr || (g->num_slots > 0 && !a.nbr)) return fail(GNN_ERR_INVALID_ARG, __func__, "plan arrays null");
   if ((p->mode == GNN_AGG_MEAN || p->mode == GNN_AGG_MEAN_BWD || p->mode == GNN_AGG_GCN) && !p->nodew)
     return fail(GNN_ERR_INVALID_ARG, __func__, "mode needs nodew");
diff --git a/elliptic_gnn_project_amd/csrc/gemm_common.hpp b/elliptic_gnn_project_amd/csrc/gemm_common.hpp
--- a/elliptic_gnn_project_amd/csrc/gemm_common.hpp
+++ b/elliptic_gnn_project_amd/csrc/gemm_common.hpp
@@ -174,7 +174,9 @@
   const int32_t* rowexp;
   const uint32_t* growmax;
   const int32_t* cptr; const int32_t* cnbr; const float* cu; int64_t ldu; int32_t ccols;
+  const uint8_t* dz_active;
 };
+constexpr int TN_ACT_CAP = 512;
 
 void launch_nt_x3(const NTArgs& a, void* ws, size_t ws_bytes, hipStream_t st);
 size_t nt_x3_workspace(int64_t k1, int64_t k2);
diff --git a/elliptic_gnn_project_amd/csrc/gemm_f32.hip b/elliptic_gnn_project_amd/csrc/gemm_f32.hip
--- a/elliptic_gnn_project_amd/csrc/gemm_f32.hip
+++ b/elliptic_gnn_project_amd/csrc/gemm_f32.hip
@@ -728,6 +728,13 @@
   if (v >= 0) return v != 0;
   return (rows_per_block + 63) / 64 + 1 <= 8;
 }
+
+static bool tn_active_pays(int64_t M) {
+  if (M < 16) return false;
+  const int64_t rpb = tn_h2_rows_per_block(M, true);
+  return (rpb + 63) / 64 + 1 > 8;
+}
+static int64_t tn_active_bytes(int64_t M) { return (ceil_div(M, GNN_ACTIVE_ROWS) + 15) / 16 * 16; }
 
 int tn_blocks2(int64_t M) {
   const int64_t chunks = ceil_div(M, 32);
@@ -900,11 +907,14 @@
   if (Nr <= 8 && nproj == 0) nb = std::max<int64_t>(nb, tn_skinny_blocks(M));
   if (Nr <= 64 && Kc <= 128 && nproj == 0) nb = std::max<int64_t>(nb, tn_blocks2(M));
   *bytes = (size_t)nb * stride * sizeof(float);
+  if (nproj > 0 && tn_active_pays(M)) *bytes += (size_t)tn_active_bytes(M);
   return GNN_OK;
 }
 
+extern "C" int gnn_gemm_tn_active_pays(int64_t M) { return tn_active_pays(M) ? 1 : 0; }
+
 static gnn_status gemm_tn_dispatch(const gnn_gemm_tn_params* p, float* out, void* workspace,
-                                   size_t workspace_bytes, gnn_stream_t stream);
+                                   size_t workspace_bytes, gnn_stream_t stream, const uint8_t* dz_active = nullptr);
 
 static bool tn_csc_args(const gnn_gemm_tn_params* p, TNArgs* a) {
   a->cptr = nullptr; a->cnbr = nullptr; a->cu = nullptr; a->ldu = 0; a->ccols = 0;
@@ -930,11 +940,22 @@
   return gemm_tn_dispatch(p, out, workspace, workspace_bytes, stream);
 }
 
+extern "C" gnn_status gnn_gemm_tn_active_f32(const gnn_gemm_tn_params* p, const uint8_t* dz_active, float* out,
+                                             void* workspace, size_t workspace_bytes, gnn_stream_t stream) {
+  return gemm_tn_dispatch(p, out, workspace, workspace_bytes, stream, dz_active);
+}
+
 
 static gnn_status gemm_tn_dispatch(const gnn_gemm_tn_params* p, float* out, void* workspace,
-                                   size_t workspace_bytes, gnn_stream_t stream) {
-  const char* __fn = "gnn_gemm_tn_f32";
+                                   size_t workspace_bytes, gnn_stream_t stream, const uint8_t* dz_active) {
+  const char* __fn = dz_active ? "gnn_gemm_tn_active_f32" : "gnn_gemm_tn_f32";
   if (!p || !out) return fail(GNN_ERR_INVALID_ARG, __fn, "null params/out");
+  if (dz_active) {
+    if (!p->dz || !p->h || p->gout || p->dz_graph || !p->a_planes || p->planes_format != GNN_PLANES_HALF_PAIR ||
+        p->math == GNN_MATH_F32 || p->M < 16)
+      return fail(GNN_ERR_UNSUPPORTED, __fn, "dz_active needs the half-pair dz form with h, no gout, no dz_graph, M >= 16");
+    if (reinterpret_cast<uintptr_t>(dz_active) & 15) return fail(GNN_ERR_INVALID_ARG, __fn, "dz_active must be 16-byte aligned");
+  }
   if (p->M < 0 || p->Nr < 1 || p->Nr > 128 || p->k1 < 1 || p->k2 < 0 || p->k1 + p->k2 > KMAX)
     return fail(GNN_ERR_UNSUPPORTED, __fn, "needs 1 <= Nr <= 128 and k1 + k2 <= 384");
   const bool planes_only = p->a_planes && !p->a1;
@@ -1006,26 +1027,47 @@
     if (a.ap_exp < -100 || a.ap_exp > 100) return fail(GNN_ERR_INVALID_ARG, __fn, "planes_exp outside [-100, 100]");
     if (a.ap_h2) {
       a.growmax = (!a.dz && a.g) ? p->g_rowmax : nullptr;
+      if (dz_active && !(tn_h2_ok(a) && a.dz && !a.gout && !a.cptr))
+        return fail(GNN_ERR_UNSUPPORTED, __fn, "dz_active outside the half-pair dz-form TN's shapes");
       if (p->math != GNN_MATH_F32 && tn_h2_ok(a)) {
+        const bool call_side = a.cptr && !tn_csc_in_kernel(tn_h2_rows_per_block(a.M, true));
+        uint8_t* ws_flags = nullptr;
+        if (call_side && tn_active_pays(a.M)) {
+          const size_t off = (size_t)nblk * stride * sizeof(float);
+          if (workspace_bytes < off + (size_t)tn_active_bytes(a.M) || (reinterpret_cast<uintptr_t>(workspace) & 15))
+            return fail(GNN_ERR_WORKSPACE, __fn, "workspace too small for the activity flags (gnn_gemm_tn_workspace_size)");
+          ws_flags = static_cast<uint8_t*>(workspace) + off;
+        }
+        a.dz_active = dz_active ? dz_active : ws_flags;
         int nred = nblk;
-        const bool ks = a.dz && a.M <= tn_ksplit_max_m();
-        if (ks) {
+        const bool ksr = a.dz && a.M <= tn_ksplit_max_m();
+        const bool ks = ksr && !a.dz_active;
+        if (ksr) {
           const int64_t chunks = ceil_div(a.M, 32), per = ceil_div(chunks, 128);
           nred = (int)ceil_div(chunks, per);
           a.rows_per_block = per * 32;
         }
         if (a.rows_per_block != tn_h2_rows_per_block(a.M, a.dz != nullptr))
           return fail(GNN_ERR_HIP, __fn, "internal: TN row-block rule mismatch");
+        if (a.dz_active) {
+          if (a.rows_per_block / GNN_ACTIVE_ROWS > TN_ACT_CAP)
+            return fail(GNN_ERR_UNSUPPORTED, __fn, "dz_active: row block beyond the chunk list's capacity");
+        }
         if (a.cptr && !tn_csc_in_kernel(a.rows_per_block)) {
           gnn_agg_params ag{};
           ag.mode = GNN_AGG_SUM;
           ag.transpose = 1;
-          const gnn_status s = gnn_aggregate_f32(p->dz_graph, &ag, p->dz_u, p->ldu, p->dz_cols,
-                                                 const_cast<float*>(p->dz), p->lddz, stream);
+          gnn_agg_active act{};
+          act.row_active = ws_flags;
+          act.active_with = p->dz + p->dz_cols;
+          act.ld_active_with = p->lddz;
+          act.active_with_cols = nproj - p->dz_cols;
+          const gnn_status s = gnn_aggregate_active_f32(p->dz_graph, &ag, p->dz_u, p->ldu, p->dz_cols,
+                                                        const_cast<float*>(p->dz), p->lddz, &act, stream);
           if (s != GNN_OK) return s;
           a.cptr = nullptr;
         }
-        launch_tn_h2(a, ks ? 2 * nred : nblk, st, ks);
+        launch_tn_h2(a, ks ? 2 * nred : nred, st, ks);
         GNN_LAUNCH_CHECK();
         slab_reduce_kernel<<<red_blocks(n_out), 256, 0, st>>>(a.slab, stride, nred, out, n_out, sqo);
         GNN_LAUNCH_CHECK();
diff --git a/elliptic_gnn_project_amd/csrc/gemm_planes.hip b/elliptic_gnn_project_amd/csrc/gemm_planes.hip
--- a/elliptic_gnn_project_amd/csrc/gemm_planes.hip
+++ b/elliptic_gnn_project_amd/csrc/gemm_planes.hip
@@ -477,10 +477,11 @@
   return zm;
 }
 
-template <int KT, bool GOUT, int LAB = 0, int NW = 4, bool GF = false, int KS = 1, bool CSC = false>
+template <int KT, bool GOUT, int LAB = 0, int NW = 4, bool GF = false, int KS = 1, bool CSC = false, bool ACT = false>
 __global__ __launch_bounds__(64 * NW) void gemm_tn_h2_kernel(TNArgs a) {
   static_assert(NW == 4 || NW == 8, "4 or 8 waves");
   static_assert(KS == 1 || (KS == 2 && NW == 8), "split-K: the 8-wave form");
+  static_assert(!ACT || (NW == 8 && !GOUT && !GF && KS == 1 && !CSC && !(LAB & 16)), "ACT: the plain dz form");
   constexpr int T = 64 * NW;
   constexpr int NPA = (2 * PT_ROWS * (PT_MAXLD / 8) + T - 1) / T;
   constexpr int RP = PT_ROWS / (T / 128);
@@ -490,6 +491,8 @@
   __shared__ __attribute__((aligned(16))) uint16_t At[2][2 * PT_APL];
   __shared__ float dzL[2][256];
   __shared__ float redm[2 * NW];
+  __shared__ int32_t clist[ACT ? TN_ACT_CAP : 1];
+  __shared__ int32_t actw[NW];
   constexpr int NU = 2 * NPA + RP / 2 + 2 * RP + RP / 2 + 3;
   constexpr int NG = 3 * KTW;
   constexpr int RING = (LAB & 16) ? 2 : 1;
@@ -505,7 +508,28 @@
   const int pr = min(4 * ktb, (ld - 32 * kt0) >> 3);
   const int64_t mbeg = (int64_t)rblk * a.rows_per_block;
   const int64_t mend = min(a.M, mbeg + a.rows_per_block);
-  const int nch = mend > mbeg ? (int)((mend - mbeg + PT_ROWS - 1) / PT_ROWS) : 0;
+  const int Mi = (int)a.M;
+  int nch = mend > mbeg ? (int)((mend - mbeg + PT_ROWS - 1) / PT_ROWS) : 0;
+  if constexpr (ACT) {
+    const int nf = (Mi + PT_ROWS - 1) / PT_ROWS;
+    const int q0 = (int)(mbeg / PT_ROWS), q1 = min(nf, (int)((mbeg + a.rows_per_block) / PT_ROWS));
+    const int q = q0 + tid;
+    const bool on = q < q1 && a.dz_active[q] != 0;
+    const uint64_t bm = __ballot(on);
+    if (lane == 0) actw[wave] = __popcll(bm);
+    __syncthreads();
+    int wbase = 0, n_act = 0;
+#pragma unroll
+    for (int w2 = 0; w2 < NW; ++w2) {
+      const int v = actw[w2];
+      wbase += w2 < wave ? v : 0;
+      n_act += v;
+    }
+    const int pos = wbase + __popcll(bm & ((1ull << lane) - 1ull));
+    if (on && pos < TN_ACT_CAP) clist[pos] = q;
+    __syncthreads();
+    nch = min(n_act, TN_ACT_CAP);
+  }
   typedef _Float16 f16x8 __attribute__((ext_vector_type(8)));
   const int wrow = 32 * (wave & 3);
   const int tbase = NW == 4 ? 0 : (wave >> 2) * KTW;
@@ -576,7 +600,26 @@
         }
       }
     }
-    for (int64_t r0 = mbeg + tid; !GF && !CSC && r0 < mend; r0 += 4 * T) {
+    if constexpr (ACT) {
+      constexpr int CP = T / PT_ROWS;
+      for (int k0 = tid / PT_ROWS; k0 < nch; k0 += 4 * CP) {
+        float v[4][MAXPROJ];
+#pragma unroll
+        for (int u = 0; u < 4; ++u) {
+          const int64_t r = min(clist[min(k0 + CP * u, nch - 1)] * PT_ROWS + (tid & (PT_ROWS - 1)), Mi - 1);
+#pragma unroll
+          for (int q = 0; q < MAXPROJ; ++q) v[u][q] = a.dz[r * a.lddz + min(q, nq - 1)];
+        }
+#pragma unroll
+        for (int u = 0; u < 4; ++u) {
+          float s = 0.f;
+#pragma unroll
+          for (int q = 0; q < MAXPROJ; ++q) s += q < nq ? fabsf(v[u][q]) : 0.f;
+          zm = fmaxf(zm, k0 + CP * u < nch ? s : 0.f);
+        }
+      }
+    }
+    for (int64_t r0 = mbeg + tid; !GF && !CSC && !ACT && r0 < mend; r0 += 4 * T) {
       float v[4][MAXPROJ];
 #pragma unroll
       for (int u = 0; u < 4; ++u) {
@@ -619,31 +662,54 @@
     gunsc = ldexpf(1.0f, E - 4 - 11 - a.ap_exp);
   };
 
-  const int Mi = (int)a.M;
-  auto ldbase = [&](int c) __attribute__((always_inline)) { return min((int)mbeg + c * PT_ROWS, Mi - PT_ROWS); };
   const int clast = max(nch - 1, 0);
+  auto cid = [&](int c) __attribute__((always_inline)) { return __builtin_amdgcn_readfirstlane(clist[c]); };
+  auto ldbase = [&](int c) __attribute__((always_inline)) {
+    if constexpr (ACT) return min(cid(c) * PT_ROWS, Mi - PT_ROWS);
+    else return min((int)mbeg + c * PT_ROWS, Mi - PT_ROWS);
+  };
+  auto zrange = [&](int k, int& lo, int& hi) __attribute__((always_inline)) {
+    if constexpr (ACT) {
+      const int q = cid(min(k, clast)), mb = min(q * PT_ROWS, Mi - PT_ROWS);
+      lo = k < nch ? q * PT_ROWS - mb : PT_ROWS;
+      hi = min(Mi, (q + 1) * PT_ROWS) - mb;
+    } else {
+      const int mb = ldbase(k);
+      lo = (int)mbeg + k * PT_ROWS - mb;
+      hi = (int)mend - mb;
+    }
+  };
+  int ab2 = 0, ab3 = 0, az2lo = 0, az2hi = 0, glo = 0;
   u32x4 ra[RING][NPA];
   float rg[RGN][RP];
   float rz = 0.f;
-  auto load_a = [&](int s, int j, int c) __attribute__((always_inline)) {
-    ra[s][j] = __builtin_amdgcn_raw_buffer_load_b128(arsrc, (int)goff[j], ldbase(c) * ld * 2, 0);
-  };
-  auto load_g = [&](int sg, int c) __attribute__((always_inline)) {
-    uint32_t o = (uint32_t)((ldbase(c) + RP * go) * hld);
+  auto load_a_at = [&](int s, int j, int mb) __attribute__((always_inline)) {
+    ra[s][j] = __builtin_amdgcn_raw_buffer_load_b128(arsrc, (int)goff[j], mb * ld * 2, 0);
+  };
+  auto load_a = [&](int s, int j, int c) __attribute__((always_inline)) { load_a_at(s, j, ldbase(c)); };
+  auto load_g_at = [&](int sg, int mb) __attribute__((always_inline)) {
+    uint32_t o = (uint32_t)((mb + RP * go) * hld);
 #pragma unroll
     for (int i = 0; i < RP; ++i) {
       rg[sg][i] = hb[o];
       o += (uint32_t)hld;
     }
   };
-  auto load_z = [&](int c) __attribute__((always_inline)) {
-    if constexpr (!GF) rz = a.dz[(uint32_t)((ldbase(c) + zr) * (int)a.lddz + zqc)];
+  auto load_g = [&](int sg, int c) __attribute__((always_inline)) { load_g_at(sg, ldbase(c)); };
+  auto load_z_at = [&](int mb) __attribute__((always_inline)) {
+    if constexpr (!GF) rz = a.dz[(uint32_t)((mb + zr) * (int)a.lddz + zqc)];
+  };
+  auto load_z = [&](int c) __attribute__((always_inline)) { load_z_at(ldbase(c)); };
+  auto put_zlh = [&](int k, int lo, int hi, float v) __attribute__((always_inline)) {
+    if constexpr (GF) return;
+    const bool ok = tid < PT_ROWS * MAXPROJ && zq < a.nproj && zr >= lo && zr < hi;
+    if (T == 256 || tid < 256) dzL[k & 1][tid] = ok ? v : 0.0f;
   };
   auto put_zv = [&](int k, float v) __attribute__((always_inline)) {
     if constexpr (GF) return;
-    const int mb = ldbase(k);
-    const bool ok = tid < PT_ROWS * MAXPROJ && zq < a.nproj && zr >= (int)mbeg + k * PT_ROWS - mb && zr < (int)mend - mb;
-    if (T == 256 || tid < 256) dzL[k & 1][tid] = ok ? v : 0.0f;
+    int lo, hi;
+    zrange(k, lo, hi);
+    put_zlh(k, lo, hi, v);
   };
   auto put_z = [&](int k) __attribute__((always_inline)) { put_zv(k, rz); };
 
@@ -677,6 +743,7 @@
       e[i] = g * gsc;
       return;
     }
+    if constexpr (ACT) rg[sg][i] = RP * go + i >= glo ? rg[sg][i] : 0.0f;
     if (half == 0) {
       const float4 z = zv[i];
       float g = z.x * pcol[0];
@@ -718,8 +785,12 @@
     const int sa = RING == 1 ? 0 : (par ^ 1);
     const int sg = RGN == 1 ? 0 : (par ^ 1);
     if (k < Z0) {
-      if (k & 1) load_a(sa, k >> 1, min(c + 1 + RING, clast));
-      else put_a(sa, k >> 1, c + 1);
+      if (k & 1) {
+        if constexpr (ACT) load_a_at(sa, k >> 1, ab2);
+        else load_a(sa, k >> 1, min(c + 1 + RING, clast));
+      } else {
+        put_a(sa, k >> 1, c + 1);
+      }
     } else if (k < G0) {
       z_read(c + 1, 2 * (k - Z0), 2);
     } else if (k < S0) {
@@ -729,10 +800,16 @@
     } else if (k == P0) {
       g_put(c + 1);
     } else if (k == P0 + 1) {
-      load_g(sg, min(c + 1 + RGN, clast));
+      if constexpr (ACT) load_g_at(sg, ab2);
+      else load_g(sg, min(c + 1 + RGN, clast));
     } else if (k == P0 + 2) {
-      put_z(c + 2);
-      load_z(min(c + 3, clast));
+      if constexpr (ACT) {
+        put_zlh(c + 2, az2lo, az2hi, rz);
+        load_z_at(ab3);
+      } else {
+        put_z(c + 2);
+        load_z(min(c + 3, clast));
+      }
     }
   };
 
@@ -747,6 +824,12 @@
   auto compute = [&](int c, auto parc) __attribute__((always_inline)) {
     constexpr int par = decltype(parc)::value;
     const int buf = c & 1;
+    if constexpr (ACT) {
+      glo = az2lo;
+      zrange(c + 2, az2lo, az2hi);
+      ab2 = ldbase(min(c + 2, clast));
+      ab3 = ldbase(min(c + 3, clast));
+    }
     f16x8 gf[3], af[2][2];
 #pragma unroll
     for (int p = 0; p < 3; ++p) gf[p] = *reinterpret_cast<const f16x8*>(Gt[buf] + p * PT_GPL + gfo);
@@ -818,6 +901,10 @@
 #pragma unroll
     for (int j = 0; j < NPA; ++j) put_a(0, j, 0);
     z_read(0, 0, RP);
+    if constexpr (ACT) {
+      zrange(0, glo, az2hi);
+      zrange(1, az2lo, az2hi);
+    }
 #pragma unroll
     for (int i = 0; i < RP; ++i) {
       g_row(i, 0, 0, 0);
@@ -1222,6 +1309,10 @@
     else gemm_tn_h2_kernel<11, false, 0, 8, true><<<nblk, 512, 0, st>>>(a);
     return;
   }
+  if (a.dz_active) {
+    gemm_tn_h2_kernel<11, false, 0, 8, false, 1, false, true><<<nblk, 512, 0, st>>>(a);
+    return;
+  }
   if (a.cptr) {
     if (ks) gemm_tn_h2_kernel<11, false, 0, 8, false, 2, true><<<nblk, 512, 0, st>>>(a);
     else gemm_tn_h2_kernel<11, false, 0, 8, false, 1, true><<<nblk, 512, 0, st>>>(a);
diff --git a/elliptic_gnn_project_amd/fused.py b/elliptic_gnn_project_amd/fused.py
--- a/elliptic_gnn_project_amd/fused.py
+++ b/elliptic_gnn_project_amd/fused.py
@@ -21,6 +21,7 @@
 _K1_PAD = os.environ.get("GNNMP_K1_PAD", "1") != "0"
 _SIDE_PREP = os.environ.get("GNNMP_SIDE_PREP", "0") == "1"
 _TN_CSC = os.environ.get("GNNMP_TN_CSC", "1") != "0"
+_TN_ACTIVE = os.environ.get("GNNMP_TN_ACTIVE", "1") != "0"
 _NT_COLSUM = os.environ.get("GNNMP_NT_COLSUM", "1") != "0"
 _GCN_CE = os.environ.get("GNNMP_GCN_CE", "1") != "0"
 _BN_COLSUM = os.environ.get("GNNMP_BN_COLSUM", "1") != "0"
@@ -156,7 +157,7 @@
 
 
 def gemm_tn(nr, a1, a2=None, g=None, dz=None, proj=None, h=None, hscale=1.0, gout=None, math=None,
-            planes=None, check_planes=False, sq=None, sq_skip=(0, 0), row_exp=None, csc=None):
+            planes=None, check_planes=False, sq=None, sq_skip=(0, 0), row_exp=None, csc=None, dz_active=None):
     if planes is not None:
         M, k1, k2, dev = planes.n, planes.k1, planes.k2, planes.img.device
     else:
@@ -203,7 +204,13 @@
         e0 = torch.cuda.Event(enable_timing=True)
         e1 = torch.cuda.Event(enable_timing=True)
         e0.record()
-    _lib.call("gnn_gemm_tn_f32", p, out.data_ptr(), ws.data_ptr(), ws.numel() * 4, _lib.stream_handle(dev))
+    if dz_active is not None:
+        if dz_active.dtype != torch.uint8 or dz_active.numel() < (M + _lib.ACTIVE_ROWS - 1) // _lib.ACTIVE_ROWS:
+            raise ValueError("dz_active: uint8, one per 16 rows of dz")
+        _lib.call("gnn_gemm_tn_active_f32", p, dz_active.data_ptr(), out.data_ptr(), ws.data_ptr(), ws.numel() * 4,
+                  _lib.stream_handle(dev))
+    else:
+        _lib.call("gnn_gemm_tn_f32", p, out.data_ptr(), ws.data_ptr(), ws.numel() * 4, _lib.stream_handle(dev))
     if sq is not None:
         from .train_ops import grad_sq_produced
 
@@ -264,6 +271,23 @@
                    csc=csc):
         return None
     return csc
+
+
+def _tn_active_flags(ctx, dz, hscale):
+    L = ctx.meta[0]
+    N = dz.size(0)
+    if not _TN_ACTIVE or L != 2 or ctx.needs_input_grad[0] or ctx.bimgs[0] is not None:
+        return None
+    saved = ctx.saved_tensors
+    if saved[L] is not None or getattr(ctx, "image", None) is None or not isinstance(ctx.image[0], HalfPairImage):
+        return None
+    if not _lib.load().gnn_gemm_tn_active_pays(N):
+        return None
+    hs1, Wl0 = saved[1], saved[2 * L - 1]
+    if not gemm_tn(Wl0.size(0), None, None, h=hs1, hscale=hscale, planes=ctx.image[0], check_planes=True, dz=dz,
+                   proj=ctx.P):
+        return None
+    return torch.empty((N + _lib.ACTIVE_ROWS - 1) // _lib.ACTIVE_ROWS, dtype=torch.uint8, device=dz.device)
 
 
 def gemm_tn_input(nr: int, x: torch.Tensor, g: torch.Tensor):
@@ -421,6 +445,7 @@
         hscale = 1.0 / (1.0 - p) if p > 0 else 1.0
         N = dlogits.size(0)
         csc_fold = None
+        act = None
         buf = getattr(dlogits, "_gnnmp_dz", None)
         if (buf is not None and buf.shape == (N, 2 * C) and dlogits.stride() == (2 * C, 1)
                 and dlogits.data_ptr() == buf.data_ptr() + C * buf.element_size()):
@@ -429,7 +454,11 @@
             if u is not None:
                 csc_fold = _csc_fold(ctx, dz, u, hscale)
                 if csc_fold is None:
-                    aggregate(plan, u, _lib.AGG_SUM, transpose=True, out=dz[:, :C])
+                    act = _tn_active_flags(ctx, dz, hscale)
+                    if act is not None:
+                        aggregate(plan, u, _lib.AGG_SUM, transpose=True, out=dz[:, :C], active=(act, dz[:, C:]))
+                    else:
+                        aggregate(plan, u, _lib.AGG_SUM, transpose=True, out=dz[:, :C])
             else:
                 aggregate(plan, dlogits, _lib.AGG_MEAN_BWD, transpose=True, nodew=plan.deg, out=dz[:, :C])
         else:
@@ -471,7 +500,8 @@
                     a_l, im = aggregate(plan, hs[0], _lib.AGG_MEAN, nodew=plan.deg), None
             if l == L - 2:
                 dW, db, dW2, dzs = gemm_tn(fo, a_l, hs[l], dz=dz, proj=P, h=hs[l + 1], hscale=hscale,
-                                           gout=gout, planes=im, sq=sq, sq_skip=(-2 * C, -C), csc=csc_fold)
+                                           gout=gout, planes=im, sq=sq, sq_skip=(-2 * C, -C), csc=csc_fold,
+                                           dz_active=act if (im is not None and gout is None) else None)
                 grads[3 * (L - 1) + 0] = dW2[:C]
                 grads[3 * (L - 1) + 1] = dzs[C:]
                 grads[3 * (L - 1) + 2] = dW2[C:]
diff --git a/include/gnnmp.h b/include/gnnmp.h
--- a/include/gnnmp.h
+++ b/include/gnnmp.h
@@ -8,7 +8,7 @@
 extern "C" {
 #endif
 
-#define GNNMP_ABI_VERSION 27
+#define GNNMP_ABI_VERSION 28
 
 typedef struct ihipStream_t* gnn_stream_t;
 
@@ -103,6 +103,19 @@
 
 gnn_status gnn_aggregate_f32(const gnn_graph* g, const gnn_agg_params* p, const float* x,
                              int64_t ldx, int64_t F, float* y, int64_t ldy, gnn_stream_t stream);
+
+#define GNN_ACTIVE_ROWS 16
+
+typedef struct {
+  uint8_t* row_active;
+  const float* active_with;
+  int64_t ld_active_with;
+  int32_t active_with_cols;
+} gnn_agg_active;
+
+gnn_status gnn_aggregate_active_f32(const gnn_graph* g, const gnn_agg_params* p, const float* x, int64_t ldx,
+                                    int64_t F, float* y, int64_t ldy, const gnn_agg_active* act,
+                                    gnn_stream_t stream);
 
 gnn_status gnn_aggregate_bf16(const gnn_graph* g, const gnn_agg_params* p, const void* x, int64_t ldx,
                               int64_t F, void* y, int64_t ldy, gnn_stream_t stream);
@@ -287,6 +300,9 @@
 gnn_status gnn_gemm_tn_workspace_size(int64_t M, int64_t Nr, int64_t Kc, int32_t nproj, size_t* bytes);
 gnn_status gnn_gemm_tn_f32(const gnn_gemm_tn_params* p, float* out, void* workspace, size_t workspace_bytes,
                            gnn_stream_t stream);
+gnn_status gnn_gemm_tn_active_f32(const gnn_gemm_tn_params* p, const uint8_t* dz_active, float* out,
+                                  void* workspace, size_t workspace_bytes, gnn_stream_t stream);
+int gnn_gemm_tn_active_pays(int64_t M);
 gnn_status gnn_gemm_tn_sq_blocks(int64_t n_out, int32_t* nb);
 int gnn_gemm_nt_planes_ok(const gnn_gemm_nt_params* p);
 int gnn_gemm_tn_planes_ok(const gnn_gemm_tn_params* p);
```

Result: faster. 2.331 billion edges/s (median of 6 runs) (+5.3%).
